# jnvance/DMRG.x

Measured on AMD Instinct MI355X. Metric: superblock MatMults/sec inside the ground-state eigensolve (Lanczos step = 1 MatMult + reorthogonalisation), higher is better.
Workload: dtype f64

## Files before the change

### dmrg.x_amd/_capi.py

```python
import ctypes as C
import os

_HERE = os.path.dirname(os.path.abspath(__file__))
LIB_PATH = os.environ.get("DMRGX_LIB") or os.path.join(_HERE, "libdmrgx_hip.so")

DMRGX_OK = 0
DMRGX_ERR_ARG = 62
DMRGX_ERR_OUTOFRANGE = 63
DMRGX_ERR_DEVICE = 97
DMRGX_ERR_NOTCONV = 91
CELL_DENSE, CELL_IDENT = 1, 2


class DmrgxError(RuntimeError):
    def __init__(self, code, msg):
        super().__init__(f"dmrgx status {code}: {msg}")
        self.code = code


class Cell(C.Structure):
    _fields_ = [("row_sector", C.c_int32), ("r0", C.c_int32), ("c0", C.c_int32), ("nr", C.c_int32), ("nc", C.c_int32),
                ("kind", C.c_int32), ("scale", C.c_double), ("data", C.c_void_p), ("ld", C.c_int64)]


class SecOp(C.Structure):
    _fields_ = [("shift", C.c_int32), ("transposed", C.c_int32), ("ncells", C.c_int32), ("cells", C.POINTER(Cell))]


class Sectors(C.Structure):
    _fields_ = [("nsec", C.c_int32), ("size", C.POINTER(C.c_int32))]


class Term(C.Structure):
    _fields_ = [("a", C.c_double), ("left_op", C.c_int32), ("right_op", C.c_int32)]


class KronDesc(C.Structure):
    _fields_ = [("left", Sectors), ("right", Sectors), ("nblocks", C.c_int32),
                ("block_il", C.POINTER(C.c_int32)), ("block_ir", C.POINTER(C.c_int32)),
                ("n_left_ops", C.c_int32), ("n_right_ops", C.c_int32),
                ("left_ops", C.POINTER(SecOp)), ("right_ops", C.POINTER(SecOp)),
                ("h_left", C.POINTER(SecOp)), ("h_right", C.POINTER(SecOp)),
                ("nterms", C.c_int32), ("terms", C.POINTER(Term)),
                ("world_size", C.c_int32), ("rank", C.c_int32)]


class RdmReport(C.Structure):
    _fields_ = [(k, C.c_int32) for k in ("n_sweeps", "solver", "trid_persistent_matrices", "trid_launch_matrices", "max_workgroups_per_matrix",
                                         "merge_levels", "wy_blocks_max", "timed_out", "process_timeouts", "persistent_off")]


class RdmVecTask(C.Structure):
    _fields_ = [("side", C.c_int32), ("k", C.c_int32), ("count", C.c_int32), ("pad", C.c_int32), ("dst_dev", C.c_void_p), ("ld", C.c_int64)]


class KronInfo(C.Structure):
    _fields_ = [("n_states", C.c_int64), ("vec_len", C.c_int64), ("local_offset", C.c_int64), ("local_len", C.c_int64),
                ("seg_stride", C.c_int64), ("flops_alg", C.c_double), ("bytes_alg", C.c_double), ("flops_exec", C.c_double),
                ("bytes_workspace", C.c_double), ("n_groups", C.c_int32), ("n_tiles_stage1", C.c_int32), ("n_tiles_stage2", C.c_int32),
                ("n_tiles_big", C.c_int32), ("flops_alg_big", C.c_double)]


class AxpyTask(C.Structure):
    _fields_ = [("dst", C.c_void_p), ("dst_base", C.c_void_p), ("src", C.c_void_p), ("ldd", C.c_int64), ("lds", C.c_int64),
                ("nr", C.c_int32), ("nc", C.c_int32), ("transposed", C.c_int32), ("alpha", C.c_double)]


class Dot2dTask(C.Structure):
    _fields_ = [("a", C.c_void_p), ("lda", C.c_int64), ("b", C.c_void_p), ("ldb", C.c_int64), ("nr", C.c_int32), ("nc", C.c_int32), ("out", C.c_int32), ("pad", C.c_int32)]


class GemmTask(C.Structure):
    _fields_ = [("M", C.c_int32), ("N", C.c_int32), ("K", C.c_int32), ("accumulate", C.c_int32),
                ("A", C.c_void_p), ("lda", C.c_int64), ("B", C.c_void_p), ("ldb", C.c_int64), ("C", C.c_void_p), ("ldc", C.c_int64)]


class Rotation(C.Structure):
    _fields_ = [("n_new", C.c_int32), ("old_sector", C.POINTER(C.c_int32)), ("kept", C.POINTER(C.c_int32)), ("rot_t", C.POINTER(C.c_void_p))]


ALLGATHER_FN = C.CFUNCTYPE(C.c_int32, C.c_void_p, C.c_void_p, C.c_int64, C.c_void_p)
ALLREDUCE_FN = C.CFUNCTYPE(C.c_int32, C.c_void_p, C.c_void_p, C.c_int64, C.c_void_p)


class EigsOpts(C.Structure):
    _fields_ = [("ncv", C.c_int32), ("max_it", C.c_int32), ("tol", C.c_double), ("seed", C.c_uint64),
                ("use_initial", C.c_int32), ("max_matvec", C.c_int32), ("allgather", ALLGATHER_FN), ("allreduce_sum", ALLREDUCE_FN), ("user", C.c_void_p),
                ("comm", C.c_void_p), ("method", C.c_int32), ("min_initial_norm2", C.c_double), ("gd_minv", C.c_int32), ("reserved_", C.c_int32)]


class EigsStats(C.Structure):
    _fields_ = [("n_matvec", C.c_int32), ("n_restart", C.c_int32), ("converged", C.c_int32), ("start_rejected", C.c_int32),
                ("residual", C.c_double), ("seconds", C.c_double)]


SIGNATURES = {
    "dmrgx_abi_version": (C.c_int32, []),
    "dmrgx_last_error": (C.c_char_p, []),
    "dmrgx_device_count": (C.c_int32, [C.POINTER(C.c_int32)]),
    "dmrgx_kron_plan_create": (C.c_int32, [C.POINTER(KronDesc), C.c_void_p, C.POINTER(C.c_void_p)]),
    "dmrgx_kron_plan_info": (C.c_int32, [C.c_void_p, C.POINTER(KronInfo)]),
    "dmrgx_kron_apply": (C.c_int32, [C.c_void_p, C.c_void_p, C.c_void_p, C.c_void_p]),
    "dmrgx_kron_plan_destroy": (C.c_int32, [C.c_void_p]),
    "dmrgx_kron_diag": (C.c_int32, [C.c_void_p, C.c_void_p, C.c_void_p]),
    "dmrgx_kron_plan_timing": (C.c_int32, [C.c_void_p, C.c_int32]),
    "dmrgx_kron_plan_timing_read": (C.c_int32, [C.c_void_p, C.POINTER(C.c_double), C.POINTER(C.c_int64)]),
    "dmrgx_kron_vec_to_striped": (C.c_int32, [C.c_void_p, C.c_void_p, C.c_void_p, C.c_void_p]),
    "dmrgx_kron_vec_from_striped": (C.c_int32, [C.c_void_p, C.c_void_p, C.c_void_p, C.c_void_p]),
    "dmrgx_stripe_bounds": (C.c_int32, [C.c_int32, C.c_int32, C.c_int32, C.POINTER(C.c_int32), C.POINTER(C.c_int32)]),
    "dmrgx_stripe_bounds_of_block": (C.c_int32, [C.c_int32, C.c_int32, C.c_int32, C.c_int32, C.POINTER(C.c_int32), C.POINTER(C.c_int32)]),
    "dmrgx_dgemm_nn": (C.c_int32, [C.c_int32, C.c_int32, C.c_int32, C.c_void_p, C.c_int64, C.c_void_p, C.c_int64,
                                   C.c_void_p, C.c_int64, C.c_void_p]),
    "dmrgx_rdm_create": (C.c_int32, [C.POINTER(Sectors), C.POINTER(Sectors), C.c_int32, C.POINTER(C.c_int32), C.POINTER(C.c_int32),
                                     C.c_void_p, C.c_void_p, C.POINTER(C.c_void_p)]),
    "dmrgx_rdm_eigenvalues": (C.c_int32, [C.c_void_p, C.c_int32, C.c_int32, C.POINTER(C.c_double)]),
    "dmrgx_rdm_create_warm": (C.c_int32, [C.POINTER(Sectors), C.POINTER(Sectors), C.c_int32, C.POINTER(C.c_int32), C.POINTER(C.c_int32),
                               C.c_void_p, C.c_void_p, C.c_void_p, C.POINTER(C.c_void_p)]),
    "dmrgx_rdm_eigenvectors": (C.c_int32, [C.c_void_p, C.c_int32, C.c_int32, C.c_int32, C.c_void_p, C.c_int64, C.c_void_p]),
    "dmrgx_rdm_info": (C.c_int32, [C.c_void_p, C.POINTER(RdmReport)]),
    "dmrgx_rdm_select": (C.c_int32, [C.c_void_p, C.POINTER(C.c_int32), C.c_void_p]),
    "dmrgx_rdm_eigenvectors_batch": (C.c_int32, [C.c_void_p, C.c_int32, C.POINTER(RdmVecTask), C.c_void_p]),
    "dmrgx_rdm_destroy": (C.c_int32, [C.c_void_p]),
    "dmrgx_cells_axpy": (C.c_int32, [C.c_int32, C.POINTER(AxpyTask), C.c_void_p]),
    "dmrgx_rotate_ops": (C.c_int32, [C.POINTER(Sectors), C.POINTER(Rotation), C.c_int32, C.POINTER(SecOp), C.POINTER(C.POINTER(C.c_void_p)), C.c_void_p]),
    "dmrgx_malloc": (C.c_int32, [C.POINTER(C.c_void_p), C.c_size_t]),
    "dmrgx_free": (C.c_int32, [C.c_void_p]),
    "dmrgx_mem_stats": (C.c_int32, [C.POINTER(C.c_size_t), C.POINTER(C.c_size_t), C.POINTER(C.c_size_t)]),
    "dmrgx_memcpy_h2d": (C.c_int32, [C.c_void_p, C.c_void_p, C.c_size_t, C.c_void_p]),
    "dmrgx_memcpy_d2h": (C.c_int32, [C.c_void_p, C.c_void_p, C.c_size_t, C.c_void_p]),
    "dmrgx_memcpy_d2d": (C.c_int32, [C.c_void_p, C.c_void_p, C.c_size_t, C.c_void_p]),
    "dmrgx_memset_zero": (C.c_int32, [C.c_void_p, C.c_size_t, C.c_void_p]),
    "dmrgx_stream_sync": (C.c_int32, [C.c_void_p]),
    "dmrgx_dgemm_batch": (C.c_int32, [C.c_int32, C.c_void_p, C.c_void_p]),
    "dmrgx_dot": (C.c_int32, [C.c_int64, C.c_void_p, C.c_void_p, C.POINTER(C.c_double), C.c_void_p]),
    "dmrgx_dot_async": (C.c_int32, [C.c_int64, C.c_void_p, C.c_void_p, C.c_void_p, C.c_void_p]),
    "dmrgx_dot2d_batch": (C.c_int32, [C.c_int32, C.c_void_p, C.c_void_p, C.c_void_p]),
    "dmrgx_eigs_comm_timing": (C.c_int32, [C.POINTER(C.c_double), C.POINTER(C.c_double), C.POINTER(C.c_int64), C.c_int32]),
    "dmrgx_eigs_lowest": (C.c_int32, [C.c_void_p, C.POINTER(EigsOpts), C.POINTER(C.c_double), C.c_void_p,
                                      C.POINTER(EigsStats), C.c_void_p]),
    "dmrgx_rdm_create_subset": (C.c_int32, [C.POINTER(Sectors), C.POINTER(Sectors), C.c_int32, C.POINTER(C.c_int32), C.POINTER(C.c_int32),
                                            C.c_void_p, C.c_void_p, C.c_void_p, C.POINTER(C.c_void_p)]),
    "dmrgx_set_device": (C.c_int32, [C.c_int32]),
    "dmrgx_comm_unique_id": (C.c_int32, [C.c_void_p]),
    "dmrgx_comm_init": (C.c_int32, [C.c_int32, C.c_int32, C.c_void_p, C.POINTER(C.c_void_p)]),
    "dmrgx_comm_init_host_staged": (C.c_int32, [C.c_int32, C.c_int32, C.c_char_p, C.POINTER(C.c_void_p)]),
    "dmrgx_comm_info": (C.c_int32, [C.c_void_p, C.POINTER(C.c_int32), C.POINTER(C.c_int32), C.POINTER(C.c_int32)]),
    "dmrgx_comm_allgather": (C.c_int32, [C.c_void_p, C.c_void_p, C.c_int64, C.c_void_p]),
    "dmrgx_comm_allreduce_sum": (C.c_int32, [C.c_void_p, C.c_void_p, C.c_int64, C.c_void_p]),
    "dmrgx_comm_bcast": (C.c_int32, [C.c_void_p, C.c_void_p, C.c_size_t, C.c_int32, C.c_void_p]),
    "dmrgx_comm_allgather_host": (C.c_int32, [C.c_void_p, C.c_void_p, C.c_void_p, C.c_size_t, C.c_void_p]),
    "dmrgx_comm_barrier": (C.c_int32, [C.c_void_p, C.c_void_p]),
    "dmrgx_comm_destroy": (C.c_int32, [C.c_void_p]),
}

_lib = None


def lib():
    global _lib
    if _lib is None:
        import torch
        if not os.path.exists(LIB_PATH):
            raise ImportError(f"{LIB_PATH} not built: run `make` (hipcc --offload-arch=gfx950). "
                              "The dmrgx hot path has no CPU fallback.")
        L = C.CDLL(LIB_PATH)
        for name, (res, args) in SIGNATURES.items():
            fn = getattr(L, name)
            fn.restype, fn.argtypes = res, args
        if L.dmrgx_abi_version() != 3:
            raise ImportError("dmrgx ABI version mismatch")
        _lib = L
    return _lib


def check(status):
    if status != DMRGX_OK:
        raise DmrgxError(status, lib().dmrgx_last_error().decode(errors="replace"))


def require_device():
    n = C.c_int32(0)
    check(lib().dmrgx_device_count(C.byref(n)))
    return n.value
```

### dmrg.x_amd/csrc/common.h

```cpp
#pragma once
#include <cstring>
#include <hip/hip_runtime.h>
#include <algorithm>
#include <cstdarg>
#include <cstdio>
#include <cstdint>
#include <string>
#include <vector>
#include "dmrgx.h"

namespace dmrgx {

void set_error(const char* fmt, ...);

#define DMRGX_HIP(call)                                                                              \
    do {                                                                                             \
        hipError_t e__ = (call);                                                                     \
        if (e__ != hipSuccess) {                                                                     \
            ::dmrgx::set_error("%s:%d: %s -> %s", __FILE__, __LINE__, #call, hipGetErrorString(e__)); \
            return DMRGX_ERR_DEVICE;                                                                 \
        }                                                                                            \
    } while (0)

#define DMRGX_CHK(call)                    \
    do {                                   \
        dmrgx_status s__ = (call);         \
        if (s__ != DMRGX_OK) return s__;   \
    } while (0)

#define DMRGX_FAIL(code, ...)              \
    do {                                   \
        ::dmrgx::set_error(__VA_ARGS__);   \
        return (code);                     \
    } while (0)

inline int32_t stripe_cut(int32_t n, int32_t W, int32_t w)
{
    if (w <= 0) return 0;
    if (w >= W) return n;
    const int64_t even = ((int64_t)n * w) / W;
    if ((int64_t)n < (int64_t)48 * W) return (int32_t)even;
    const int64_t c16 = ((even + 8) / 16) * 16, c64 = ((even + 32) / 64) * 64;
    const int64_t d64 = c64 > even ? c64 - even : even - c64;
    const int64_t cut = (d64 <= 16 && c64 > 0 && c64 < n) ? c64 : c16;
    return (int32_t)std::min<int64_t>(std::max<int64_t>(cut, 0), n);
}

hipError_t pool_malloc(void** out, size_t bytes);
hipError_t pool_free(void* p);
hipError_t zero_async(void* p, size_t bytes, hipStream_t st);
constexpr uint64_t POISON_F64_BITS = 0x7ff8badbadbadbadull;
bool pool_poison();
hipError_t poison_f64_async(void* p, size_t bytes, hipStream_t st);
void pool_stats(size_t* in_use, size_t* cached, size_t* peak);
hipError_t h2d_async(void* dst, const void* src, size_t bytes, hipStream_t st);

inline int32_t stripe_of_rank(int32_t W, int32_t w, int32_t k) { return (w + k) % W; }

struct DevBuf {
    void* p = nullptr;
    size_t bytes = 0;
    DevBuf() = default;
    DevBuf(const DevBuf&) = delete;
    DevBuf& operator=(const DevBuf&) = delete;
    ~DevBuf() { release(); }
    dmrgx_status alloc(size_t n) {
        release();
        if (n == 0) return DMRGX_OK;
        hipError_t e = pool_malloc(&p, n);
        if (e != hipSuccess) { p = nullptr; set_error("hipMalloc(%zu) failed: %s", n, hipGetErrorString(e)); return DMRGX_ERR_MEM; }
        bytes = n;
        return DMRGX_OK;
    }
    dmrgx_status alloc_f64(size_t count, hipStream_t st) {
        DMRGX_CHK(alloc(count * sizeof(double)));
        if (p && pool_poison()) DMRGX_HIP(poison_f64_async(p, bytes, st));
        return DMRGX_OK;
    }
    void release() { if (p && owned) (void)pool_free(p); p = nullptr; bytes = 0; owned = true; }
    void view(void* ptr, size_t n) { release(); p = n ? ptr : nullptr; bytes = n; owned = false; }
    template <class T> T* as() const { return reinterpret_cast<T*>(p); }
    bool owned = true;
};

template <class T>
dmrgx_status upload(DevBuf& buf, const std::vector<T>& host, hipStream_t st) {
    DMRGX_CHK(buf.alloc(host.size() * sizeof(T)));
    if (!host.empty()) DMRGX_HIP(h2d_async(buf.p, host.data(), host.size() * sizeof(T), st));
    return DMRGX_OK;
}

struct PackedUpload {
    std::vector<char> host;
    template <class T> size_t add(const std::vector<T>& v) {
        const size_t off = (host.size() + 15) & ~(size_t)15, bytes = v.size() * sizeof(T);
        if (host.capacity() < off + bytes) host.reserve(std::max(2 * host.capacity(), off + bytes + (bytes >> 1)));
        host.resize(off);
        if (bytes) { const char* p = reinterpret_cast<const char*>(v.data()); host.insert(host.end(), p, p + bytes); }
        return off;
    }
    dmrgx_status upload(DevBuf& buf, hipStream_t st) {
        DMRGX_CHK(buf.alloc(std::max<size_t>(host.size(), 16)));
        constexpr size_t piece = (size_t)4 << 20;
        for (size_t off = 0; off < host.size(); off += piece)
            DMRGX_HIP(h2d_async(static_cast<char*>(buf.p) + off, host.data() + off, std::min(piece, host.size() - off), st));
        return DMRGX_OK;
    }
    template <class T> static void view(DevBuf& dst, const DevBuf& arena, size_t off, size_t n) { dst.view(static_cast<char*>(arena.p) + off, n * sizeof(T)); }
};
template <class T> inline T* packed_at(const DevBuf& buf, size_t off) { return reinterpret_cast<T*>(static_cast<char*>(buf.p) + off); }

}
```

### dmrg.x_amd/csrc/eigs.hip

```cpp
#include "common.h"
#include <mutex>
#include <algorithm>
#include <chrono>
#include <cmath>
#include <cstring>
#include <cstddef>

namespace dmrgx {
namespace {

constexpr int DOT_BLOCKS = 1024, DOT_THREADS = 256, DOT_CHUNK = 8, MAX_NCV = 64, FUSE_NV = 24, GD_NV = 8;

__device__ __forceinline__ double wave_sum(double v) {
#pragma unroll
    for (int o = 32; o > 0; o >>= 1) v += __shfl_down(v, o, 64);
    return v;
}

template <bool VEC2>
__global__ void __launch_bounds__(DOT_THREADS)
multi_dot_kernel(const double* __restrict__ V, int64_t ldv, int nv, const double* __restrict__ w, int64_t n, double* __restrict__ partial)
{
    __shared__ double red[DOT_THREADS / 64][DOT_CHUNK];
    const int v0 = blockIdx.y * DOT_CHUNK;
// ... 421 lines not shown
#pragma unroll
    for (int i = 0; i < NVMAX + 2; ++i) {
        if ((DOTS && (i < nv || i == NVMAX)) || i == NVMAX + 1) {
            const double s2 = wave_sum(acc[i]);
            if (lane == 0) red[wave][i] = s2;
        }
    }
    __syncthreads();
    if (DOTS) {
        if (threadIdx.x <= nv + 1) {
            const int src = threadIdx.x < nv ? threadIdx.x : (threadIdx.x == nv ? NVMAX : NVMAX + 1);
            double s2 = 0.0;
            for (int wv = 0; wv < DOT_THREADS / 64; ++wv) s2 += red[wv][src];
            partial[(int64_t)threadIdx.x * gridDim.x + blockIdx.x] = s2;
        }
    } else if (threadIdx.x == 0) {
        double s2 = 0.0;
        for (int wv = 0; wv < DOT_THREADS / 64; ++wv) s2 += red[wv][NVMAX + 1];
        partial[blockIdx.x] = s2;
    }
}

__global__ void gd_zero_pads_kernel(double* __restrict__ W, int64_t ld, int count, int64_t n, double* __restrict__ t, double* __restrict__ D)
{
    for (int j = threadIdx.x; j < count; j += blockDim.x) W[(int64_t)j * ld + n] = 0.0;
    if (threadIdx.x == 0) { t[n] = 0.0; D[n] = 0.0; }
}

__global__ void __launch_bounds__(DOT_THREADS)
gd_reduce_look_kernel(const double* __restrict__ partial, double* __restrict__ out, int count, int nblk, int look_idx, int look_only,
                      const GdState* __restrict__ S, double* __restrict__ look)
{
    __shared__ double red[DOT_THREADS / 64];
    const int i = blockIdx.x;
    if (i >= count) return;
    double t = 0.0;
    if (!look_only) {
        double s = 0.0;
        for (int b = threadIdx.x; b < nblk; b += DOT_THREADS) s += partial[(int64_t)i * nblk + b];
        s = wave_sum(s);
        if ((threadIdx.x & 63) == 0) red[threadIdx.x >> 6] = s;
        __syncthreads();
        if (threadIdx.x == 0) { for (int k = 0; k < DOT_THREADS / 64; ++k) t += red[k]; out[i] = t; }
    } else if (threadIdx.x == 0) t = out[i];
    if (threadIdx.x == 0 && i == look_idx) { look[0] = t; look[1] = S->theta; look[2] = S->hv0_2; }
}

__global__ void random_fill_kernel(double* __restrict__ v, int64_t n, uint64_t seed, int64_t index_offset)
{
    for (int64_t e = (int64_t)blockIdx.x * blockDim.x + threadIdx.x; e < n; e += (int64_t)gridDim.x * blockDim.x) {
        uint64_t z = seed + 0x9E3779B97F4A7C15ull * (uint64_t)(e + index_offset + 1);
        z = (z ^ (z >> 30)) * 0xBF58476D1CE4E5B9ull;
        z = (z ^ (z >> 27)) * 0x94D049BB133111EBull;
        z ^= z >> 31;
        v[e] = (double)(z >> 11) * (2.0 / 9007199254740992.0) - 1.0;
    }
}

void jacobi_eigh(int n, std::vector<double>& A, std::vector<double>& w, std::vector<double>& Q)
{
    Q.assign((size_t)n * n, 0.0);
    for (int i = 0; i < n; ++i) Q[(size_t)i * n + i] = 1.0;
    for (int sweep = 0; sweep < 60; ++sweep) {
        double off = 0.0, diag = 0.0;
        for (int i = 0; i < n; ++i) { diag += A[(size_t)i * n + i] * A[(size_t)i * n + i]; for (int j = i + 1; j < n; ++j) off += A[(size_t)i * n + j] * A[(size_t)i * n + j]; }
        if (off <= 1e-32 * (diag + off) || off == 0.0) break;
        for (int p = 0; p < n - 1; ++p)
            for (int q = p + 1; q < n; ++q) {
                const double apq = A[(size_t)p * n + q];
                if (apq == 0.0) continue;
                const double app = A[(size_t)p * n + p], aqq = A[(size_t)q * n + q];
                const double tau = (aqq - app) / (2.0 * apq);
                const double t = (tau >= 0 ? 1.0 : -1.0) / (std::fabs(tau) + std::sqrt(1.0 + tau * tau));
                const double c = 1.0 / std::sqrt(1.0 + t * t), s = t * c;
                for (int k = 0; k < n; ++k) {
                    const double akp = A[(size_t)k * n + p], akq = A[(size_t)k * n + q];
                    A[(size_t)k * n + p] = c * akp - s * akq; A[(size_t)k * n + q] = s * akp + c * akq;
                }
                for (int k = 0; k < n; ++k) {
                    const double apk = A[(size_t)p * n + k], aqk = A[(size_t)q * n + k];
                    A[(size_t)p * n + k] = c * apk - s * aqk; A[(size_t)q * n + k] = s * apk + c * aqk;
                }
                for (int k = 0; k < n; ++k) {
                    const double qkp = Q[(size_t)k * n + p], qkq = Q[(size_t)k * n + q];
                    Q[(size_t)k * n + p] = c * qkp - s * qkq; Q[(size_t)k * n + q] = s * qkp + c * qkq;
                }
            }
    }
    std::vector<int> idx(n);
    for (int i = 0; i < n; ++i) idx[i] = i;
    std::sort(idx.begin(), idx.end(), [&](int a, int b) { return A[(size_t)a * n + a] < A[(size_t)b * n + b]; });
    w.resize(n);
    std::vector<double> Qs((size_t)n * n);
    for (int j = 0; j < n; ++j) { w[j] = A[(size_t)idx[j] * n + idx[j]]; for (int i = 0; i < n; ++i) Qs[(size_t)i * n + j] = Q[(size_t)i * n + idx[j]]; }
    Q.swap(Qs);
}

}
}

using namespace dmrgx;

static dmrgx_status eigs_davidson(dmrgx_kron_plan* plan, const dmrgx_eigs_opts* opts, double* e0, double* psi_full, dmrgx_eigs_stats* stats, hipStream_t st);

namespace {
std::mutex g_ct_mutex;
double g_ct_allgather_ms = 0.0, g_ct_apply_ms = 0.0;
int64_t g_ct_matvecs = 0;
struct CommTimer {
    hipStream_t st;
    std::vector<hipEvent_t> ev;
    size_t used = 0;
    explicit CommTimer(hipStream_t s) : st(s) {}
    void mark()
    {
        if (used == ev.size()) { hipEvent_t e; if (hipEventCreate(&e) != hipSuccess) return; ev.push_back(e); }
        (void)hipEventRecord(ev[used++], st);
    }
    ~CommTimer()
    {
        double ag = 0.0, ap = 0.0; int64_t nmv = 0;
        for (size_t i = 0; i + 2 < used; i += 3) {
            float a = 0.f, b = 0.f;
            if (hipEventSynchronize(ev[i + 2]) != hipSuccess) break;
            if (hipEventElapsedTime(&a, ev[i], ev[i + 1]) == hipSuccess && hipEventElapsedTime(&b, ev[i + 1], ev[i + 2]) == hipSuccess) { ag += a; ap += b; ++nmv; }
        }
        for (hipEvent_t e : ev) (void)hipEventDestroy(e);
        if (nmv) { std::lock_guard<std::mutex> lk(g_ct_mutex); g_ct_allgather_ms += ag; g_ct_apply_ms += ap; g_ct_matvecs += nmv; }
    }
};
}

extern "C" dmrgx_status dmrgx_eigs_comm_timing(double* allgather_ms, double* apply_ms, int64_t* n_matvec, int32_t reset)
{
    std::lock_guard<std::mutex> lk(g_ct_mutex);
    if (allgather_ms) *allgather_ms = g_ct_allgather_ms;
    if (apply_ms) *apply_ms = g_ct_apply_ms;
    if (n_matvec) *n_matvec = g_ct_matvecs;
    if (reset) { g_ct_allgather_ms = 0.0; g_ct_apply_ms = 0.0; g_ct_matvecs = 0; }
    return DMRGX_OK;
}

static double* pinned_scalars()
{
    static thread_local double* p = nullptr;
    if (!p && hipHostMalloc((void**)&p, (8 + MAX_NCV + 2) * sizeof(double), hipHostMallocDefault) != hipSuccess) { (void)hipGetLastError(); p = nullptr; }
    return p;
}
static bool start_too_light(const dmrgx_eigs_opts* opts, const double* pin)
{
    return opts->min_initial_norm2 > 0.0 && pin && !(pin[2] >= opts->min_initial_norm2);
}

extern "C" dmrgx_status dmrgx_eigs_lowest(dmrgx_kron_plan* plan, const dmrgx_eigs_opts* opts, double* e0,
                                          double* psi_full, dmrgx_eigs_stats* stats, void* stream)
{
    hipStream_t st = (hipStream_t)stream;
    if (!plan || !opts || !e0 || !psi_full) DMRGX_FAIL(DMRGX_ERR_ARG, "eigs_lowest: null argument");
    dmrgx_kron_info I;
    DMRGX_CHK(dmrgx_kron_plan_info(plan, &I));
    const bool gd_space = std::min<int64_t>(opts->ncv > 0 ? opts->ncv : 16, I.n_states) >= 2;
    if (opts->method == 1 && opts->use_initial && opts->max_matvec <= 0 && gd_space) return eigs_davidson(plan, opts, e0, psi_full, stats, st);
    const bool dist = I.vec_len != I.n_states;
    const bool hooks = opts->allgather && opts->allreduce_sum;
    if (dist && !hooks && !opts->comm) DMRGX_FAIL(DMRGX_ERR_ARG, "eigs_lowest: a striped plan needs a communicator (opts->comm) or the allgather/allreduce hooks");
    auto gather_full = [&](double* full) -> dmrgx_status {
        return hooks ? opts->allgather(opts->user, full, I.seg_stride, st) : dmrgx_comm_allgather(opts->comm, full, I.seg_stride, st);
    };
    const int64_t n = I.local_len, N = I.n_states;
    int m = opts->ncv > 0 ? opts->ncv : 16;
    m = (int)std::min<int64_t>(std::min(m, MAX_NCV), N);
    if (m < 1) DMRGX_FAIL(DMRGX_ERR_ARG, "eigs_lowest: empty problem");
    const int max_it = opts->max_it > 0 ? opts->max_it : std::max<int>(100, (int)(2 * N / m));
    const double tol = opts->tol > 0 ? opts->tol : 1e-8;
    const auto t_begin = std::chrono::steady_clock::now();

    DevBuf dV, dW, dX, dTmp, dPartial, dScal, dQ;
    DMRGX_CHK(dV.alloc_f64((size_t)(m + 1) * n, st));
    DMRGX_CHK(dW.alloc_f64((size_t)n, st));
    DMRGX_CHK(dTmp.alloc_f64((size_t)(m / 2 + 2) * n, st));
    if (dist) DMRGX_CHK(dX.alloc_f64((size_t)I.vec_len, st));
    DMRGX_CHK(dPartial.alloc_f64((size_t)(MAX_NCV + DOT_CHUNK + 1) * DOT_BLOCKS, st));
    const int row = m + 2;
    DMRGX_CHK(dScal.alloc_f64((size_t)((m + 1) * row + 3 * (MAX_NCV + 2)), st));
    DMRGX_CHK(dQ.alloc_f64((size_t)MAX_NCV * MAX_NCV, st));
    double* V = dV.as<double>();
    double* w = dW.as<double>();
    double* c1 = dScal.as<double>() + (size_t)(m + 1) * row;
    double* c2 = c1 + (MAX_NCV + 2);
    double* nrm = c2 + (MAX_NCV + 2);
    auto Hrow = [&](int j) { return dScal.as<double>() + (size_t)j * row; };
    auto vec = [&](int j) { return V + (size_t)j * n; };
    DMRGX_HIP(zero_async(dV.p, dV.bytes, st));
    DMRGX_HIP(zero_async(dW.p, dW.bytes, st));
    if (dist) DMRGX_HIP(zero_async(dX.p, dX.bytes, st));

    const bool vec2 = (n % 2 == 0);
    const int nblk = DOT_BLOCKS;
    auto allreduce = [&](double* buf, int64_t count) -> dmrgx_status {
        if (!dist) return DMRGX_OK;
        return hooks ? opts->allreduce_sum(opts->user, buf, count, st) : dmrgx_comm_allreduce_sum(opts->comm, buf, count, st);
    };
    auto multi_dot = [&](int nv) -> dmrgx_status {
        const int chunks = (nv + 1 + DOT_CHUNK - 1) / DOT_CHUNK;
        if (vec2) hipLaunchKernelGGL(multi_dot_kernel<true>, dim3(nblk, chunks), dim3(DOT_THREADS), 0, st, V, n, nv, w, n, dPartial.as<double>());
        else hipLaunchKernelGGL(multi_dot_kernel<false>, dim3(nblk, chunks), dim3(DOT_THREADS), 0, st, V, n, nv, w, n, dPartial.as<double>());
        DMRGX_HIP(hipGetLastError());
        hipLaunchKernelGGL(reduce_partials_kernel, dim3(nv + 1), dim3(DOT_THREADS), 0, st, dPartial.as<double>(), c1, nv + 1, nblk);
        DMRGX_HIP(hipGetLastError());
        return allreduce(c1, nv + 1);
    };
    auto multi_axpy = [&](int nv, double* hacc, bool final) -> dmrgx_status {
        if (final) { hipLaunchKernelGGL(norm_after_projection_kernel, dim3(1), dim3(64), 0, st, c1, nv, nrm); DMRGX_HIP(hipGetLastError()); }
        hipLaunchKernelGGL(multi_axpy_kernel, dim3(nblk), dim3(DOT_THREADS), 0, st, V, n, nv, c1, w, n, dPartial.as<double>(), hacc);
        DMRGX_HIP(hipGetLastError());
        return DMRGX_OK;
    };
    auto normalise_into = [&](double* dst) -> dmrgx_status {
        hipLaunchKernelGGL(scale_copy_kernel, dim3(1024), dim3(256), 0, st, w, dst, n, nrm);
        DMRGX_HIP(hipGetLastError());
        return DMRGX_OK;
    };
    CommTimer ctimer(st);
    auto matvec = [&](const double* v_local, double* y_local) -> dmrgx_status {
        if (!dist) return dmrgx_kron_apply(plan, v_local, y_local, st);
        DMRGX_HIP(hipMemcpyAsync(dX.as<double>() + I.local_offset, v_local, (size_t)n * sizeof(double), hipMemcpyDeviceToDevice, st));
        ctimer.mark();
        DMRGX_CHK(gather_full(dX.as<double>()));
        ctimer.mark();
        const dmrgx_status rc = dmrgx_kron_apply(plan, dX.as<double>(), y_local, st);
        ctimer.mark();
        return rc;
    };

    if (opts->use_initial) DMRGX_HIP(hipMemcpyAsync(w, psi_full + I.local_offset, (size_t)n * sizeof(double), hipMemcpyDeviceToDevice, st));
    else {
        if (!dist) { hipLaunchKernelGGL(random_fill_kernel, dim3(1024), dim3(256), 0, st, w, n, opts->seed, (int64_t)0); DMRGX_HIP(hipGetLastError()); }
        else {
            DevBuf ref;
            DMRGX_CHK(ref.alloc((size_t)N * sizeof(double)));
            hipLaunchKernelGGL(random_fill_kernel, dim3(1024), dim3(256), 0, st, ref.as<double>(), N, opts->seed, (int64_t)0);
            DMRGX_HIP(hipGetLastError());
            DMRGX_CHK(dmrgx_kron_vec_to_striped(plan, ref.as<double>(), dX.as<double>(), st));
            DMRGX_HIP(hipMemcpyAsync(w, dX.as<double>() + I.local_offset, (size_t)n * sizeof(double), hipMemcpyDeviceToDevice, st));
            DMRGX_HIP(hipStreamSynchronize(st));
        }
    }
    DMRGX_CHK(multi_dot(0));
    double* const pin = opts->use_initial ? pinned_scalars() : nullptr;
    if (pin) { pin[2] = 0.0; DMRGX_HIP(hipMemcpyAsync(pin + 2, c1, sizeof(double), hipMemcpyDeviceToHost, st)); }
    DMRGX_HIP(hipMemcpyAsync(nrm, c1, sizeof(double), hipMemcpyDeviceToDevice, st));
    DMRGX_CHK(normalise_into(vec(0)));

    const bool looks = opts->max_matvec <= 0;
    static thread_local double* look_buf = nullptr;
    static thread_local hipEvent_t look_ev[2] = {nullptr, nullptr};
    constexpr size_t look_stride = (size_t)(MAX_NCV + 1) * (MAX_NCV + 2);
    if (looks && !look_buf) {
        DMRGX_HIP(hipHostMalloc((void**)&look_buf, 2 * look_stride * sizeof(double), hipHostMallocDefault));
        DMRGX_HIP(hipEventCreateWithFlags(&look_ev[0], hipEventDisableTiming)); DMRGX_HIP(hipEventCreateWithFlags(&look_ev[1], hipEventDisableTiming));
    }
    int look_mm[2] = {0, 0};
    std::vector<double> T((size_t)m * m, 0.0), theta, Q, hbuf((size_t)(m + 1) * row);
    int k = 0, n_matvec = 0, restarts = 0, converged = 0;
    double beta_m = 0.0, resid = 0.0, lambda = 0.0;
    std::vector<double> Qdev;
    auto null_start = [&]() { return opts->use_initial && restarts == 0 && k == 0 && ((!(std::fabs(hbuf[0]) > 0.0) && !(hbuf[(size_t)m + 1] > 0.0)) || start_too_light(opts, pin)); };
    auto redo_from_random = [&]() -> dmrgx_status {
        dV.release(); dW.release(); dTmp.release(); dX.release();
        dmrgx_eigs_opts o2 = *opts;
        o2.use_initial = 0;
        dmrgx_eigs_stats s2;
        memset(&s2, 0, sizeof(s2));
        const dmrgx_status rc = dmrgx_eigs_lowest(plan, &o2, e0, psi_full, &s2, (void*)st);
        if (stats) { *stats = s2; stats->n_matvec += n_matvec; stats->start_rejected = 1;
                     stats->seconds = std::chrono::duration<double>(std::chrono::steady_clock::now() - t_begin).count(); }
        return rc;
    };
    while (true) {
        DMRGX_HIP(zero_async(Hrow(k), (size_t)(m + 1 - k) * row * sizeof(double), st));
        int jend = m;
        if (opts->max_matvec > 0) jend = std::min(m, k + std::max(0, opts->max_matvec - n_matvec));
        const bool capped = jend < m || (opts->max_matvec > 0 && n_matvec + (m - k) >= opts->max_matvec);
        bool early = false;
        for (int j = k; j < jend; ++j) {
            DMRGX_CHK(matvec(vec(j), w));
            ++n_matvec;
            const int nv = j + 1;
            DMRGX_CHK(multi_dot(nv));
            if (nv <= FUSE_NV) {
                hipLaunchKernelGGL(axpy_dot_kernel<FUSE_NV>, dim3(nblk), dim3(DOT_THREADS), 0, st, V, n, nv, c1, w, n, dPartial.as<double>(), Hrow(j));
                DMRGX_HIP(hipGetLastError());
                hipLaunchKernelGGL(reduce_partials_kernel, dim3(nv + 1), dim3(DOT_THREADS), 0, st, dPartial.as<double>(), c2, nv + 1, nblk);
                DMRGX_HIP(hipGetLastError());
                DMRGX_CHK(allreduce(c2, nv + 1));
            } else {
                DMRGX_CHK(multi_axpy(nv, Hrow(j), false));
                DMRGX_CHK(multi_dot(nv));
                DMRGX_HIP(hipMemcpyAsync(c2, c1, (size_t)(nv + 1) * sizeof(double), hipMemcpyDeviceToDevice, st));
            }
            if (vec2) hipLaunchKernelGGL(axpy_normalise_kernel<true>, dim3(nblk), dim3(DOT_THREADS), 0, st, V, n, nv, c2, w, vec(j + 1), n, Hrow(j) + m + 1, Hrow(j));
            else hipLaunchKernelGGL(axpy_normalise_kernel<false>, dim3(nblk), dim3(DOT_THREADS), 0, st, V, n, nv, c2, w, vec(j + 1), n, Hrow(j) + m + 1, Hrow(j));
            DMRGX_HIP(hipGetLastError());
            if (looks && j + 1 < m) {
                const int slot = j & 1;
                DMRGX_HIP(hipMemcpyAsync(look_buf + (size_t)slot * look_stride, dScal.p, (size_t)(m + 1) * row * sizeof(double), hipMemcpyDeviceToHost, st));
                DMRGX_HIP(hipEventRecord(look_ev[slot], st));
                look_mm[slot] = j + 1;
// ... 321 lines not shown
```

### dmrg.x_amd/csrc/ggemm.h

```cpp
#pragma once
#include "common.h"
#include <algorithm>

namespace dmrgx {

enum : int32_t { GPROD_GEMM = 0, GPROD_AXPY = 1 };

struct GProd {
    const double* A;
    const double* B;
    int32_t lda, ldb;
    int32_t K;
    int32_t kind;
    double alpha;
};

struct GGroup {
    double* C;
    int32_t ldc;
    int32_t M, N;
    int32_t prod_begin, prod_end;
    int32_t n_axpy;
    int32_t accumulate;
};

struct GTile { int32_t group, tm, tn, pad; };

constexpr int GG_BM = 64, GG_BN = 64, GG_BK = 16, GG_THREADS = 256;

dmrgx_status ggemm_launch(const GTile* d_tiles, const GGroup* d_groups, const GProd* d_prods, int32_t ntiles, hipStream_t st, int big = 0);

constexpr int GG_CLUSTER = 8;
inline void ggemm_append_tiles(std::vector<GTile>& tiles, int32_t g, int32_t M, int32_t N, int32_t cost = 1) {
    const int32_t TM = (M + GG_BM - 1) / GG_BM, TN = (N + GG_BN - 1) / GG_BN;
    for (int32_t bm = 0; bm < TM; bm += GG_CLUSTER)
        for (int32_t bn = 0; bn < TN; bn += GG_CLUSTER)
            for (int32_t tm = bm; tm < std::min(TM, bm + GG_CLUSTER); ++tm)
                for (int32_t tn = bn; tn < std::min(TN, bn + GG_CLUSTER); ++tn) tiles.push_back(GTile{g, tm, tn, cost});
}

inline void ggemm_append_tiles_mixed(std::vector<GTile>& big, std::vector<GTile>& small, int32_t g, int32_t M, int32_t N, int32_t cost = 1, bool allow_big = true) {
    const int32_t mb = allow_big ? (M / 128) * 2 : 0, nb = allow_big ? (N / 128) * 2 : 0;
    for (int32_t bm = 0; bm < mb; bm += 2 * GG_CLUSTER)
        for (int32_t bn = 0; bn < nb; bn += 2 * GG_CLUSTER)
            for (int32_t tm = bm; tm < std::min(mb, bm + 2 * GG_CLUSTER); tm += 2)
                for (int32_t tn = bn; tn < std::min(nb, bn + 2 * GG_CLUSTER); tn += 2) big.push_back(GTile{g, tm, tn, 4 * cost});
    const int32_t TM = (M + GG_BM - 1) / GG_BM, TN = (N + GG_BN - 1) / GG_BN;
    for (int32_t bm = 0; bm < TM; bm += GG_CLUSTER)
        for (int32_t bn = 0; bn < TN; bn += GG_CLUSTER)
            for (int32_t tm = bm; tm < std::min(TM, bm + GG_CLUSTER); ++tm)
                for (int32_t tn = bn; tn < std::min(TN, bn + GG_CLUSTER); ++tn)
                    if (tm >= mb || tn >= nb) small.push_back(GTile{g, tm, tn, cost});
}

int ggemm_slots(int unit = 1);
void ggemm_schedule_core(std::vector<GTile>& tiles, const std::vector<int32_t>& first_gemm_product_of_group, int unit);
template <class GroupVec>
inline void ggemm_schedule(std::vector<GTile>& tiles, const GroupVec& groups, int unit = 1) {
    std::vector<int32_t> p0(groups.size());
    for (size_t i = 0; i < groups.size(); ++i) p0[i] = groups[i].prod_begin + groups[i].n_axpy < groups[i].prod_end ? groups[i].prod_begin + groups[i].n_axpy : -1;
    ggemm_schedule_core(tiles, p0, unit);
}

struct GemmSet {
    std::vector<GTile> big, small;
    size_t off_big = 0, off_small = 0;
};
struct GemmBatch {
    std::vector<GProd> prods;
    std::vector<GGroup> groups;
    bool skip_empty_k = false;
    size_t off_prods = 0, off_groups = 0;
    const GProd* d_prods = nullptr;
    const GGroup* d_groups = nullptr;

    void group(GemmSet& s, const GGroup& g, int32_t cost) {
        groups.push_back(g);
        ggemm_append_tiles_mixed(s.big, s.small, (int32_t)groups.size() - 1, g.M, g.N, cost);
    }
    void gemm(GemmSet& s, double* C, int32_t ldc, int32_t M, int32_t N, const double* A, int32_t lda, const double* B, int32_t ldb, int32_t K, int32_t accumulate = 0) {
        if (M <= 0 || N <= 0 || (K <= 0 && skip_empty_k)) return;
        const int32_t p0 = (int32_t)prods.size();
        if (K > 0) prods.push_back(GProd{A, B, lda, ldb, K, GPROD_GEMM, 1.0});
        group(s, GGroup{C, ldc, M, N, p0, (int32_t)prods.size(), 0, accumulate}, (K + GG_BK - 1) / GG_BK);
    }
    void pack(PackedUpload& pk) {
        if (prods.empty()) prods.push_back(GProd{nullptr, nullptr, 0, 0, 0, GPROD_GEMM, 0.0});
        if (groups.empty()) groups.push_back(GGroup{nullptr, 0, 0, 0, 0, 0, 0, 0});
        off_prods = pk.add(prods); off_groups = pk.add(groups);
    }
    void pack(GemmSet& s, PackedUpload& pk) const {
        ggemm_schedule(s.big, groups, 2); ggemm_schedule(s.small, groups);
        s.off_big = pk.add(s.big); s.off_small = pk.add(s.small);
    }
    void bind(const DevBuf& tab) { d_prods = packed_at<GProd>(tab, off_prods); d_groups = packed_at<GGroup>(tab, off_groups); }
    dmrgx_status launch(const GemmSet& s, const DevBuf& tab, hipStream_t st) const {
        if (!d_groups) DMRGX_FAIL(DMRGX_ERR_INTERNAL, "GemmBatch::launch before bind");
        DMRGX_CHK(ggemm_launch(packed_at<GTile>(tab, s.off_big), d_groups, d_prods, (int32_t)s.big.size(), st, 1));
        return ggemm_launch(packed_at<GTile>(tab, s.off_small), d_groups, d_prods, (int32_t)s.small.size(), st, 0);
    }
};

}
```

### dmrg.x_amd/csrc/ggemm.hip

```cpp
#include "ggemm.h"
#include <algorithm>
#include <cstdlib>
#include <map>
#include <mutex>
#include <utility>

namespace dmrgx {

typedef double d4 __attribute__((ext_vector_type(4)));

#ifdef DMRGX_TILE_TRACE
#define GG_TRACE_PARAM , unsigned long long* __restrict__ trace
#define GG_STAMP(I) { if (trace && threadIdx.x == 0) trace[(size_t)t * 8 + (I)] = __builtin_amdgcn_s_memrealtime(); }
#define GG_STAMP_ID() { if (trace && threadIdx.x == 0) { unsigned hw, xcc; asm volatile("s_getreg_b32 %0, hwreg(HW_REG_HW_ID)" : "=s"(hw)); asm volatile("s_getreg_b32 %0, hwreg(HW_REG_XCC_ID)" : "=s"(xcc)); trace[(size_t)t * 8 + 7] = ((unsigned long long)xcc << 32) | hw; } }
#define GG_TRACE_FWD , trace
#define GG_CLK0() unsigned long long clk0_ = __builtin_amdgcn_s_memtime();
#define GG_CLK1() { if (trace && threadIdx.x == 0) trace[(size_t)t * 8 + 6] = __builtin_amdgcn_s_memtime() - clk0_; }
#else
#define GG_TRACE_PARAM
#define GG_TRACE_FWD
#define GG_STAMP(I)
#define GG_STAMP_ID()
#define GG_CLK0()
#define GG_CLK1()
#endif
typedef const double __attribute__((address_space(1)))* gptr;
typedef double __attribute__((address_space(1)))* gwptr;
typedef const char __attribute__((address_space(1)))* gbptr;

typedef const GTile __attribute__((address_space(4)))* ktile_ptr;
typedef const GGroup __attribute__((address_space(4)))* kgroup_ptr;
typedef const GProd __attribute__((address_space(4)))* kprod_ptr;
__device__ __forceinline__ GTile kload(ktile_ptr p, int i) { GTile r; r.group = p[i].group; r.tm = p[i].tm; r.tn = p[i].tn; r.pad = p[i].pad; return r; }
__device__ __forceinline__ GGroup kload(kgroup_ptr p, int i)
{
    GGroup r;
    r.C = p[i].C; r.ldc = p[i].ldc; r.M = p[i].M; r.N = p[i].N; r.prod_begin = p[i].prod_begin; r.prod_end = p[i].prod_end;
    r.n_axpy = p[i].n_axpy; r.accumulate = p[i].accumulate;
    return r;
}
__device__ __forceinline__ GProd kload(kprod_ptr p, int i)
{
    GProd r;
    r.A = p[i].A; r.B = p[i].B; r.lda = p[i].lda; r.ldb = p[i].ldb; r.K = p[i].K; r.kind = p[i].kind; r.alpha = p[i].alpha;
    return r;
}


template <int TR, int TC, int WR, int WC, bool DEEP>
__device__ __forceinline__ void
ggemm_body(const GTile* __restrict__ tiles_, const GGroup* __restrict__ groups_, const GProd* __restrict__ prods_, int ntiles, int* __restrict__ ctr GG_TRACE_PARAM)
{
    const ktile_ptr tiles = (ktile_ptr)tiles_;
    const kgroup_ptr groups = (kgroup_ptr)groups_;
    const kprod_ptr prods = (kprod_ptr)prods_;
    constexpr int THREADS = 64 * WR * WC;
    constexpr int BM = 16 * TR * WR, BN = 16 * TC * WC, BK = GG_BK;
    constexpr int AS_LD = BK + 2;
    constexpr int BS_LD = BN + 16;
    constexpr int AROWS = THREADS / 16;
    constexpr int NA = BM / AROWS;
    constexpr int BROWS = THREADS / BN;
    constexpr int NB = BK / BROWS;
    constexpr bool RELAYOUT = (TR == 2 && TC == 2 && WR == 2 && WC == 2);
    extern __shared__ double gg_smem[];
    double (*As)[BM * AS_LD] = (double (*)[BM * AS_LD])gg_smem;
    double (*Bs)[BK * BS_LD] = (double (*)[BK * BS_LD])(gg_smem + 2 * BM * AS_LD);

    const int tid = threadIdx.x, wave = __builtin_amdgcn_readfirstlane(tid >> 6);
    int& sh_next = *(int*)(gg_smem + 2 * BM * AS_LD + 2 * BK * BS_LD);
    const int G = gridDim.x;
    const bool dyn = ntiles > G;
    const int xcd = blockIdx.x & 7, qbase = G >> 3;
    int t = blockIdx.x;
    GTile tl = kload(tiles, t);
    if (tl.group < 0) return;
    GGroup g = kload(groups, tl.group);
    const GTile tl_none = GTile{-1, 0, 0, 0};
#define GG_LANES()                                                                            \
    int tp_ = tid;                                                                            \
    asm volatile("" : "+v"(tp_));                                                             \
    const int a_r = tp_ >> 4, a_k = tp_ & 15, b_k = tp_ / BN, b_j = tp_ % BN;                 \
    (void)a_r; (void)a_k; (void)b_k; (void)b_j;
    unsigned st_a, st_b;
    {
        GG_LANES();
        st_a = (unsigned)(size_t)&As[0][a_r * AS_LD + a_k];
        st_b = (unsigned)(size_t)&Bs[0][b_k * BS_LD + b_j];
    }

    int lm0, ln0, lmrem, lnrem;
    double rc_a[NA], rc_b[NB];
    const double *cA = nullptr, *cB = nullptr;
    int clda = 0, cldb = 0, cK = 0;
    int lp = 0, lk = 0, lpend = 0;
    bool lmore = false;
    int kz[2] = {0, 0};
    int npre = 0;
    int vm_after = 0;

#define GG_LOADER_TILE(TL, GR)                                                                \
    {                                                                                         \
        lm0 = (TL).tm * GG_BM; ln0 = (TL).tn * GG_BN;                                         \
        lmrem = min(BM, (GR).M - lm0);                                                        \
        lnrem = min(BN, (GR).N - ln0);                                                        \
    }
#define GG_PRODUCT_SET(PR)                                                                    \
    {                                                                                         \
        cA = (PR).A; cB = (PR).B; clda = (PR).lda; cldb = (PR).ldb; cK = (PR).K;              \
        const int kc_ = min(cK, BK) - 1;                                                      \
        GG_LANES();                                                                           \
        const int bcol = min(b_j, lnrem - 1);                                                 \
        _Pragma("unroll") for (int s = 0; s < NA; ++s) aoff[s] = ((unsigned)min(a_r + AROWS * s, lmrem - 1) * (unsigned)clda + (unsigned)min(a_k, kc_)) * 8u; \
        _Pragma("unroll") for (int s = 0; s < NB; ++s) boff[s] = ((unsigned)min(b_k + BROWS * s, kc_) * (unsigned)cldb + (unsigned)bcol) * 8u; \
    }
#define GG_PRODUCT(P) { const GProd pr_ = kload(prods, P); GG_PRODUCT_SET(pr_); }
#define GG_RA_0_0 "v[96:97]"
#define GG_CA_0_0 "v96", "v97"
#define GG_RA_0_1 "v[98:99]"
#define GG_CA_0_1 "v98", "v99"
#define GG_RA_0_2 "v[100:101]"
#define GG_CA_0_2 "v100", "v101"
#define GG_RA_0_3 "v[102:103]"
#define GG_CA_0_3 "v102", "v103"
#define GG_RB_0_0 "v[104:105]"
#define GG_CB_0_0 "v104", "v105"
#define GG_RB_0_1 "v[106:107]"
#define GG_CB_0_1 "v106", "v107"
#define GG_RB_0_2 "v[108:109]"
#define GG_CB_0_2 "v108", "v109"
#define GG_RB_0_3 "v[110:111]"
#define GG_CB_0_3 "v110", "v111"
#define GG_RA_1_0 "v[112:113]"
#define GG_CA_1_0 "v112", "v113"
#define GG_RA_1_1 "v[114:115]"
#define GG_CA_1_1 "v114", "v115"
#define GG_RA_1_2 "v[116:117]"
#define GG_CA_1_2 "v116", "v117"
#define GG_RA_1_3 "v[118:119]"
#define GG_CA_1_3 "v118", "v119"
#define GG_RB_1_0 "v[120:121]"
#define GG_CB_1_0 "v120", "v121"
#define GG_RB_1_1 "v[122:123]"
#define GG_CB_1_1 "v122", "v123"
#define GG_RB_1_2 "v[124:125]"
#define GG_CB_1_2 "v124", "v125"
#define GG_RB_1_3 "v[126:127]"
#define GG_CB_1_3 "v126", "v127"
#define GG_ZT_0_0 "v_cndmask_b32_e64 v96, v96, 0, %0\n\tv_cndmask_b32_e64 v97, v97, 0, %0"
#define GG_ZT_0_1 "v_cndmask_b32_e64 v98, v98, 0, %0\n\tv_cndmask_b32_e64 v99, v99, 0, %0"
#define GG_ZT_0_2 "v_cndmask_b32_e64 v100, v100, 0, %0\n\tv_cndmask_b32_e64 v101, v101, 0, %0"
#define GG_ZT_0_3 "v_cndmask_b32_e64 v102, v102, 0, %0\n\tv_cndmask_b32_e64 v103, v103, 0, %0"
#define GG_ZT_1_0 "v_cndmask_b32_e64 v112, v112, 0, %0\n\tv_cndmask_b32_e64 v113, v113, 0, %0"
#define GG_ZT_1_1 "v_cndmask_b32_e64 v114, v114, 0, %0\n\tv_cndmask_b32_e64 v115, v115, 0, %0"
#define GG_ZT_1_2 "v_cndmask_b32_e64 v116, v116, 0, %0\n\tv_cndmask_b32_e64 v117, v117, 0, %0"
#define GG_ZT_1_3 "v_cndmask_b32_e64 v118, v118, 0, %0\n\tv_cndmask_b32_e64 v119, v119, 0, %0"
#define GG_LD1(OP, SET, S, OFFV, BASE, BREG) asm volatile("global_load_dwordx2 " GG_R##OP##_##SET##_##S ", %0, %1" : : "v"(OFFV), BREG(BASE) : "memory", GG_C##OP##_##SET##_##S)
#define GG_ST1(OP, SET, S, ADDR, OFFS) asm volatile("ds_write_b64 %0, " GG_R##OP##_##SET##_##S " offset:%1" : : "v"(ADDR), "i"(OFFS) : "memory")
#define GG_Z1(SET, S) asm volatile(GG_ZT_##SET##_##S : : "s"(zm_) : GG_CA_##SET##_##S)
#define GG_LOADER_NEXT()                                                                      \
    {                                                                                         \
        lk += BK;                                                                             \
        if (lk >= cK) { ++lp; lk = 0; if (lp < lpend) GG_PRODUCT(lp); }                       \
        lmore = lp < lpend;                                                                   \
    }
#define GG_LOADER_BASES()                                                                     \
        const int klast_ = cK - 1 - lk;                                                       \
        const int back_ = (klast_ < BK - 1 && cK >= BK) ? BK - 1 - klast_ : 0;                \
        const int kz_ = klast_ < BK - 1 ? (cK >= BK ? back_ : -(klast_ + 1)) : 0;             \
        gbptr A_ = (gbptr)(cA + (size_t)lm0 * clda + (lk - back_));                           \
        gbptr B_ = (gbptr)(cB + (size_t)(lk - back_) * cldb + ln0);
#define GG_GLOAD_D(SET)                                                                       \
    {                                                                                         \
        static_assert(!DEEP || (NA == 4 && NB == 4), "staging register table");               \
        GG_LOADER_BASES();                                                                    \
        kz[SET] = kz_;                                                                        \
        GG_LD1(A, SET, 0, aoff[0], A_, "{s[96:97]}"); GG_LD1(A, SET, 1, aoff[1 % NA], A_, "{s[96:97]}");   \
        GG_LD1(A, SET, 2, aoff[2 % NA], A_, "{s[96:97]}"); GG_LD1(A, SET, 3, aoff[3 % NA], A_, "{s[96:97]}");   \
        GG_LD1(B, SET, 0, boff[0], B_, "{s[98:99]}"); GG_LD1(B, SET, 1, boff[1 % NB], B_, "{s[98:99]}");   \
        GG_LD1(B, SET, 2, boff[2 % NB], B_, "{s[98:99]}"); GG_LD1(B, SET, 3, boff[3 % NB], B_, "{s[98:99]}");   \
        GG_LOADER_NEXT();                                                                     \
    }
#define GG_VMWAIT(N) asm volatile("s_waitcnt vmcnt(%0)" : : "n"(N) : "memory")
#define GG_LSTORE_D(BUF, SET)                                                                 \
    {                                                                                         \
        if (kz[SET] != 0) {                                                                   \
            GG_LANES();                                                                       \
            const unsigned long long zm_ = __builtin_amdgcn_ballot_w64(kz[SET] > 0 ? a_k < kz[SET] : a_k >= -kz[SET]);   \
            GG_Z1(SET, 0); GG_Z1(SET, 1); GG_Z1(SET, 2); GG_Z1(SET, 3);                       \
        }                                                                                     \
        GG_ST1(A, SET, 0, st_a, 8 * ((BUF) * BM * AS_LD + AROWS * 0 * AS_LD)); GG_ST1(A, SET, 1, st_a, 8 * ((BUF) * BM * AS_LD + AROWS * 1 * AS_LD)); \
        GG_ST1(A, SET, 2, st_a, 8 * ((BUF) * BM * AS_LD + AROWS * 2 * AS_LD)); GG_ST1(A, SET, 3, st_a, 8 * ((BUF) * BM * AS_LD + AROWS * 3 * AS_LD)); \
        GG_ST1(B, SET, 0, st_b, 8 * ((BUF) * BK * BS_LD + BROWS * 0 * BS_LD)); GG_ST1(B, SET, 1, st_b, 8 * ((BUF) * BK * BS_LD + BROWS * 1 * BS_LD)); \
        GG_ST1(B, SET, 2, st_b, 8 * ((BUF) * BK * BS_LD + BROWS * 2 * BS_LD)); GG_ST1(B, SET, 3, st_b, 8 * ((BUF) * BK * BS_LD + BROWS * 3 * BS_LD)); \
    }
#define GG_GLOAD_C()                                                                          \
    {                                                                                         \
        GG_LOADER_BASES();                                                                    \
        kz[0] = kz_;                                                                          \
        _Pragma("unroll") for (int s = 0; s < NA; ++s) rc_a[s] = *(gptr)(A_ + aoff[s]);       \
        _Pragma("unroll") for (int s = 0; s < NB; ++s) rc_b[s] = *(gptr)(B_ + boff[s]);       \
        GG_LOADER_NEXT();                                                                     \
    }
#define GG_LSTORE_C(BUF)                                                                      \
    {                                                                                         \
        if (kz[0] != 0) {                                                                     \
            GG_LANES();                                                                       \
            const bool z_ = kz[0] > 0 ? a_k < kz[0] : a_k >= -kz[0];                          \
            _Pragma("unroll") for (int s = 0; s < NA; ++s) rc_a[s] = z_ ? 0.0 : rc_a[s];      \
        }                                                                                     \
        _Pragma("unroll") for (int s = 0; s < NA; ++s)                                        \
            asm volatile("ds_write_b64 %0, %1 offset:%2" : : "v"(st_a), "v"(rc_a[s]), "i"(8 * ((BUF) * BM * AS_LD + AROWS * s * AS_LD)) : "memory"); \
        _Pragma("unroll") for (int s = 0; s < NB; ++s)                                        \
            asm volatile("ds_write_b64 %0, %1 offset:%2" : : "v"(st_b), "v"(rc_b[s]), "i"(8 * ((BUF) * BK * BS_LD + BROWS * s * BS_LD)) : "memory"); \
    }

#define GG_FRAG(SET, BUF, KK)                                                                 \
    {                                                                                         \
        _Pragma("unroll") for (int mi = 0; mi < TR; ++mi)                                     \
            asm volatile("ds_read_b64 %0, %1 offset:%2" : "=v"(fa[SET][mi]) : "v"(lds_a), "i"(8 * ((BUF) * BM * AS_LD + 16 * AS_LD * mi + (KK))) : "memory"); \
        _Pragma("unroll") for (int ni = 0; ni < TC; ++ni)                                     \
            asm volatile("ds_read_b64 %0, %1 offset:%2" : "=v"(fb[SET][ni]) : "v"(lds_b), "i"(8 * ((BUF) * BK * BS_LD + (KK) * BS_LD + 16 * ni)) : "memory"); \
    }
#define GG_FRAG_WAIT(SET)                                                                     \
    {                                                                                         \
        asm volatile("s_waitcnt lgkmcnt(0)" ::: "memory");                                    \
        _Pragma("unroll") for (int mi = 0; mi < TR; ++mi) asm volatile("" : "+v"(fa[SET][mi])); \
        _Pragma("unroll") for (int ni = 0; ni < TC; ++ni) asm volatile("" : "+v"(fb[SET][ni])); \
    }
#define GG_MFMA(SET, GUARD, I0, I1)       \
    {                                                                                         \
        _Pragma("unroll") for (int q = (I0); q < (I1); ++q) {                                 \
            const int mi = q / TC, ni = q % TC;                                               \
            GUARD(acc[mi][ni], fa[SET][mi], fb[SET][ni], q);                                  \
        }                                                                                     \
        __builtin_amdgcn_sched_barrier(0);                                                    \
    }
#define GG_CLAIM()                                                                            \
    asm volatile("s_mov_b64 s[94:95], exec\n\ts_mov_b64 exec, 1\n\tglobal_atomic_add %0, %1, %2, %3 sc0\n\ts_mov_b64 exec, s[94:95]" \
                 : "+v"(claim) : "v"(0u), "v"(1u), "{s[92:93]}"(ctr + xcd) : "memory", "s94", "s95")
#define GG_STEP_D(BUF, OTH, GUARD)                                                            \
    {                                                                                         \
        constexpr int NM = TR * TC;                                                           \
        GG_FRAG_WAIT(0);                                                                      \
        GG_MFMA(0, GUARD, 0, 1);                                                              \
        const bool ld_ = lmore;                                                               \
        __builtin_amdgcn_sched_barrier(0);                                                    \
        GG_MFMA(0, GUARD, 1, 2);                                                              \
        if (ld_) {                                                                            \
            GG_GLOAD_D(BUF);                                                                  \
            if (dyn && !lmore && wave == 0) GG_CLAIM();    \
        }                                                                                     \
        __builtin_amdgcn_sched_barrier(0);                                                    \
        GG_MFMA(0, GUARD, 2, NM - 1);                                                         \
        GG_FRAG(1, BUF, 4);                                                                   \
        GG_MFMA(0, GUARD, NM - 1, NM);                                                        \
        GG_FRAG_WAIT(1);                                                                      \
        GG_MFMA(1, GUARD, 0, NM - 1);                                                         \
        GG_FRAG(0, BUF, 8);                                                                   \
        GG_MFMA(1, GUARD, NM - 1, NM);                                                        \
        GG_FRAG_WAIT(0);                                                                      \
        GG_MFMA(0, GUARD, 0, 1);                                                              \
        if (have1) {                                                                          \
            if (ld_ && lmore) { GG_VMWAIT(NA + NB); } else { GG_VMWAIT(0); }    \
            GG_LSTORE_D(OTH, OTH);                                                            \
        }                                                                                     \
        __builtin_amdgcn_sched_barrier(0);                                                    \
        GG_MFMA(0, GUARD, 1, NM - 1);                                                         \
        GG_FRAG(1, BUF, 12);                                                                  \
        GG_MFMA(0, GUARD, NM - 1, NM);                                                        \
        GG_FRAG_WAIT(1);                                                                      \
        __syncthreads();                                                                      \
        if (have1) GG_FRAG(0, OTH, 0);                                                        \
        __builtin_amdgcn_sched_barrier(0);                                                    \
        GG_MFMA(1, GUARD, 0, NM);                                                             \
        have = have1; have1 = ld_;                                                            \
    }
#define GG_STEP_C(BUF, OTH, GUARD)                                                            \
    {                                                                                         \
        constexpr int NM = TR * TC;                                                           \
        GG_FRAG_WAIT(0);                                                                      \
        GG_MFMA(0, GUARD, 0, 1);                                                              \
        const bool ld_ = lmore;                                                               \
        __builtin_amdgcn_sched_barrier(0);                                                    \
        GG_MFMA(0, GUARD, 1, 2);                                                              \
        if (ld_) {                                                                            \
            GG_GLOAD_C();                                                                     \
            if (dyn && !lmore && wave == 0) GG_CLAIM();                                       \
        }                                                                                     \
        __builtin_amdgcn_sched_barrier(0);                                                    \
        GG_MFMA(0, GUARD, 2, NM - 1);                                                         \
        GG_FRAG(1, BUF, 4);                                                                   \
        GG_MFMA(0, GUARD, NM - 1, NM);                                                        \
        GG_FRAG_WAIT(1);                                                                      \
        GG_MFMA(1, GUARD, 0, NM - 1);                                                         \
        GG_FRAG(0, BUF, 8);                                                                   \
        GG_MFMA(1, GUARD, NM - 1, NM);                                                        \
        GG_FRAG_WAIT(0);                                                                      \
        GG_MFMA(0, GUARD, 0, 1);                                                              \
        if (ld_) GG_LSTORE_C(OTH);                                                            \
        __builtin_amdgcn_sched_barrier(0);                                                    \
        GG_MFMA(0, GUARD, 1, NM - 1);                                                         \
        GG_FRAG(1, BUF, 12);                                                                  \
        GG_MFMA(0, GUARD, NM - 1, NM);                                                        \
        GG_FRAG_WAIT(1);                                                                      \
        __syncthreads();                                                                      \
        if (ld_) GG_FRAG(0, OTH, 0);                                                          \
        __builtin_amdgcn_sched_barrier(0);                                                    \
        GG_MFMA(1, GUARD, 0, NM);                                                             \
        have = ld_;                                                                           \
    }
#define GG_STREAM(GUARD)                                                                      \
    while (have) {                                                                            \
        if (DEEP) { GG_STEP_D(0, 1, GUARD); } else { GG_STEP_C(0, 1, GUARD); }                \
        if (!have) break;                                                                     \
        if (DEEP) { GG_STEP_D(1, 0, GUARD); } else { GG_STEP_C(1, 0, GUARD); }                \
    }

    for (;;) {
        GG_STAMP(0);
        unsigned aoff[NA], boff[NB];
        const int m0 = tl.tm * GG_BM, n0 = tl.tn * GG_BN;
        const int mrem = min(BM, g.M - m0), nrem = min(BN, g.N - n0);
        int wrow = (wave / WC) * 16 * TR, wcol = (wave % WC) * 16 * TC;
        int tr_eff, tc_eff;
        if (RELAYOUT && mrem <= 32) {
            wrow = 0; wcol = 16 * wave;
            tr_eff = (mrem + 15) >> 4; tc_eff = nrem > wcol ? 1 : 0;
        } else if (RELAYOUT && nrem <= 32) {
            wrow = 16 * wave; wcol = 0;
            tr_eff = mrem > wrow ? 1 : 0; tc_eff = (nrem + 15) >> 4;
        } else {
            tr_eff = min(TR, max(0, (mrem - wrow + 15) >> 4)); tc_eff = min(TC, max(0, (nrem - wcol + 15) >> 4));
        }
        unsigned lds_a, lds_b;
        {
            int tf = tid;
            asm volatile("" : "+v"(tf));
            const int l15 = tf & 15, l4 = (tf >> 4) & 3;
            lds_a = (unsigned)(size_t)&As[0][(wrow + l15) * AS_LD + l4];
            lds_b = (unsigned)(size_t)&Bs[0][l4 * BS_LD + wcol + l15];
        }
        double fa[2][TR], fb[2][TC];

        d4 acc[TR][TC];
#pragma unroll
        for (int mi = 0; mi < TR; ++mi)
#pragma unroll
            for (int ni = 0; ni < TC; ++ni) acc[mi][ni] = (d4){0.0, 0.0, 0.0, 0.0};

        const int pend = g.prod_end;
        const int p0 = tl.pad >= 0 ? tl.pad : pend;
        if (npre == 0 && p0 < pend) {
            GG_LOADER_TILE(tl, g);
            lp = p0; lk = 0; lpend = pend;
            GG_PRODUCT(lp);
            GG_STAMP(1);
            vm_after = 0;
            if (DEEP) { GG_GLOAD_D(0); npre = 1; if (lmore) { GG_GLOAD_D(1); npre = 2; vm_after = NA + NB; } }
            else { GG_GLOAD_C(); npre = 1; }
        } else if (lmore) {
            GG_PRODUCT(lp);
        } else {
#pragma unroll
            for (int s = 0; s < NA; ++s) aoff[s] = 0u;
#pragma unroll
            for (int s = 0; s < NB; ++s) boff[s] = 0u;
        }
        bool have = npre >= 1, have1 = npre >= 2;
        (void)have1;
        if (have) {
            if (DEEP) {
                if (vm_after == NA + NB) { GG_VMWAIT(NA + NB); }
                else if (vm_after == NA + NB + TR * TC * 4) { GG_VMWAIT(NA + NB + TR * TC * 4); }
                else if (vm_after == TR * TC * 4) { GG_VMWAIT(TR * TC * 4); }
                else { GG_VMWAIT(0); }
                GG_LSTORE_D(0, 0);
            } else GG_LSTORE_C(0);
        }
        npre = 0;
        unsigned claim = 0xffffffffu;
        if (dyn && have && !lmore && wave == 0) GG_CLAIM();
        __syncthreads();
        GG_STAMP(2);
        GG_CLK0();
        if (have) GG_FRAG(0, 0, 0);
        unsigned gmask = 0;
#pragma unroll
        for (int q = 0; q < TR * TC; ++q) gmask |= ((q / TC) < tr_eff && (q % TC) < tc_eff) ? (1u << q) : 0u;
gmask = __builtin_amdgcn_readfirstlane(gmask);
#define GG_ALL(ACC, FA, FB, Q) ACC = __builtin_amdgcn_mfma_f64_16x16x4f64(FA, FB, ACC, 0, 0, 0)
#define GG_BIT(ACC, FA, FB, Q)                                                                \
        asm volatile("s_bitcmp1_b32 %3, %4\n\ts_cbranch_scc0 1f\n\tv_mfma_f64_16x16x4_f64 %0, %1, %2, %0\n1:" : "+v"(ACC) : "v"(FA), "v"(FB), "s"(gmask), "n"(Q) : "scc")
        if (TR * TC > 6) { GG_STREAM(GG_ALL) }
        else { GG_STREAM(GG_BIT) }
        GG_STAMP(3);
        GG_CLK1();
#pragma unroll
        for (int s = 0; s < NA; ++s) asm volatile("" : "=v"(rc_a[s]));
#pragma unroll
        for (int s = 0; s < NB; ++s) asm volatile("" : "=v"(rc_b[s]));
        int t_n = ntiles;
        if (dyn) {
            asm volatile("s_waitcnt vmcnt(0)" : "+v"(claim) : : "memory");
            if (tid == 0) sh_next = claim != 0xffffffffu ? (int)claim : (int)atomicAdd(&ctr[xcd], 1);
            __syncthreads();
            t_n = xcd + 8 * (__builtin_amdgcn_readfirstlane(sh_next) + qbase);
        }
        const GTile tl_n = t_n < ntiles ? kload(tiles, t_n) : tl_none;
        const bool nx = tl_n.group >= 0;
        GGroup g_n = g;
        GProd pr_n = GProd{nullptr, nullptr, 0, 0, 0, 0, 0.0};
        if (nx) g_n = kload(groups, tl_n.group);
        if (nx && tl_n.pad >= 0) pr_n = kload(prods, tl_n.pad);

        int tq = tid;
        asm volatile("" : "+v"(tq));
        const int el15 = tq & 15, el4 = (tq >> 4) & 3;
        const int erow = wrow + el4, ecol = wcol + el15;
        int q = g.prod_begin;
        const int axpy_end = q + g.n_axpy;
        const bool full_tile = mrem == BM && nrem == BN;
        if (DEEP && full_tile && q < axpy_end) {
#define GG_SREG_0 "v[96:97]"
#define GG_SCLB_0 "v96", "v97"
#define GG_SREG_1 "v[98:99]"
#define GG_SCLB_1 "v98", "v99"
#define GG_SREG_2 "v[100:101]"
#define GG_SCLB_2 "v100", "v101"
#define GG_SREG_3 "v[102:103]"
#define GG_SCLB_3 "v102", "v103"
#define GG_SREG_4 "v[104:105]"
#define GG_SCLB_4 "v104", "v105"
#define GG_SREG_5 "v[106:107]"
#define GG_SCLB_5 "v106", "v107"
#define GG_SREG_6 "v[108:109]"
#define GG_SCLB_6 "v108", "v109"
#define GG_SREG_7 "v[110:111]"
#define GG_SCLB_7 "v110", "v111"
#define GG_SREG_8 "v[112:113]"
#define GG_SCLB_8 "v112", "v113"
#define GG_SREG_9 "v[114:115]"
#define GG_SCLB_9 "v114", "v115"
#define GG_SREG_10 "v[116:117]"
#define GG_SCLB_10 "v116", "v117"
#define GG_SREG_11 "v[118:119]"
#define GG_SCLB_11 "v118", "v119"
#define GG_SREG_12 "v[120:121]"
#define GG_SCLB_12 "v120", "v121"
#define GG_SREG_13 "v[122:123]"
#define GG_SCLB_13 "v122", "v123"
#define GG_SREG_14 "v[124:125]"
#define GG_SCLB_14 "v124", "v125"
#define GG_SREG_15 "v[126:127]"
#define GG_SCLB_15 "v126", "v127"
#define GG_SLD(U, OFFV, BASE, IMM) asm volatile("global_load_dwordx2 " GG_SREG_##U ", %0, %1 offset:" #IMM : : "v"(OFFV), "{s[96:97]}"(BASE) : "memory", GG_SCLB_##U)
#define GG_SFMA(U, EL, AL) { double t_ = EL; asm volatile("v_fma_f64 %0, %1, " GG_SREG_##U ", %0" : "+v"(t_) : "s"(AL)); EL = t_; }
#define GG_SLOAD0(PR)                                                                         \
            {                                                                                 \
                const unsigned lo_ = ((unsigned)erow * (unsigned)(PR).ldb + (unsigned)ecol) * 8u;   \
                { gbptr S_ = (gbptr)((PR).B + (size_t)(m0 + 0 + 4 * 0) * (PR).ldb + n0); GG_SLD(0, lo_, S_, 0); GG_SLD(1, lo_, S_, 128); } \
                { gbptr S_ = (gbptr)((PR).B + (size_t)(m0 + 0 + 4 * 1) * (PR).ldb + n0); GG_SLD(2, lo_, S_, 0); GG_SLD(3, lo_, S_, 128); } \
                { gbptr S_ = (gbptr)((PR).B + (size_t)(m0 + 0 + 4 * 2) * (PR).ldb + n0); GG_SLD(4, lo_, S_, 0); GG_SLD(5, lo_, S_, 128); } \
                { gbptr S_ = (gbptr)((PR).B + (size_t)(m0 + 0 + 4 * 3) * (PR).ldb + n0); GG_SLD(6, lo_, S_, 0); GG_SLD(7, lo_, S_, 128); } \
            }
#define GG_SLOAD1(PR)                                                                         \
            {                                                                                 \
                const unsigned lo_ = ((unsigned)erow * (unsigned)(PR).ldb + (unsigned)ecol) * 8u;   \
                { gbptr S_ = (gbptr)((PR).B + (size_t)(m0 + 16 + 4 * 0) * (PR).ldb + n0); GG_SLD(8, lo_, S_, 0); GG_SLD(9, lo_, S_, 128); } \
                { gbptr S_ = (gbptr)((PR).B + (size_t)(m0 + 16 + 4 * 1) * (PR).ldb + n0); GG_SLD(10, lo_, S_, 0); GG_SLD(11, lo_, S_, 128); } \
                { gbptr S_ = (gbptr)((PR).B + (size_t)(m0 + 16 + 4 * 2) * (PR).ldb + n0); GG_SLD(12, lo_, S_, 0); GG_SLD(13, lo_, S_, 128); } \
                { gbptr S_ = (gbptr)((PR).B + (size_t)(m0 + 16 + 4 * 3) * (PR).ldb + n0); GG_SLD(14, lo_, S_, 0); GG_SLD(15, lo_, S_, 128); } \
            }
#define GG_SFMA0(AL)                                                                          \
            {                                                                                 \
                GG_SFMA(0, acc[0][0][0], AL); \
                GG_SFMA(1, acc[0][1][0], AL); \
                GG_SFMA(2, acc[0][0][1], AL); \
                GG_SFMA(3, acc[0][1][1], AL); \
                GG_SFMA(4, acc[0][0][2], AL); \
                GG_SFMA(5, acc[0][1][2], AL); \
                GG_SFMA(6, acc[0][0][3], AL); \
                GG_SFMA(7, acc[0][1][3], AL); \
            }
#define GG_SFMA1(AL)                                                                          \
            {                                                                                 \
                GG_SFMA(8, acc[1][0][0], AL); \
                GG_SFMA(9, acc[1][1][0], AL); \
                GG_SFMA(10, acc[1][0][1], AL); \
                GG_SFMA(11, acc[1][1][1], AL); \
                GG_SFMA(12, acc[1][0][2], AL); \
                GG_SFMA(13, acc[1][1][2], AL); \
                GG_SFMA(14, acc[1][0][3], AL); \
                GG_SFMA(15, acc[1][1][3], AL); \
            }
            static_assert(!DEEP || (TR == 2 && TC == 2), "scaled-copy register table");
            GProd pa = kload(prods, q);
            GG_SLOAD0(pa); GG_SLOAD1(pa);
            for (; q < axpy_end; ++q) {
                const bool more = q + 1 < axpy_end;
                const GProd pb = more ? kload(prods, q + 1) : pa;
                const double al = pa.alpha;
                GG_VMWAIT(8);
                GG_SFMA0(al);
                if (more) { GG_SLOAD0(pb); GG_VMWAIT(8); } else { GG_VMWAIT(0); }
                GG_SFMA1(al);
                if (more) GG_SLOAD1(pb);
                pa = pb;
            }
#undef GG_SLOAD0
#undef GG_SLOAD1
#undef GG_SFMA0
#undef GG_SFMA1
        }
        for (; q < axpy_end; ++q) {
            const GProd pr = kload(prods, q);
            gbptr S = (gbptr)(pr.B + (size_t)m0 * pr.ldb + n0);
#pragma unroll
            for (int mi = 0; mi < TR; ++mi)
#pragma unroll
                for (int ni = 0; ni < TC; ++ni)
#pragma unroll
                    for (int r = 0; r < 4; ++r) {
                        const int row = erow + mi * 16 + 4 * r, col = ecol + ni * 16;
                        if (row < mrem && col < nrem && mi < tr_eff && ni < tc_eff) acc[mi][ni][r] += pr.alpha * *(gptr)(S + ((unsigned)row * (unsigned)pr.ldb + (unsigned)col) * 8u);
                    }
        }
        GG_STAMP(4);

        vm_after = 0;
        if (nx && tl_n.pad >= 0) {
            GG_LOADER_TILE(tl_n, g_n);
            lp = tl_n.pad; lk = 0; lpend = g_n.prod_end;
            GG_PRODUCT_SET(pr_n);
            if (DEEP) { GG_GLOAD_D(0); npre = 1; if (lmore) { GG_GLOAD_D(1); npre = 2; vm_after = NA + NB; } }
            else { GG_GLOAD_C(); npre = 1; }
        }

        if (full_tile && !g.accumulate) {
            const unsigned lo = ((unsigned)erow * (unsigned)g.ldc + (unsigned)ecol) * 8u;
#pragma unroll
            for (int mi = 0; mi < TR; ++mi)
#pragma unroll
                for (int r = 0; r < 4; ++r) {
                    char __attribute__((address_space(1)))* C = (char __attribute__((address_space(1)))*)(g.C + (size_t)(m0 + mi * 16 + 4 * r) * g.ldc + n0);
#pragma unroll
                    for (int ni = 0; ni < TC; ++ni)
                        asm volatile("global_store_dwordx2 %0, %1, %2 offset:%3" : : "v"(lo), "v"(acc[mi][ni][r]), "s"(C), "n"(ni * 128) : "memory");
                }
            vm_after += TR * TC * 4;
        } else {
            vm_after = -1;
            char __attribute__((address_space(1)))* C = (char __attribute__((address_space(1)))*)(g.C + (size_t)m0 * g.ldc + n0);
#pragma unroll
            for (int mi = 0; mi < TR; ++mi)
#pragma unroll
                for (int r = 0; r < 4; ++r) {
                    const int row = erow + mi * 16 + 4 * r;
                    const unsigned ro = (unsigned)row * (unsigned)g.ldc;
#pragma unroll
                    for (int ni = 0; ni < TC; ++ni) {
                        const int col = ecol + ni * 16;
                        if (row < mrem && col < nrem && mi < tr_eff && ni < tc_eff) {
                            gwptr c = (gwptr)(C + (ro + (unsigned)col) * 8u);
                            *c = g.accumulate ? (*c + acc[mi][ni][r]) : acc[mi][ni][r];
                        }
                    }
                }
        }
        GG_STAMP(5);
        GG_STAMP_ID();
        if (!nx) break;
        t = t_n; tl = tl_n; g = g_n;
    }
#undef GG_STREAM
#undef GG_STEP
#undef GG_FRAG
#undef GG_FRAG_WAIT
#undef GG_MFMA
#undef GG_PRODUCT
#undef GG_PRODUCT_SET
#undef GG_LOADER_TILE
#undef GG_GLOAD_D
#undef GG_GLOAD_C
#undef GG_LSTORE_D
#undef GG_LSTORE_C
}

__global__ void __launch_bounds__(256) __attribute__((amdgpu_waves_per_eu(5, 5)))
ggemm_kernel_64(const GTile* __restrict__ tiles, const GGroup* __restrict__ groups, const GProd* __restrict__ prods, int ntiles, int* __restrict__ ctr GG_TRACE_PARAM)
{
    ggemm_body<2, 2, 2, 2, true>(tiles, groups, prods, ntiles, ctr GG_TRACE_FWD);
}
__global__ void __launch_bounds__(512, 4)
ggemm_kernel_128(const GTile* __restrict__ tiles, const GGroup* __restrict__ groups, const GProd* __restrict__ prods, int ntiles, int* __restrict__ ctr GG_TRACE_PARAM)
{
    ggemm_body<4, 2, 2, 4, false>(tiles, groups, prods, ntiles, ctr GG_TRACE_FWD);
}


int ggemm_slots(int unit)
{
    static std::mutex mu;
    static int cus_of[64] = {0};
    int dev = 0;
    if (hipGetDevice(&dev) != hipSuccess || dev < 0 || dev >= 64) { (void)hipGetLastError(); dev = 0; }
    int cus;
    {
        std::lock_guard<std::mutex> lock(mu);
        if (cus_of[dev] == 0) {
            int n = 0;
            if (hipDeviceGetAttribute(&n, hipDeviceAttributeMultiprocessorCount, dev) != hipSuccess || n <= 0) { (void)hipGetLastError(); n = 256; }
            cus_of[dev] = (n / 8) * 8 > 0 ? (n / 8) * 8 : 8;
        }
        cus = cus_of[dev];
    }
    return (unit == 2 ? 2 : 4) * cus;
}

static inline int64_t tile_cost(const GTile& t) { return 4 * (int64_t)t.pad + 12; }

void ggemm_schedule_core(std::vector<GTile>& tiles, const std::vector<int32_t>& first_gemm, int unit)
{
    constexpr int NX = 8;
    if (tiles.empty()) return;
    if (tiles.size() <= (size_t)ggemm_slots(unit) / 4) {
        for (GTile& t : tiles) t.pad = first_gemm[(size_t)t.group];
        return;
    }
    struct Cl { uint32_t begin, end; int32_t len16; int64_t cost; };
    static_assert(GG_CLUSTER == 8, "cluster edge as a shift");
    const int sh = unit == 2 ? 4 : 3;
    static thread_local std::vector<Cl> cl;
    cl.clear();
    const size_t nt = tiles.size();
    for (size_t i = 0; i < nt;) {
        size_t j = i;
        int64_t c = 0;
        const int32_t grp = tiles[i].group, cm = tiles[i].tm >> sh, cn = tiles[i].tn >> sh;
        while (j < nt && tiles[j].group == grp && (tiles[j].tm >> sh) == cm && (tiles[j].tn >> sh) == cn && j - i < 256) { c += tile_cost(tiles[j]); ++j; }
        cl.push_back(Cl{(uint32_t)i, (uint32_t)j, tiles[i].pad >> 4, c});
        i = j;
    }
    std::stable_sort(cl.begin(), cl.end(), [](const Cl& a, const Cl& b) { return a.cost > b.cost; });
    static thread_local std::vector<Cl> binc[NX];
    int64_t load[NX] = {0};
    size_t count[NX] = {0};
    for (int x = 0; x < NX; ++x) binc[x].clear();
    for (const Cl& c : cl) {
        int best = 0;
        for (int x = 1; x < NX; ++x) if (load[x] < load[best]) best = x;
        load[best] += c.cost;
        count[best] += c.end - c.begin;
        binc[best].push_back(c);
    }
    size_t maxbin = 0;
    for (int x = 0; x < NX; ++x) maxbin = std::max(maxbin, count[x]);
    std::vector<GTile> out(maxbin * NX, GTile{-1, 0, 0, -1});
    for (int x = 0; x < NX; ++x) {
        std::stable_sort(binc[x].begin(), binc[x].end(), [](const Cl& a, const Cl& b) { return a.len16 > b.len16; });
        size_t pos = (size_t)x;
        for (const Cl& c : binc[x])
            for (uint32_t t = c.begin; t < c.end; ++t, pos += NX) { GTile v = tiles[t]; v.pad = first_gemm[(size_t)v.group]; out[pos] = v; }
    }
    tiles.swap(out);
}

#ifdef DMRGX_TILE_TRACE
static unsigned long long* g_trace_buf = nullptr;
static size_t g_trace_cap = 0, g_trace_used = 0;
extern "C" void dmrgx_debug_tile_trace(void* dev_buf, size_t capacity_words) { g_trace_buf = (unsigned long long*)dev_buf; g_trace_cap = capacity_words; g_trace_used = 0; }
extern "C" size_t dmrgx_debug_tile_trace_used() { return g_trace_used; }
#define GG_TRACE_ARG , trace_
#else
#define GG_TRACE_ARG
#endif

dmrgx_status ggemm_launch(const GTile* d_tiles, const GGroup* d_groups, const GProd* d_prods, int32_t ntiles, hipStream_t st, int big)
{
    if (ntiles <= 0) return DMRGX_OK;
#ifdef DMRGX_TILE_TRACE
    unsigned long long* trace_ = nullptr;
    if (g_trace_buf && g_trace_used + (size_t)ntiles * 8 <= g_trace_cap) { trace_ = g_trace_buf + g_trace_used; g_trace_used += (size_t)ntiles * 8; }
#endif
    const unsigned grid = (unsigned)std::min(ntiles, ggemm_slots(big ? 2 : 1));
    int* ctr = nullptr;
    if (ntiles > (int32_t)grid) {
        constexpr unsigned HALF = 512;
        struct Ring { int* base; unsigned next; };
        static std::mutex mu;
        static std::map<std::pair<int, hipStream_t>, Ring> rings;
        int dev = 0;
        DMRGX_HIP(hipGetDevice(&dev));
        std::lock_guard<std::mutex> lock(mu);
        Ring& r = rings[std::make_pair(dev, st)];
        if (!r.base) { DMRGX_HIP(hipMalloc((void**)&r.base, 2 * HALF * 16 * sizeof(int))); r.next = 0; }
        const unsigned slot = r.next % (2 * HALF);
        if (slot % HALF == 0) DMRGX_HIP(hipMemsetAsync(r.base + (size_t)slot * 16, 0, HALF * 16 * sizeof(int), st));
        r.next = slot + 1;
        ctr = r.base + (size_t)slot * 16;
    }
    constexpr size_t lds64 = (2 * 64 * (GG_BK + 2) + 2 * GG_BK * (64 + 16)) * sizeof(double) + 16, lds128 = (2 * 128 * (GG_BK + 2) + 2 * GG_BK * (128 + 16)) * sizeof(double) + 16;
    if (big) hipLaunchKernelGGL(ggemm_kernel_128, dim3(grid), dim3(512), lds128, st, d_tiles, d_groups, d_prods, ntiles, ctr GG_TRACE_ARG);
    else hipLaunchKernelGGL(ggemm_kernel_64, dim3(grid), dim3(256), lds64, st, d_tiles, d_groups, d_prods, ntiles, ctr GG_TRACE_ARG);
    DMRGX_HIP(hipGetLastError());
    return DMRGX_OK;
}

}
```

### dmrg.x_amd/csrc/kron_plan.hip

```cpp
#include "ggemm.h"
#include <algorithm>
#include <functional>
#include <map>
#include <set>
#include <tuple>
#include <cstring>
#include <memory>
#include <new>

namespace dmrgx {

namespace {

struct NCell {
    int32_t q, r0, c0, nr, nc, kind;
    double scale;
    const double* data;
    int64_t ld;
    bool tr;
};

struct PCell {
    int32_t q, r0, c0, nr, nc, kind;
    double scale;
    int64_t off;
};

struct CopyTask {
    int64_t dst_off;
    const double* src;
    int64_t lds;
    int32_t nr, nc, ldd, tr;
    double a;
    int32_t round;
};

struct CopyTile { int32_t task, ti, tj, pad; };

struct ZeroRect { int64_t off; int32_t ld, nr, nc, pad; };
__global__ void __launch_bounds__(256) zero_rects_kernel(const ZeroRect* __restrict__ rects, double* __restrict__ arena)
{
    const ZeroRect r = rects[blockIdx.x];
    const int64_t n = (int64_t)r.nr * r.nc;
    for (int64_t e = (int64_t)blockIdx.y * 256 + threadIdx.x; e < n; e += (int64_t)gridDim.y * 256) arena[r.off + (e / r.nc) * r.ld + e % r.nc] = 0.0;
}

__global__ void __launch_bounds__(256)
cell_copy_kernel(const CopyTile* __restrict__ tiles, const CopyTask* __restrict__ tasks, double* __restrict__ arena)
{
    __shared__ double buf[32][33];
    const CopyTile t = tiles[blockIdx.x];
    const CopyTask k = tasks[t.task];
    const int tx = threadIdx.x & 31, ty = threadIdx.x >> 5;
    const int i0 = t.ti * 32, j0 = t.tj * 32;
    double* dst = arena + k.dst_off;
    if (!k.tr) {
        for (int r = ty; r < 32; r += 8) {
            const int i = i0 + r, j = j0 + tx;
            if (i < k.nr && j < k.nc) { const double v = k.a * k.src[(size_t)i * k.lds + j]; double& o = dst[(size_t)i * k.ldd + j]; o = k.round == 0 ? v : o + v; }
        }
    } else {
        for (int r = ty; r < 32; r += 8) {
            const int j = j0 + r, i = i0 + tx;
            buf[r][tx] = (i < k.nr && j < k.nc) ? k.src[(size_t)j * k.lds + i] : 0.0;
        }
        __syncthreads();
        for (int r = ty; r < 32; r += 8) {
            const int i = i0 + r, j = j0 + tx;
            if (i < k.nr && j < k.nc) { const double v = k.a * buf[tx][r]; double& o = dst[(size_t)i * k.ldd + j]; o = k.round == 0 ? v : o + v; }
        }
    }
}

struct LayoutSeg { int64_t ref_off, full_off; int32_t nrow, ncol, ref_ld, full_ld; };
__global__ void layout_copy_kernel(const LayoutSeg* __restrict__ segs, const double* __restrict__ src, double* __restrict__ dst, int to_striped)
{
    const LayoutSeg s = segs[blockIdx.y];
    const int64_t n = (int64_t)s.nrow * s.ncol;
    for (int64_t e = (int64_t)blockIdx.x * blockDim.x + threadIdx.x; e < n; e += (int64_t)gridDim.x * blockDim.x) {
        const int64_t i = e / s.ncol, j = e % s.ncol;
        const int64_t a = s.ref_off + i * s.ref_ld + j, b = s.full_off + i * s.full_ld + j;
        if (to_striped) dst[b] = src[a]; else dst[a] = src[b];
    }
}

struct RedTask { int64_t dst_off, slab_off; int32_t ldc, M, N, nslab; };
struct RedTile { int32_t task, chunk; };
constexpr int RED_CHUNK = 2048;
__global__ __launch_bounds__(256) void slab_reduce_kernel(const RedTile* __restrict__ tiles, const RedTask* __restrict__ tasks,
                                                          double* __restrict__ y, const double* __restrict__ arena)
{
    const RedTile t = tiles[blockIdx.x];
    const RedTask k = tasks[t.task];
    const uint32_t mn = (uint32_t)k.M * (uint32_t)k.N, N = (uint32_t)k.N;
    const double* sl = arena + k.slab_off;
    double* yb = y + k.dst_off;
    constexpr int NE = RED_CHUNK / 256;
    const uint32_t e0 = (uint32_t)t.chunk * RED_CHUNK + threadIdx.x;
    double v[NE];
    double* d[NE];
#pragma unroll
    for (int i = 0; i < NE; ++i) {
        const uint32_t e = min(e0 + (uint32_t)i * 256u, mn - 1);
        const uint32_t row = e / N, col = e - row * N;
        d[i] = yb + (size_t)row * k.ldc + col;
        v[i] = *d[i];
    }
    for (int s = 0; s < k.nslab; ++s) {
        const double* p = sl + (size_t)s * mn;
#pragma unroll
        for (int i = 0; i < NE; ++i) v[i] += p[min(e0 + (uint32_t)i * 256u, mn - 1)];
    }
#pragma unroll
    for (int i = 0; i < NE; ++i) if (e0 + (uint32_t)i * 256u < mn) *d[i] = v[i];
}

struct DiagSrc { int64_t off; int32_t ld, n, round; int64_t dst; double scale; };
struct DiagSeg { int64_t out_off; int32_t nrow, ncol; int64_t l0, r0; };
__global__ void __launch_bounds__(256) diag_gather_kernel(const DiagSrc* __restrict__ src, int nsrc, int round, const double* __restrict__ arena, double* __restrict__ dvec)
{
    const int t = blockIdx.x;
    if (t >= nsrc) return;
    const DiagSrc s = src[t];
    if (s.round != round) return;
    for (int i = threadIdx.x; i < s.n; i += 256) dvec[s.dst + i] += s.off >= 0 ? arena[s.off + (int64_t)i * (s.ld + 1)] : s.scale;
}
__global__ void __launch_bounds__(256) diag_fill_kernel(const DiagSeg* __restrict__ segs, const double* __restrict__ dA, const double* __restrict__ dB,
                                                         int nterms, int64_t NL, int64_t NR, double* __restrict__ out)
{
    const DiagSeg s = segs[blockIdx.y];
    const int64_t n = (int64_t)s.nrow * s.ncol;
    for (int64_t e = (int64_t)blockIdx.x * 256 + threadIdx.x; e < n; e += (int64_t)gridDim.x * 256) {
        const int64_t l = e / s.ncol, r = e % s.ncol;
        double d = 0.0;
        for (int t = 0; t < nterms; ++t) d += dA[(int64_t)t * NL + s.l0 + l] * dB[(int64_t)t * NR + s.r0 + r];
        out[s.out_off + e] = d;
    }
}

}
}

using namespace dmrgx;

enum : int32_t { BASE_ARENA = 0, BASE_X = 1, BASE_Y = 2 };

namespace dmrgx {
struct RelProd { int64_t a_off, b_off; int32_t lda, ldb, K, kind; double alpha; int32_t a_base, b_base; };
struct RelGroup { int64_t c_off; int32_t c_base, ldc, M, N, prod_begin, prod_end, n_axpy, accumulate; };

__global__ void patch_tables_kernel(const RelProd* __restrict__ rp, GProd* __restrict__ gp, int np,
                                    const RelGroup* __restrict__ rg, GGroup* __restrict__ gg, int ng,
                                    double* arena, const double* x, double* y)
{
    const int i = blockIdx.x * blockDim.x + threadIdx.x;
    const double* bases[3] = {arena, x, y};
    if (i < np) {
        const RelProd r = rp[i];
        GProd g;
        g.A = bases[r.a_base] + r.a_off; g.B = bases[r.b_base] + r.b_off;
        g.lda = r.lda; g.ldb = r.ldb; g.K = r.K; g.kind = r.kind; g.alpha = r.alpha;
        gp[i] = g;
    }
    if (i < ng) {
        const RelGroup r = rg[i];
        GGroup g;
        g.C = const_cast<double*>(bases[r.c_base]) + r.c_off;
        g.ldc = r.ldc; g.M = r.M; g.N = r.N; g.prod_begin = r.prod_begin; g.prod_end = r.prod_end;
        g.n_axpy = r.n_axpy; g.accumulate = r.accumulate;
        gg[i] = g;
    }
}
}

struct dmrgx_kron_plan {
    int32_t world = 1, rank = 0;
    dmrgx_kron_info info{};
    DevBuf arena;
    DevBuf d_tables;
    DevBuf d_rprods, d_rgroups;
    struct Patched { const double* x = nullptr; double* y = nullptr; DevBuf prods, groups; };
    std::vector<std::unique_ptr<Patched>> patched;
    size_t patched_next = 0;
    static constexpr size_t PATCHED_MAX = 24;
    DevBuf d_tiles1, d_tiles2, d_tiles1b, d_tiles2b;
    int32_t nprods = 0, ngroups = 0, ntiles1 = 0, ntiles2 = 0, ntiles1b = 0, ntiles2b = 0;
    DevBuf d_layout;
    int32_t nlayout = 0;
    DevBuf d_red_tasks, d_red_tiles;
    int32_t n_red_tiles = 0;
    std::vector<DiagSrc> diag_src;
    std::vector<DiagSeg> diag_segs;
    int32_t diag_terms = 0, diag_rounds = 0;
    int64_t diag_NL = 0, diag_NR = 0;
    bool timing = false;
    std::vector<hipEvent_t> ev;
    size_t ev_used = 0;
    ~dmrgx_kron_plan() { for (hipEvent_t e : ev) (void)hipEventDestroy(e); }
};

namespace {

dmrgx_status normalise_op(const dmrgx_secop* op, const dmrgx_sectors& sec, const char* what, std::vector<NCell>& out)
{
    out.clear();
    if (!op) return DMRGX_OK;
    if (op->ncells < 0 || (op->ncells > 0 && !op->cells)) DMRGX_FAIL(DMRGX_ERR_ARG, "%s: bad cell list", what);
    for (int32_t i = 0; i < op->ncells; ++i) {
        const dmrgx_cell& c = op->cells[i];
        NCell n;
        if (!op->transposed) { n.q = c.row_sector; n.r0 = c.r0; n.c0 = c.c0; n.nr = c.nr; n.nc = c.nc; n.tr = false; }
        else { n.q = c.row_sector - op->shift; n.r0 = c.c0; n.c0 = c.r0; n.nr = c.nc; n.nc = c.nr; n.tr = true; }
        n.kind = c.kind; n.scale = c.scale; n.data = c.data; n.ld = c.ld;
        const int32_t qc = n.q + op->shift;
        if (n.q < 0 || n.q >= sec.nsec || qc < 0 || qc >= sec.nsec)
            DMRGX_FAIL(DMRGX_ERR_OUTOFRANGE, "%s: cell %d sector (%d -> %d) out of range [0,%d)", what, i, n.q, qc, sec.nsec);
        if (n.nr <= 0 || n.nc <= 0 || n.r0 < 0 || n.c0 < 0 || n.r0 + n.nr > sec.size[n.q] || n.c0 + n.nc > sec.size[qc])
            DMRGX_FAIL(DMRGX_ERR_OUTOFRANGE, "%s: cell %d rectangle [%d+%d, %d+%d) exceeds block %d x %d", what, i,
                       n.r0, n.nr, n.c0, n.nc, sec.size[n.q], sec.size[qc]);
        if (n.kind == DMRGX_CELL_IDENT) { if (n.nr != n.nc) DMRGX_FAIL(DMRGX_ERR_ARG, "%s: identity cell %d not square", what, i); }
        else if (n.kind == DMRGX_CELL_DENSE) {
            if (!n.data || n.ld < (n.tr ? n.nr : n.nc)) DMRGX_FAIL(DMRGX_ERR_ARG, "%s: dense cell %d has no data / bad ld", what, i);
        } else DMRGX_FAIL(DMRGX_ERR_ARG, "%s: cell %d has unknown kind %d", what, i, n.kind);
        out.push_back(n);
    }
    return DMRGX_OK;
}

struct Builder {
    std::vector<RelProd> prods;
    std::vector<RelGroup> groups;
    std::vector<GTile> tiles1, tiles2, tiles1b, tiles2b;
    std::vector<int32_t> stage2_groups;
    double flops_alg = 0, flops_exec = 0, flops_alg_big = 0;
    static constexpr bool big = false;
    void append_tiles(std::vector<GTile>& b, std::vector<GTile>& s64, int32_t g, int32_t M, int32_t N, int32_t cost) { ggemm_append_tiles_mixed(b, s64, g, M, N, cost, big); }
    int32_t max_split = 1;

    int32_t ksteps(int32_t g) const {
        int32_t c = 0;
        for (int32_t p = groups[g].prod_begin; p < groups[g].prod_end; ++p)
            c += prods[p].kind == GPROD_GEMM ? (prods[p].K + GG_BK - 1) / GG_BK : 1;
        return c;
    }

    std::vector<RedTask> red_tasks;
    std::vector<RedTile> red_tiles;
    int64_t slab_elems = 0;
    void finalize_stage2(int64_t slab_base) {
        double total = 0;
        for (int32_t g : stage2_groups) {
            const RelGroup& G = groups[g];
            total += (double)ksteps(g) * ((G.M + GG_BM - 1) / GG_BM) * ((G.N + GG_BN - 1) / GG_BN);
        }
        constexpr double units = 8192.0;
        const double min_seg = std::min(16.0, std::max(4.0, total / 1024.0));
        const double seg_target = std::max(total / units, min_seg);
        const size_t ng = stage2_groups.size();
        for (size_t gi = 0; gi < ng; ++gi) {
            const int32_t g = stage2_groups[gi];
            const int32_t cost = ksteps(g);
            const int32_t axpy_begin = groups[g].prod_begin, gemm_begin = groups[g].prod_begin + groups[g].n_axpy, gemm_end = groups[g].prod_end;
            int32_t gcost = 0;
            for (int32_t p = gemm_begin; p < gemm_end; ++p) gcost += (prods[p].K + GG_BK - 1) / GG_BK;
            std::vector<int32_t> cuts;
            {
                int32_t S = (int32_t)std::min<double>(64.0, std::max(1.0, std::floor(gcost / seg_target + 0.5)));
                if ((int64_t)groups[g].M * groups[g].N >= (int64_t)1 << 31) S = 1;
                if (gcost < 2) S = 1;
                S = std::min(S, gcost);
                for (int32_t i = 1; i < S; ++i) cuts.push_back((int32_t)(((int64_t)gcost * i) / S));
                cuts.push_back(gcost);
                cuts.erase(std::unique(cuts.begin(), cuts.end()), cuts.end());
            }
            const int32_t S = (int32_t)cuts.size();
            if (S == 1) { append_tiles(tiles2b, tiles2, g, groups[g].M, groups[g].N, cost); continue; }
            max_split = std::max(max_split, S);
            const int64_t mn = (int64_t)groups[g].M * groups[g].N;
            red_tasks.push_back(RedTask{groups[g].c_off, slab_base + slab_elems, groups[g].ldc, groups[g].M, groups[g].N, S - 1});
            for (int64_t c = 0; c * RED_CHUNK < mn; ++c) red_tiles.push_back(RedTile{(int32_t)red_tasks.size() - 1, (int32_t)c});
            std::vector<int32_t> pstart;
            { int32_t acc = 0; for (int32_t p = gemm_begin; p < gemm_end; ++p) { pstart.push_back(acc); acc += (prods[p].K + GG_BK - 1) / GG_BK; } }
            const int32_t n_axpy = groups[g].n_axpy;
            int32_t lo = 0, pcur = gemm_begin;
            for (int32_t sidx = 0; sidx < S; ++sidx) {
                const int32_t hi = cuts[sidx];
                const int32_t nb = (int32_t)prods.size();
                int32_t n_axpy_seg = 0;
                for (int32_t q = sidx; q < n_axpy; q += S) { const RelProd ax = prods[axpy_begin + q]; prods.push_back(ax); ++n_axpy_seg; }
                while (pcur < gemm_end && pstart[pcur - gemm_begin] + (prods[pcur].K + GG_BK - 1) / GG_BK <= lo) ++pcur;
                for (int32_t p = pcur; p < gemm_end; ++p) {
                    const int32_t ps = pstart[p - gemm_begin], pe = ps + (prods[p].K + GG_BK - 1) / GG_BK;
                    if (ps >= hi) break;
                    const int32_t olo = std::max(lo, ps), ohi = std::min(hi, pe);
                    if (olo >= ohi) continue;
                    RelProd sub = prods[p];
                    const int32_t k0 = (olo - ps) * GG_BK, k1 = std::min(prods[p].K, (ohi - ps) * GG_BK);
                    sub.a_off += k0; sub.b_off += (int64_t)k0 * sub.ldb; sub.K = k1 - k0;
                    prods.push_back(sub);
                }
                const int32_t ne = (int32_t)prods.size();
                if (sidx == 0) {
                    groups[g].prod_begin = nb; groups[g].prod_end = ne; groups[g].n_axpy = n_axpy_seg;
                    append_tiles(tiles2b, tiles2, g, groups[g].M, groups[g].N, (hi - lo) + n_axpy_seg);
                } else {
                    RelGroup ng2 = groups[g];
                    ng2.c_base = BASE_ARENA;
                    ng2.c_off = slab_base + slab_elems + (int64_t)(sidx - 1) * mn;
                    ng2.ldc = ng2.N;
                    ng2.prod_begin = nb; ng2.prod_end = ne; ng2.n_axpy = n_axpy_seg; ng2.accumulate = 0;
                    groups.push_back(ng2);
                    append_tiles(tiles2b, tiles2, (int32_t)groups.size() - 1, ng2.M, ng2.N, (hi - lo) + n_axpy_seg);
                }
                lo = hi;
            }
            slab_elems += (int64_t)(S - 1) * mn;
        }
    }

    int32_t open(int32_t c_base, int64_t c_off, int32_t ldc, int32_t M, int32_t N, int32_t accumulate) {
        RelGroup g{c_off, c_base, ldc, M, N, (int32_t)prods.size(), (int32_t)prods.size(), 0, accumulate};
        groups.push_back(g);
        return (int32_t)groups.size() - 1;
    }
    void add_gemm(int32_t a_base, int64_t a_off, int32_t lda, int32_t b_base, int64_t b_off, int32_t ldb, int32_t K) {
        prods.push_back(RelProd{a_off, b_off, lda, ldb, K, GPROD_GEMM, 1.0, a_base, b_base});
    }
    void add_axpy(int32_t s_base, int64_t s_off, int32_t lds, double alpha) {
        prods.push_back(RelProd{0, s_off, 0, lds, 0, GPROD_AXPY, alpha, BASE_ARENA, s_base});
    }
    void close(int32_t g, int stage) {
        RelGroup& G = groups[g];
        G.prod_end = (int32_t)prods.size();
        std::stable_sort(prods.begin() + G.prod_begin, prods.end(), [](const RelProd& a, const RelProd& b) { return a.kind > b.kind; });
        G.n_axpy = 0;
        for (int32_t p = G.prod_begin; p < G.prod_end; ++p) {
            const double mn = (double)G.M * G.N;
            if (prods[p].kind == GPROD_AXPY) { G.n_axpy++; flops_alg += 2.0 * mn; }
            else {
                flops_alg += 2.0 * mn * prods[p].K;
                const double tm = (G.M + 15) / 16, tn = (G.N + 15) / 16;
                flops_exec += 2.0 * tm * tn * 256.0 * (double)(((prods[p].K + 3) / 4) * 4);
                if (big) flops_alg_big += 2.0 * (double)((G.M / 128) * 128) * (double)((G.N / 128) * 128) * prods[p].K;
            }
        }
        if (stage == 1) append_tiles(tiles1b, tiles1, g, G.M, G.N, ksteps(g));
        else stage2_groups.push_back(g);
    }
};

}

extern "C" dmrgx_status dmrgx_kron_plan_create(const dmrgx_kron_desc* d, void* stream, dmrgx_kron_plan** out)
{
    hipStream_t st = (hipStream_t)stream;
    if (!d || !out) DMRGX_FAIL(DMRGX_ERR_ARG, "kron_plan_create: null argument");
    *out = nullptr;
    const int32_t W = d->world_size <= 0 ? 1 : d->world_size, me = d->rank;
    if (me < 0 || me >= W) DMRGX_FAIL(DMRGX_ERR_ARG, "kron_plan_create: rank %d outside world %d", me, W);
    const dmrgx_sectors& SL = d->left;
    const dmrgx_sectors& SR = d->right;
    if (SL.nsec <= 0 || SR.nsec <= 0 || !SL.size || !SR.size) DMRGX_FAIL(DMRGX_ERR_ARG, "kron_plan_create: empty sector table");
    for (int i = 0; i < SL.nsec; ++i) if (SL.size[i] <= 0) DMRGX_FAIL(DMRGX_ERR_ARG, "left sector %d has size %d", i, SL.size[i]);
    for (int i = 0; i < SR.nsec; ++i) if (SR.size[i] <= 0) DMRGX_FAIL(DMRGX_ERR_ARG, "right sector %d has size %d", i, SR.size[i]);
    const int32_t nb = d->nblocks;
    if (nb <= 0 || !d->block_il || !d->block_ir) DMRGX_FAIL(DMRGX_ERR_ARG, "kron_plan_create: no KronBlocks");

    std::map<std::pair<int32_t, int32_t>, int32_t> kmap;
    std::vector<int64_t> ref_off(nb + 1, 0);
    for (int32_t k = 0; k < nb; ++k) {
        const int32_t il = d->block_il[k], ir = d->block_ir[k];
        if (il < 0 || il >= SL.nsec || ir < 0 || ir >= SR.nsec) DMRGX_FAIL(DMRGX_ERR_OUTOFRANGE, "KronBlock %d = (%d,%d) out of range", k, il, ir);
        if (!kmap.emplace(std::make_pair(il, ir), k).second) DMRGX_FAIL(DMRGX_ERR_ARG, "KronBlock (%d,%d) listed twice", il, ir);
        ref_off[k + 1] = ref_off[k] + (int64_t)SL.size[il] * SR.size[ir];
    }
    const int64_t N = ref_off[nb];
    auto nLk = [&](int32_t k) { return SL.size[d->block_il[k]]; };
    auto nRk = [&](int32_t k) { return SR.size[d->block_ir[k]]; };
    auto cbeg = [&](int32_t k, int32_t w) { return stripe_cut(nRk(k), W, stripe_of_rank(W, w, k)); };
    auto cend = [&](int32_t k, int32_t w) { return stripe_cut(nRk(k), W, stripe_of_rank(W, w, k) + 1); };
    std::vector<std::vector<int64_t>> seg_off(W, std::vector<int64_t>(nb + 1, 0));
    int64_t max_seg = 0;
    for (int32_t w = 0; w < W; ++w) {
        for (int32_t k = 0; k < nb; ++k) seg_off[w][k + 1] = seg_off[w][k] + (int64_t)nLk(k) * (cend(k, w) - cbeg(k, w));
        max_seg = std::max(max_seg, seg_off[w][nb]);
    }
    const int64_t seg_stride = (W == 1) ? N : ((max_seg + 63) / 64) * 64;
    auto panel_off = [&](int32_t k, int32_t w) { return (int64_t)w * seg_stride + seg_off[w][k]; };
    auto panel_ld = [&](int32_t k, int32_t w) { return cend(k, w) - cbeg(k, w); };

    if (d->n_left_ops < 0 || d->n_right_ops < 0 || d->nterms < 0) DMRGX_FAIL(DMRGX_ERR_ARG, "negative count");
    std::vector<std::vector<NCell>> Lops(d->n_left_ops), Rops(d->n_right_ops);
    std::vector<NCell> HL, HR;
    for (int32_t i = 0; i < d->n_left_ops; ++i) DMRGX_CHK(normalise_op(&d->left_ops[i], SL, "left op", Lops[i]));
    for (int32_t i = 0; i < d->n_right_ops; ++i) DMRGX_CHK(normalise_op(&d->right_ops[i], SR, "right op", Rops[i]));
    if (d->h_left) { if (d->h_left->shift != 0) DMRGX_FAIL(DMRGX_ERR_ARG, "H_L must have shift 0"); DMRGX_CHK(normalise_op(d->h_left, SL, "H_L", HL)); }
    if (d->h_right) { if (d->h_right->shift != 0) DMRGX_FAIL(DMRGX_ERR_ARG, "H_R must have shift 0"); DMRGX_CHK(normalise_op(d->h_right, SR, "H_R", HR)); }

    std::set<int32_t> usedL, usedR;
    for (int32_t t = 0; t < d->nterms; ++t) {
        const dmrgx_term& T = d->terms[t];
        if (T.left_op < 0 || T.left_op >= d->n_left_ops || T.right_op < 0 || T.right_op >= d->n_right_ops)
            DMRGX_FAIL(DMRGX_ERR_OUTOFRANGE, "term %d references operator (%d,%d) out of range", t, T.left_op, T.right_op);
        if (d->left_ops[T.left_op].shift + d->right_ops[T.right_op].shift != 0)
            DMRGX_FAIL(DMRGX_ERR_ARG, "term %d does not conserve Sz (shifts %d,%d)", t, d->left_ops[T.left_op].shift, d->right_ops[T.right_op].shift);
        if (T.a != 0.0) { usedL.insert(T.left_op); usedR.insert(T.right_op); }
    }
    std::vector<char> coverL(d->n_left_ops, 0), coverR(d->n_right_ops, 0);
    {
        std::vector<std::vector<int32_t>> adj(d->n_left_ops);
        for (int32_t t = 0; t < d->nterms; ++t) if (d->terms[t].a != 0.0) adj[d->terms[t].left_op].push_back(d->terms[t].right_op);
        std::vector<int32_t> matchR(d->n_right_ops, -1), matchL(d->n_left_ops, -1);
        std::vector<char> seen;
        std::function<bool(int32_t)> augment = [&](int32_t l) -> bool {
            for (int32_t r : adj[l]) {
                if (seen[r]) continue;
                seen[r] = 1;
                if (matchR[r] < 0 || augment(matchR[r])) { matchR[r] = l; matchL[l] = r; return true; }
            }
            return false;
        };
        for (int32_t l : usedL) { seen.assign(d->n_right_ops, 0); augment(l); }
        std::vector<char> zL(d->n_left_ops, 0), zR(d->n_right_ops, 0);
        std::vector<int32_t> stack;
        for (int32_t l : usedL) if (matchL[l] < 0) { zL[l] = 1; stack.push_back(l); }
        while (!stack.empty()) {
            const int32_t l = stack.back(); stack.pop_back();
            for (int32_t r : adj[l]) {
                if (zR[r] || matchL[l] == r) continue;
                zR[r] = 1;
                const int32_t l2 = matchR[r];
                if (l2 >= 0 && !zL[l2]) { zL[l2] = 1; stack.push_back(l2); }
            }
        }
        for (int32_t l : usedL) coverL[l] = !zL[l];
        for (int32_t r : usedR) coverR[r] = zR[r];
    }
    struct Group { int32_t sA, sB; std::vector<PCell> left, rightT; };
    std::vector<Group> G;
    std::vector<CopyTask> copies;
    int64_t arena_ops = 0;
    auto new_dense = [&](int32_t nr, int32_t nc) { int64_t o = arena_ops; arena_ops += (int64_t)nr * nc; return o; };

    auto build_side = [&](const std::vector<std::pair<double, const std::vector<NCell>*>>& contrib, bool transpose_out, std::vector<PCell>& dst) {
        std::map<std::tuple<int32_t, int32_t, int32_t, int32_t, int32_t, int32_t>, int32_t> index;
        std::map<int32_t, int32_t> rounds;
        for (auto& ct : contrib) {
            for (const NCell& c : *ct.second) {
                auto key = std::make_tuple(c.q, c.r0, c.c0, c.nr, c.nc, c.kind);
                auto it = index.find(key);
                int32_t di;
                if (it == index.end()) {
                    PCell pc;
                    pc.kind = c.kind; pc.scale = 0.0; pc.off = -1;
                    if (!transpose_out) { pc.q = c.q; pc.r0 = c.r0; pc.c0 = c.c0; pc.nr = c.nr; pc.nc = c.nc; }
                    else { pc.q = c.q; pc.r0 = c.c0; pc.c0 = c.r0; pc.nr = c.nc; pc.nc = c.nr; }
                    if (c.kind == DMRGX_CELL_DENSE) pc.off = new_dense(pc.nr, pc.nc);
                    dst.push_back(pc);
                    di = (int32_t)dst.size() - 1;
                    index.emplace(key, di);
                } else di = it->second;
                if (c.kind == DMRGX_CELL_IDENT) dst[di].scale += ct.first * c.scale;
                else {
                    CopyTask k;
                    k.dst_off = dst[di].off; k.src = c.data; k.lds = c.ld;
                    k.nr = dst[di].nr; k.nc = dst[di].nc; k.ldd = dst[di].nc;
                    k.tr = (c.tr != transpose_out) ? 1 : 0;
                    k.a = ct.first; k.round = rounds[di]++;
                    copies.push_back(k);
                }
            }
        }
    };

    {
        std::map<std::pair<int32_t, int32_t>, std::vector<int32_t>> by_key;
        for (int32_t t = 0; t < d->nterms; ++t) {
            const dmrgx_term& T = d->terms[t];
            if (T.a == 0.0) continue;
            if (coverR[T.right_op]) by_key[{1, T.right_op}].push_back(t);
            else if (coverL[T.left_op]) by_key[{0, T.left_op}].push_back(t);
            else DMRGX_FAIL(DMRGX_ERR_INTERNAL, "kron_plan_create: term %d is not covered", t);
        }
        for (auto& kv : by_key) {
            Group g;
            std::vector<std::pair<double, const std::vector<NCell>*>> cl, cr;
            if (kv.first.first == 1) {
                g.sB = d->right_ops[kv.first.second].shift; g.sA = -g.sB;
                cr.push_back({1.0, &Rops[kv.first.second]});
                for (int32_t t : kv.second) cl.push_back({d->terms[t].a, &Lops[d->terms[t].left_op]});
            } else {
                g.sA = d->left_ops[kv.first.second].shift; g.sB = -g.sA;
                cl.push_back({1.0, &Lops[kv.first.second]});
                for (int32_t t : kv.second) cr.push_back({d->terms[t].a, &Rops[d->terms[t].right_op]});
            }
            build_side(cl, false, g.left);
            build_side(cr, true, g.rightT);
            G.push_back(std::move(g));
        }
    }
    std::vector<PCell> PHL, PHRT;
    build_side({{1.0, &HL}}, false, PHL);
    build_side({{1.0, &HR}}, true, PHRT);

    int64_t arena_T = 0;
    std::vector<std::vector<int64_t>> Toff(G.size(), std::vector<int64_t>(nb, -1));
    std::vector<std::vector<int32_t>> Ksrc(G.size(), std::vector<int32_t>(nb, -1));
    for (size_t g = 0; g < G.size(); ++g)
        for (int32_t k = 0; k < nb; ++k) {
            auto it = kmap.find({d->block_il[k] + G[g].sA, d->block_ir[k] + G[g].sB});
            if (it == kmap.end()) continue;
            Ksrc[g][k] = it->second;
            Toff[g][k] = arena_ops + arena_T;
            arena_T += (int64_t)nLk(it->second) * panel_ld(k, me);
        }
    std::vector<int64_t> TRoff(nb, -1);
    if (!PHRT.empty())
        for (int32_t k = 0; k < nb; ++k) { TRoff[k] = arena_ops + arena_T; arena_T += (int64_t)nLk(k) * panel_ld(k, me); }

    Builder B;
    std::vector<ZeroRect> zero_rects;
    auto stage1 = [&](const std::vector<PCell>& cellsT, int32_t sB, int32_t k, int32_t ksrc, int64_t toff) {
        (void)sB;
        const int32_t ir = d->block_ir[k], cs = cbeg(k, me), ce = cend(k, me), w = ce - cs;
        if (w <= 0) return;
        const int32_t M = nLk(ksrc);
        std::set<int32_t> cuts = {cs, ce};
        auto clampc = [&](int32_t v) { return std::min(std::max(v, cs), ce); };
        for (const PCell& c : cellsT) {
            if (c.q != ir) continue;
            cuts.insert(clampc(c.c0)); cuts.insert(clampc(c.c0 + c.nc));
            if (c.kind == DMRGX_CELL_IDENT)
                for (int32_t p = 0; p < W; ++p) { const int32_t sc = cbeg(ksrc, p); if (sc > c.r0 && sc < c.r0 + c.nr) cuts.insert(clampc(c.c0 + (sc - c.r0))); }
        }
        std::vector<int32_t> cv(cuts.begin(), cuts.end());
        for (size_t s = 0; s + 1 < cv.size(); ++s) {
            const int32_t o0 = cv[s], o1 = cv[s + 1];
            if (o0 >= o1) continue;
            bool any = false;
            for (const PCell& c : cellsT) if (c.q == ir && c.c0 <= o0 && c.c0 + c.nc >= o1) { any = true; break; }
            if (!any) { zero_rects.push_back(ZeroRect{toff + (o0 - cs), w, M, o1 - o0, 0}); continue; }
            const int32_t g = B.open(BASE_ARENA, toff + (o0 - cs), w, M, o1 - o0, 0);
            for (const PCell& c : cellsT) {
                if (c.q != ir || c.c0 > o0 || c.c0 + c.nc < o1) continue;
                if (c.kind == DMRGX_CELL_DENSE) {
                    for (int32_t p = 0; p < W; ++p) {
                        const int32_t k0 = std::max(c.r0, cbeg(ksrc, p)), k1 = std::min(c.r0 + c.nr, cend(ksrc, p));
                        if (k0 >= k1) continue;
                        B.add_gemm(BASE_X, panel_off(ksrc, p) + (k0 - cbeg(ksrc, p)), panel_ld(ksrc, p),
                                   BASE_ARENA, c.off + (int64_t)(k0 - c.r0) * c.nc + (o0 - c.c0), c.nc, k1 - k0);
                    }
                } else {
                    const int32_t s0 = c.r0 + (o0 - c.c0);
                    int32_t p = 0;
                    for (int32_t pp = 0; pp < W; ++pp) if (cbeg(ksrc, pp) <= s0 && s0 < cend(ksrc, pp)) p = pp;
                    B.add_axpy(BASE_X, panel_off(ksrc, p) + (s0 - cbeg(ksrc, p)), panel_ld(ksrc, p), c.scale);
                }
            }
            B.close(g, 1);
        }
    };
    for (size_t g = 0; g < G.size(); ++g)
        for (int32_t k = 0; k < nb; ++k) if (Ksrc[g][k] >= 0) stage1(G[g].rightT, G[g].sB, k, Ksrc[g][k], Toff[g][k]);
    if (!PHRT.empty()) for (int32_t k = 0; k < nb; ++k) stage1(PHRT, 0, k, k, TRoff[k]);
    const int32_t n_groups_stage1 = (int32_t)B.groups.size();

    for (int32_t k = 0; k < nb; ++k) {
        const int32_t il = d->block_il[k], w = panel_ld(k, me), nl = nLk(k);
        if (w <= 0) continue;
        std::set<int32_t> cuts = {0, nl};
        for (size_t g = 0; g < G.size(); ++g) if (Ksrc[g][k] >= 0) for (const PCell& c : G[g].left) if (c.q == il) { cuts.insert(c.r0); cuts.insert(c.r0 + c.nr); }
        for (const PCell& c : PHL) if (c.q == il) { cuts.insert(c.r0); cuts.insert(c.r0 + c.nr); }
        std::vector<int32_t> cv(cuts.begin(), cuts.end());
        for (size_t s = 0; s + 1 < cv.size(); ++s) {
            const int32_t ra = cv[s], rb = cv[s + 1];
            const int32_t grp = B.open(BASE_Y, seg_off[me][k] + (int64_t)ra * w, w, rb - ra, w, 0);
            for (size_t g = 0; g < G.size(); ++g) {
                if (Ksrc[g][k] < 0) continue;
                for (const PCell& c : G[g].left) {
                    if (c.q != il || c.r0 > ra || c.r0 + c.nr < rb) continue;
                    if (c.kind == DMRGX_CELL_DENSE)
                        B.add_gemm(BASE_ARENA, c.off + (int64_t)(ra - c.r0) * c.nc, c.nc, BASE_ARENA, Toff[g][k] + (int64_t)c.c0 * w, w, c.nc);
                    else
                        B.add_axpy(BASE_ARENA, Toff[g][k] + (int64_t)(c.c0 + (ra - c.r0)) * w, w, c.scale);
                }
            }
            for (const PCell& c : PHL) {
                if (c.q != il || c.r0 > ra || c.r0 + c.nr < rb) continue;
                if (c.kind == DMRGX_CELL_DENSE)
                    B.add_gemm(BASE_ARENA, c.off + (int64_t)(ra - c.r0) * c.nc, c.nc, BASE_X, panel_off(k, me) + (int64_t)c.c0 * w, w, c.nc);
                else
                    B.add_axpy(BASE_X, panel_off(k, me) + (int64_t)(c.c0 + (ra - c.r0)) * w, w, c.scale);
            }
            if (TRoff[k] >= 0) B.add_axpy(BASE_ARENA, TRoff[k] + (int64_t)ra * w, w, 1.0);
            B.close(grp, 2);
        }
    }

    const int64_t slab_base = arena_ops + arena_T;
    B.finalize_stage2(slab_base);
    const int64_t arena_slabs = B.slab_elems;
    ggemm_schedule(B.tiles1, B.groups);
    ggemm_schedule(B.tiles2, B.groups);
    ggemm_schedule(B.tiles1b, B.groups, 2);
    ggemm_schedule(B.tiles2b, B.groups, 2);
    if (const char* dump = getenv("DMRGX_PLAN_DUMP")) {
        if (FILE* f = fopen(dump, "w")) {
            auto put = [&](const char* name, const std::vector<GTile>& tl) {
                for (size_t i = 0; i < tl.size(); ++i) {
                    const GTile& t = tl[i];
                    if (t.group < 0) { fprintf(f, "%s %zu -1 0 0 0 0 0 0\n", name, i); continue; }
                    const RelGroup& G2 = B.groups[t.group];
                    fprintf(f, "%s %zu %d %d %d %d %d %d %d\n", name, i, t.group, t.tm, t.tn, G2.M, G2.N, B.ksteps(t.group), G2.prod_end - G2.prod_begin);
                }
            };
            put("s1", B.tiles1); put("s2", B.tiles2); put("s1b", B.tiles1b); put("s2b", B.tiles2b);
            for (size_t i = 0; i < zero_rects.size(); ++i) {
                const ZeroRect& z = zero_rects[i];
                fprintf(f, "zr %zu %lld %d %d %d\n", i, (long long)z.off, z.ld, z.nr, z.nc);
            }
            for (size_t i = 0; i < B.red_tasks.size(); ++i) {
                const RedTask& r = B.red_tasks[i];
                fprintf(f, "red %zu %lld %lld %d %d %d %d\n", i, (long long)r.dst_off, (long long)r.slab_off, r.ldc, r.M, r.N, r.nslab);
            }
            fclose(f);
        }
    }

    dmrgx_kron_plan* P = new (std::nothrow) dmrgx_kron_plan();
    if (!P) DMRGX_FAIL(DMRGX_ERR_MEM, "out of host memory");
    std::unique_ptr<dmrgx_kron_plan> guard(P);
    P->world = W; P->rank = me;
    DMRGX_CHK(P->arena.alloc_f64((size_t)std::max<int64_t>(arena_ops + arena_T + arena_slabs, 1), st));
    P->n_red_tiles = (int32_t)B.red_tiles.size();
    {
        int32_t max_round = -1;
        for (auto& c : copies) max_round = std::max(max_round, c.round);
        DevBuf d_tab;
        PackedUpload pk;
        const size_t o_tasks = pk.add(copies);
        const size_t o_zero = pk.add(zero_rects);
        std::vector<std::pair<size_t, size_t>> lists;
        for (int32_t r = 0; r <= max_round; ++r) {
            std::vector<CopyTile> ct;
            for (size_t i = 0; i < copies.size(); ++i) if (copies[i].round == r)
                for (int32_t ti = 0; ti < (copies[i].nr + 31) / 32; ++ti)
                    for (int32_t tj = 0; tj < (copies[i].nc + 31) / 32; ++tj) ct.push_back(CopyTile{(int32_t)i, ti, tj, 0});
            if (ct.empty()) continue;
            lists.push_back({pk.add(ct), ct.size()});
        }
        DMRGX_CHK(pk.upload(d_tab, st));
        if (!zero_rects.empty()) {
            int64_t big = 1;
            for (const ZeroRect& r : zero_rects) big = std::max(big, (int64_t)r.nr * r.nc);
            if (zero_rects.size() >= ((size_t)1 << 23)) DMRGX_FAIL(DMRGX_ERR_ARG, "kron_plan: %zu zero rectangles exceed the launch grid", zero_rects.size());
            hipLaunchKernelGGL(zero_rects_kernel, dim3((unsigned)zero_rects.size(), (unsigned)std::min<int64_t>((big + 2047) / 2048, 512)), dim3(256), 0, st,
                               (const ZeroRect*)packed_at<ZeroRect>(d_tab, o_zero), P->arena.as<double>());
            DMRGX_HIP(hipGetLastError());
        }
        for (const auto& l : lists) {
            hipLaunchKernelGGL(cell_copy_kernel, dim3((unsigned)l.second), dim3(256), 0, st, (const CopyTile*)packed_at<CopyTile>(d_tab, l.first), (const CopyTask*)packed_at<CopyTask>(d_tab, o_tasks), P->arena.as<double>());
            DMRGX_HIP(hipGetLastError());
        }
    }
    P->nprods = (int32_t)B.prods.size(); P->ngroups = (int32_t)B.groups.size();
    P->ntiles1 = (int32_t)B.tiles1.size(); P->ntiles2 = (int32_t)B.tiles2.size();
    P->ntiles1b = (int32_t)B.tiles1b.size(); P->ntiles2b = (int32_t)B.tiles2b.size();
    {
        std::vector<LayoutSeg> segs;
        for (int32_t k = 0; k < nb; ++k) for (int32_t w = 0; w < W; ++w) {
            if (panel_ld(k, w) <= 0) continue;
            segs.push_back(LayoutSeg{ref_off[k] + cbeg(k, w), panel_off(k, w), nLk(k), panel_ld(k, w), nRk(k), panel_ld(k, w)});
        }
        P->nlayout = (int32_t)segs.size();
        PackedUpload pk;
        const size_t o0 = pk.add(B.prods), o1 = pk.add(B.groups), o2 = pk.add(B.tiles1), o3 = pk.add(B.tiles2), o4 = pk.add(B.tiles1b), o5 = pk.add(B.tiles2b),
                     o8 = pk.add(B.red_tasks), o9 = pk.add(B.red_tiles), o10 = pk.add(segs);
        DMRGX_CHK(pk.upload(P->d_tables, st));
        PackedUpload::view<std::decay<decltype(B.prods[0])>::type>(P->d_rprods, P->d_tables, o0, B.prods.size());
        PackedUpload::view<std::decay<decltype(B.groups[0])>::type>(P->d_rgroups, P->d_tables, o1, B.groups.size());
        PackedUpload::view<GTile>(P->d_tiles1, P->d_tables, o2, B.tiles1.size());
        PackedUpload::view<GTile>(P->d_tiles2, P->d_tables, o3, B.tiles2.size());
        PackedUpload::view<GTile>(P->d_tiles1b, P->d_tables, o4, B.tiles1b.size());
        PackedUpload::view<GTile>(P->d_tiles2b, P->d_tables, o5, B.tiles2b.size());
        PackedUpload::view<std::decay<decltype(B.red_tasks[0])>::type>(P->d_red_tasks, P->d_tables, o8, B.red_tasks.size());
        PackedUpload::view<std::decay<decltype(B.red_tiles[0])>::type>(P->d_red_tiles, P->d_tables, o9, B.red_tiles.size());
        PackedUpload::view<LayoutSeg>(P->d_layout, P->d_tables, o10, segs.size());
    }

    {
        std::vector<int64_t> offL(SL.nsec + 1, 0), offR(SR.nsec + 1, 0);
        for (int i = 0; i < SL.nsec; ++i) offL[i + 1] = offL[i] + SL.size[i];
        for (int i = 0; i < SR.nsec; ++i) offR[i + 1] = offR[i] + SR.size[i];
        P->diag_NL = offL[SL.nsec]; P->diag_NR = offR[SR.nsec];
        int32_t nt = 2;
        for (auto& g : G) if (g.sA == 0 && g.sB == 0) ++nt;
        P->diag_terms = nt;
        const int64_t baseB = (int64_t)nt * P->diag_NL;
        std::map<std::tuple<int32_t, int32_t, int32_t>, int32_t> rounds;
        auto add_cells = [&](const std::vector<PCell>& cells, int side, int32_t t, const std::vector<int64_t>& off, bool transposed_storage) {
            for (const PCell& c : cells) {
                const int32_t lo = std::max(c.r0, c.c0), hi = std::min(c.r0 + c.nr, c.c0 + c.nc);
                if (lo >= hi) continue;
                if (c.kind != DMRGX_CELL_DENSE && c.r0 != c.c0) continue;
                DiagSrc d;
                d.n = hi - lo; d.scale = c.scale; d.ld = c.nc;
                d.off = c.kind == DMRGX_CELL_DENSE ? c.off + (int64_t)(lo - c.r0) * c.nc + (lo - c.c0) : -1;
                d.dst = (side == 0 ? (int64_t)t * P->diag_NL : baseB + (int64_t)t * P->diag_NR) + off[c.q] + lo;
                d.round = rounds[std::make_tuple(side, t, c.q)]++;
                P->diag_rounds = std::max(P->diag_rounds, d.round + 1);
                P->diag_src.push_back(d);
                (void)transposed_storage;
            }
        };
        auto add_ones = [&](int side, int32_t t, const dmrgx_sectors& S, const std::vector<int64_t>& off) {
            for (int32_t q = 0; q < S.nsec; ++q) {
                DiagSrc d;
                d.n = S.size[q]; d.scale = 1.0; d.ld = 0; d.off = -1; d.round = rounds[std::make_tuple(side, t, q)]++;
                d.dst = (side == 0 ? (int64_t)t * P->diag_NL : baseB + (int64_t)t * P->diag_NR) + off[q];
                P->diag_rounds = std::max(P->diag_rounds, d.round + 1);
                P->diag_src.push_back(d);
            }
        };
        add_cells(PHL, 0, 0, offL, false); add_ones(1, 0, SR, offR);
        add_ones(0, 1, SL, offL); add_cells(PHRT, 1, 1, offR, true);
        int32_t t = 2;
        for (auto& g : G) {
            if (g.sA != 0 || g.sB != 0) continue;
            add_cells(g.left, 0, t, offL, false); add_cells(g.rightT, 1, t, offR, true);
            ++t;
        }
        for (int32_t k = 0; k < nb; ++k) {
            if (panel_ld(k, me) <= 0) continue;
            P->diag_segs.push_back(DiagSeg{seg_off[me][k], nLk(k), panel_ld(k, me), offL[d->block_il[k]], offR[d->block_ir[k]] + cbeg(k, me)});
        }
    }

    dmrgx_kron_info& I = P->info;
    I.n_states = N; I.vec_len = (W == 1) ? N : (int64_t)W * seg_stride; I.local_offset = (int64_t)me * seg_stride;
    I.local_len = (W == 1) ? N : seg_stride; I.seg_stride = seg_stride;
    I.flops_alg = B.flops_alg; I.flops_exec = B.flops_exec;
    double opbytes = 0;
    auto cellbytes = [&](const std::vector<PCell>& v) { for (auto& c : v) if (c.kind == DMRGX_CELL_DENSE) opbytes += 8.0 * c.nr * c.nc; };
    for (auto& g : G) { cellbytes(g.left); cellbytes(g.rightT); }
    cellbytes(PHL); cellbytes(PHRT);
    I.bytes_alg = opbytes + 8.0 * ((double)N + (double)seg_off[me][nb]);
    I.bytes_workspace = 16.0 * (double)arena_T + 16.0 * (double)B.slab_elems;
    I.n_groups = (int32_t)G.size(); I.n_tiles_stage1 = P->ntiles1 + P->ntiles1b; I.n_tiles_stage2 = P->ntiles2 + P->ntiles2b;
    I.n_tiles_big = P->ntiles1b + P->ntiles2b; I.flops_alg_big = B.flops_alg_big;
    (void)n_groups_stage1;
    *out = guard.release();
    return DMRGX_OK;
}

extern "C" dmrgx_status dmrgx_kron_plan_info(const dmrgx_kron_plan* plan, dmrgx_kron_info* info)
{
    if (!plan || !info) DMRGX_FAIL(DMRGX_ERR_ARG, "kron_plan_info: null argument");
    *info = plan->info;
    return DMRGX_OK;
}

extern "C" dmrgx_status dmrgx_kron_apply(dmrgx_kron_plan* P, const double* x_full, double* y_local, void* stream)
{
    hipStream_t st = (hipStream_t)stream;
    if (!P || !x_full || !y_local) DMRGX_FAIL(DMRGX_ERR_ARG, "kron_apply: null argument");
    dmrgx_kron_plan::Patched* T = nullptr;
    for (auto& c : P->patched) if (c->x == x_full && c->y == y_local) { T = c.get(); break; }
    if (!T) {
        if (P->patched.size() < dmrgx_kron_plan::PATCHED_MAX) {
            std::unique_ptr<dmrgx_kron_plan::Patched> c(new (std::nothrow) dmrgx_kron_plan::Patched());
            if (!c) DMRGX_FAIL(DMRGX_ERR_MEM, "out of host memory");
            DMRGX_CHK(c->prods.alloc(std::max<size_t>((size_t)P->nprods, 1) * sizeof(GProd)));
            DMRGX_CHK(c->groups.alloc(std::max<size_t>((size_t)P->ngroups, 1) * sizeof(GGroup)));
            P->patched.push_back(std::move(c));
            T = P->patched.back().get();
        } else {
            T = P->patched[P->patched_next].get();
            P->patched_next = (P->patched_next + 1) % dmrgx_kron_plan::PATCHED_MAX;
        }
        T->x = x_full; T->y = y_local;
        const int n = std::max(P->nprods, P->ngroups);
        if (n > 0) {
            hipLaunchKernelGGL(patch_tables_kernel, dim3((n + 255) / 256), dim3(256), 0, st,
                               P->d_rprods.as<RelProd>(), T->prods.as<GProd>(), P->nprods,
                               P->d_rgroups.as<RelGroup>(), T->groups.as<GGroup>(), P->ngroups,
                               P->arena.as<double>(), x_full, y_local);
            DMRGX_HIP(hipGetLastError());
        }
    }
    hipEvent_t* e = nullptr;
    if (P->timing && P->ev_used + 5 <= 5 * 4096) {
        while (P->ev.size() < P->ev_used + 5) { hipEvent_t x; DMRGX_HIP(hipEventCreate(&x)); P->ev.push_back(x); }
        e = &P->ev[P->ev_used];
        P->ev_used += 5;
    }
    if (e) DMRGX_HIP(hipEventRecord(e[0], st));
    DMRGX_CHK(ggemm_launch(P->d_tiles1b.as<GTile>(), T->groups.as<GGroup>(), T->prods.as<GProd>(), P->ntiles1b, st, 1));
    if (e) DMRGX_HIP(hipEventRecord(e[1], st));
    DMRGX_CHK(ggemm_launch(P->d_tiles1.as<GTile>(), T->groups.as<GGroup>(), T->prods.as<GProd>(), P->ntiles1, st, 0));
    if (e) DMRGX_HIP(hipEventRecord(e[2], st));
    DMRGX_CHK(ggemm_launch(P->d_tiles2b.as<GTile>(), T->groups.as<GGroup>(), T->prods.as<GProd>(), P->ntiles2b, st, 1));
    if (e) DMRGX_HIP(hipEventRecord(e[3], st));
    DMRGX_CHK(ggemm_launch(P->d_tiles2.as<GTile>(), T->groups.as<GGroup>(), T->prods.as<GProd>(), P->ntiles2, st, 0));
    if (e) DMRGX_HIP(hipEventRecord(e[4], st));
    if (P->n_red_tiles > 0) {
        hipLaunchKernelGGL(slab_reduce_kernel, dim3((unsigned)P->n_red_tiles), dim3(256), 0, st, P->d_red_tiles.as<RedTile>(), P->d_red_tasks.as<RedTask>(), y_local, P->arena.as<double>());
        DMRGX_HIP(hipGetLastError());
    }
    return DMRGX_OK;
}

extern "C" dmrgx_status dmrgx_kron_plan_timing(dmrgx_kron_plan* P, int32_t enable)
{
    if (!P) DMRGX_FAIL(DMRGX_ERR_ARG, "kron_plan_timing: null plan");
    if (enable) P->ev_used = 0;
    P->timing = enable != 0;
    return DMRGX_OK;
}

extern "C" dmrgx_status dmrgx_kron_plan_timing_read(dmrgx_kron_plan* P, double* ms, int64_t* n_applies)
{
    if (!P || !ms || !n_applies) DMRGX_FAIL(DMRGX_ERR_ARG, "kron_plan_timing_read: null argument");
    ms[0] = ms[1] = ms[2] = ms[3] = 0.0; *n_applies = (int64_t)(P->ev_used / 5);
    for (size_t i = 0; i + 4 < P->ev_used; i += 5) {
        DMRGX_HIP(hipEventSynchronize(P->ev[i + 4]));
        for (int k = 0; k < 4; ++k) { float t = 0; DMRGX_HIP(hipEventElapsedTime(&t, P->ev[i + k], P->ev[i + k + 1])); ms[k] += t; }
    }
    return DMRGX_OK;
}

extern "C" dmrgx_status dmrgx_kron_plan_destroy(dmrgx_kron_plan* plan)
{
    if (!plan) return DMRGX_OK;
    delete plan;
    return DMRGX_OK;
}

static dmrgx_status layout_copy(const dmrgx_kron_plan* P, const double* src, double* dst, int to_striped, hipStream_t st)
{
    if (!P || !src || !dst) DMRGX_FAIL(DMRGX_ERR_ARG, "kron_vec layout copy: null argument");
    if (P->nlayout == 0) return DMRGX_OK;
    hipLaunchKernelGGL(layout_copy_kernel, dim3(64, (unsigned)P->nlayout), dim3(256), 0, st, P->d_layout.as<LayoutSeg>(), src, dst, to_striped);
    DMRGX_HIP(hipGetLastError());
    return DMRGX_OK;
}

extern "C" dmrgx_status dmrgx_kron_vec_to_striped(const dmrgx_kron_plan* plan, const double* v_ref_dev, double* v_full_dev, void* stream)
{ return layout_copy(plan, v_ref_dev, v_full_dev, 1, (hipStream_t)stream); }

extern "C" dmrgx_status dmrgx_kron_vec_from_striped(const dmrgx_kron_plan* plan, const double* v_full_dev, double* v_ref_dev, void* stream)
{ return layout_copy(plan, v_full_dev, v_ref_dev, 0, (hipStream_t)stream); }

extern "C" dmrgx_status dmrgx_kron_diag(dmrgx_kron_plan* P, double* d_local, void* stream)
{
    hipStream_t st = (hipStream_t)stream;
    if (!P || !d_local) DMRGX_FAIL(DMRGX_ERR_ARG, "kron_diag: null argument");
    DevBuf dvec, d_src, d_segs;
    const size_t nvec = (size_t)P->diag_terms * (size_t)(P->diag_NL + P->diag_NR);
    DMRGX_CHK(dvec.alloc(std::max<size_t>(nvec, 1) * sizeof(double)));
    DMRGX_HIP(zero_async(dvec.p, dvec.bytes, st));
    DMRGX_HIP(zero_async(d_local, (size_t)P->info.local_len * sizeof(double), st));
    DMRGX_CHK(upload(d_src, P->diag_src, st));
    DMRGX_CHK(upload(d_segs, P->diag_segs, st));
    for (int32_t r = 0; r < P->diag_rounds; ++r) {
        hipLaunchKernelGGL(diag_gather_kernel, dim3((unsigned)P->diag_src.size()), dim3(256), 0, st, d_src.as<DiagSrc>(), (int)P->diag_src.size(), r,
                           (const double*)P->arena.as<double>(), dvec.as<double>());
        DMRGX_HIP(hipGetLastError());
    }
    if (!P->diag_segs.empty()) {
        hipLaunchKernelGGL(diag_fill_kernel, dim3(64, (unsigned)P->diag_segs.size()), dim3(256), 0, st, d_segs.as<DiagSeg>(), (const double*)dvec.as<double>(),
                           (const double*)(dvec.as<double>() + (size_t)P->diag_terms * P->diag_NL), P->diag_terms, P->diag_NL, P->diag_NR, d_local);
        DMRGX_HIP(hipGetLastError());
    }
    return DMRGX_OK;
}
```

### dmrg.x_amd/superblock.py

```python
import ctypes as C

import numpy as np
import torch

from . import _capi
from .workloads import OpSm, OpSz, OpSp, CELL_DENSE, CELL_IDENT


def _i32(values):
    arr = (C.c_int32 * len(values))(*[int(v) for v in values])
    return arr


class KronPlan:
    def __init__(self, sb, device="cuda:0", world_size=1, rank=0, stream=None):
        _capi.require_device()
        self.sb = sb
        self.device = torch.device(device)
        self._keep = []
        L = _capi.lib()

        def secop(op, transposed=False, shift=None):
            cells = (_capi.Cell * max(len(op.cells), 1))()
            for i, c in enumerate(op.cells):
                cells[i].row_sector, cells[i].r0, cells[i].c0, cells[i].nr, cells[i].nc = c.row_sector, c.r0, c.c0, c.nr, c.nc
                cells[i].kind, cells[i].scale = c.kind, c.scale
                if c.kind == CELL_DENSE:
                    t = torch.from_numpy(np.ascontiguousarray(c.array, dtype=np.float64)).to(self.device)
                    self._keep.append(t)
                    cells[i].data, cells[i].ld = t.data_ptr(), c.nc
            self._keep.append(cells)
            s = _capi.SecOp()
            s.shift = op.shift if shift is None else shift
            s.transposed = 1 if transposed else 0
            s.ncells = len(op.cells)
            s.cells = cells
            return s

        def side(ops, which):
            index, lst = {}, []
            for t in sb.terms:
                key = (t[1], t[2]) if which == 0 else (t[3], t[4])
                if key in index:
                    continue
                op, site = key
                if op == OpSm:
                    lst.append(secop(ops[(OpSp, site)], transposed=True, shift=-1))
                else:
                    lst.append(secop(ops[(op, site)]))
                index[key] = len(lst) - 1
            arr = (_capi.SecOp * max(len(lst), 1))(*lst)
            self._keep.append(arr)
            return index, arr, len(lst)

        li, larr, nl = side(sb.left_ops, 0)
        ri, rarr, nr = side(sb.right_ops, 1)
        terms = (_capi.Term * max(len(sb.terms), 1))()
        for i, t in enumerate(sb.terms):
            terms[i].a, terms[i].left_op, terms[i].right_op = t[0], li[(t[1], t[2])], ri[(t[3], t[4])]
        hl = secop(sb.h_left) if sb.h_left is not None else None
        hr = secop(sb.h_right) if sb.h_right is not None else None
        d = _capi.KronDesc()
        ls, rs = _i32(sb.left_sizes), _i32(sb.right_sizes)
        bil, bir = _i32([b[0] for b in sb.blocks]), _i32([b[1] for b in sb.blocks])
        d.left.nsec, d.left.size = len(sb.left_sizes), ls
        d.right.nsec, d.right.size = len(sb.right_sizes), rs
        d.nblocks, d.block_il, d.block_ir = len(sb.blocks), bil, bir
        d.n_left_ops, d.n_right_ops, d.left_ops, d.right_ops = nl, nr, larr, rarr
        d.h_left = C.pointer(hl) if hl is not None else None
        d.h_right = C.pointer(hr) if hr is not None else None
        d.nterms, d.terms = len(sb.terms), terms
        d.world_size, d.rank = world_size, rank
        self._handle = C.c_void_p()
        st = self._stream_ptr(stream)
        with torch.cuda.device(self.device):
            _capi.check(L.dmrgx_kron_plan_create(C.byref(d), st, C.byref(self._handle)))
        self._keep.clear()
        info = _capi.KronInfo()
        _capi.check(L.dmrgx_kron_plan_info(self._handle, C.byref(info)))
        self.info = info
        self.world_size, self.rank = world_size, rank

    @staticmethod
    def _stream_ptr(stream):
        if stream is None:
            stream = torch.cuda.current_stream()
        return C.c_void_p(stream.cuda_stream)

    def new_vector(self):
        return torch.zeros(self.info.vec_len, dtype=torch.float64, device=self.device)

    def apply(self, x_full, y_local, stream=None):
        assert x_full.dtype == torch.float64 and y_local.dtype == torch.float64
        assert x_full.numel() >= self.info.vec_len and y_local.numel() >= self.info.local_len
        _capi.check(_capi.lib().dmrgx_kron_apply(self._handle, C.c_void_p(x_full.data_ptr()), C.c_void_p(y_local.data_ptr()),
                                                 self._stream_ptr(stream)))

    def to_striped(self, v_ref, v_full, stream=None):
        _capi.check(_capi.lib().dmrgx_kron_vec_to_striped(self._handle, C.c_void_p(v_ref.data_ptr()), C.c_void_p(v_full.data_ptr()),
                                                          self._stream_ptr(stream)))

    def from_striped(self, v_full, v_ref, stream=None):
        _capi.check(_capi.lib().dmrgx_kron_vec_from_striped(self._handle, C.c_void_p(v_full.data_ptr()), C.c_void_p(v_ref.data_ptr()),
                                                            self._stream_ptr(stream)))

    def eigs_lowest(self, ncv=16, max_it=1000, tol=1e-8, seed=1, psi0=None, allgather=None, allreduce=None, stream=None,
                    max_matvec=0, comm=None, method=0, min_initial_norm2=0.0, gd_minv=0):
        opts = _capi.EigsOpts()
        opts.ncv, opts.max_it, opts.tol, opts.seed, opts.max_matvec = ncv, max_it, tol, seed, max_matvec
        psi = self.new_vector()
        if psi0 is not None:
            psi.copy_(psi0)
            opts.use_initial = 1
        self._cb = (_capi.ALLGATHER_FN(allgather) if allgather else _capi.ALLGATHER_FN(),
                    _capi.ALLREDUCE_FN(allreduce) if allreduce else _capi.ALLREDUCE_FN())
        opts.allgather, opts.allreduce_sum = self._cb
        opts.comm = comm.handle if comm is not None else None
        opts.method = method
        opts.gd_minv = gd_minv
        opts.min_initial_norm2 = min_initial_norm2
        e0 = C.c_double(0.0)
        stats = _capi.EigsStats()
        rc = _capi.lib().dmrgx_eigs_lowest(self._handle, C.byref(opts), C.byref(e0), C.c_void_p(psi.data_ptr()),
                                           C.byref(stats), self._stream_ptr(stream))
        if not (rc == _capi.DMRGX_ERR_NOTCONV and max_matvec > 0):
            _capi.check(rc)
        return e0.value, psi, stats

    def timing(self, enable):
        _capi.check(_capi.lib().dmrgx_kron_plan_timing(self._handle, 1 if enable else 0))

    def timing_read(self):
        ms, n = (C.c_double * 4)(), C.c_int64(0)
        _capi.check(_capi.lib().dmrgx_kron_plan_timing_read(self._handle, ms, C.byref(n)))
        return list(ms), n.value

    def destroy(self):
        if self._handle:
            _capi.check(_capi.lib().dmrgx_kron_plan_destroy(self._handle))
            self._handle = C.c_void_p()

    def __del__(self):
        try:
            self.destroy()
        except Exception:
            pass


def dgemm_nn(A, B, out=None):
    assert A.dtype == torch.float64 and B.dtype == torch.float64 and A.is_contiguous() and B.is_contiguous()
    M, K = A.shape
    K2, N = B.shape
    assert K == K2
    if out is None:
        out = torch.empty((M, N), dtype=torch.float64, device=A.device)
    st = C.c_void_p(torch.cuda.current_stream().cuda_stream)
    _capi.check(_capi.lib().dmrgx_dgemm_nn(M, N, K, C.c_void_p(A.data_ptr()), K, C.c_void_p(B.data_ptr()), N,
                                           C.c_void_p(out.data_ptr()), N, st))
    return out


class ReducedDensityMatrices:

    def __init__(self, left_sizes, right_sizes, blocks, psi, warm=None):
        L = _capi.lib()
        self.left_sizes, self.right_sizes, self.blocks = list(left_sizes), list(right_sizes), list(blocks)
        ls, rs = _i32(left_sizes), _i32(right_sizes)
        sl, sr = _capi.Sectors(len(left_sizes), ls), _capi.Sectors(len(right_sizes), rs)
        bil, bir = _i32([b[0] for b in blocks]), _i32([b[1] for b in blocks])
        self._handle = C.c_void_p()
        self._psi = psi
        st = C.c_void_p(torch.cuda.current_stream().cuda_stream)
        if warm:
            ptrs = (C.c_void_p * (2 * len(blocks)))()
            for (side, k), t in warm.items():
                assert t.is_contiguous() and t.dtype == torch.float64 and t.shape == (self.size(side, k),) * 2
                ptrs[2 * k + side] = t.data_ptr()
            _capi.check(L.dmrgx_rdm_create_warm(C.byref(sl), C.byref(sr), len(blocks), bil, bir, C.c_void_p(psi.data_ptr()),
                                                C.cast(ptrs, C.c_void_p), st, C.byref(self._handle)))
        else:
            _capi.check(L.dmrgx_rdm_create(C.byref(sl), C.byref(sr), len(blocks), bil, bir, C.c_void_p(psi.data_ptr()), st, C.byref(self._handle)))
        self.report = _capi.RdmReport()
        _capi.check(L.dmrgx_rdm_info(self._handle, C.byref(self.report)))
        self.sweeps = self.report.n_sweeps

    def size(self, side, k):
        return (self.left_sizes[self.blocks[k][0]], self.right_sizes[self.blocks[k][1]])[side]

    def eigenvalues(self, side, k):
        out = (C.c_double * self.size(side, k))()
        _capi.check(_capi.lib().dmrgx_rdm_eigenvalues(self._handle, side, k, out))
        return np.array(out)

    def select(self, counts):
        arr = (C.c_int32 * (2 * len(self.blocks)))(*[int(c) for c in counts])
        _capi.check(_capi.lib().dmrgx_rdm_select(self._handle, arr, None))
        self._psi = None

    def eigenvectors_batch(self, requests):
        outs, tasks = [], (_capi.RdmVecTask * max(len(requests), 1))()
        for i, (side, k, count) in enumerate(requests):
            n = self.size(side, k)
            outs.append(torch.empty((count, n), dtype=torch.float64, device="cuda"))
            tasks[i].side, tasks[i].k, tasks[i].count, tasks[i].dst_dev, tasks[i].ld = side, k, count, outs[-1].data_ptr(), n
        _capi.check(_capi.lib().dmrgx_rdm_eigenvectors_batch(self._handle, len(requests), tasks, None))
        self._psi = None
        return outs

    def eigenvectors(self, side, k, count):
        n = self.size(side, k)
        dst = torch.empty((count, n), dtype=torch.float64, device="cuda")
        st = C.c_void_p(torch.cuda.current_stream().cuda_stream)
        _capi.check(_capi.lib().dmrgx_rdm_eigenvectors(self._handle, side, k, count, C.c_void_p(dst.data_ptr()), n, st))
        if count > 0:
            self._psi = None
        return dst

    def destroy(self):
        if self._handle:
            h, self._handle = self._handle, C.c_void_p()
            self._psi = None
            _capi.check(_capi.lib().dmrgx_rdm_destroy(h))

    def __del__(self):
        try:
            self.destroy()
        except Exception:
            pass


class Communicator:

    def __init__(self, rank, world, unique_id=None, host_staged_name=None):
        L = _capi.lib()
        self.handle = C.c_void_p()
        self.rank, self.world = rank, world
        if host_staged_name is not None:
            _capi.check(L.dmrgx_comm_init_host_staged(rank, world, host_staged_name.encode(), C.byref(self.handle)))
        else:
            assert unique_id is not None and len(unique_id) == 128
            buf = (C.c_uint8 * 128).from_buffer_copy(bytes(unique_id))
            _capi.check(L.dmrgx_comm_init(rank, world, C.cast(buf, C.c_void_p), C.byref(self.handle)))

    @staticmethod
    def unique_id():
        buf = (C.c_uint8 * 128)()
        _capi.check(_capi.lib().dmrgx_comm_unique_id(C.cast(buf, C.c_void_p)))
        return bytes(buf)

    @staticmethod
    def _st(stream):
        return C.c_void_p((stream or torch.cuda.current_stream()).cuda_stream)

    def allgather(self, full, seg_stride, stream=None):
        _capi.check(_capi.lib().dmrgx_comm_allgather(self.handle, C.c_void_p(full.data_ptr()), seg_stride, self._st(stream)))

    def allreduce_sum(self, buf, stream=None):
        _capi.check(_capi.lib().dmrgx_comm_allreduce_sum(self.handle, C.c_void_p(buf.data_ptr()), buf.numel(), self._st(stream)))

    def bcast(self, buf, root, stream=None):
        _capi.check(_capi.lib().dmrgx_comm_bcast(self.handle, C.c_void_p(buf.data_ptr()), buf.numel() * buf.element_size(), root, self._st(stream)))

    def allgather_host(self, arr, stream=None):
        arr = np.ascontiguousarray(arr)
        out = np.empty((self.world,) + arr.shape, dtype=arr.dtype)
        _capi.check(_capi.lib().dmrgx_comm_allgather_host(self.handle, arr.ctypes.data_as(C.c_void_p), out.ctypes.data_as(C.c_void_p), arr.nbytes, self._st(stream)))
        return out

    def barrier(self, stream=None):
        _capi.check(_capi.lib().dmrgx_comm_barrier(self.handle, self._st(stream)))

    def info(self):
        r, w, b = C.c_int32(), C.c_int32(), C.c_int32()
        _capi.check(_capi.lib().dmrgx_comm_info(self.handle, C.byref(r), C.byref(w), C.byref(b)))
        return r.value, w.value, b.value

    def destroy(self):
        if self.handle:
            _capi.check(_capi.lib().dmrgx_comm_destroy(self.handle))
            self.handle = C.c_void_p()
```

### include/dmrgx.h

```cpp
#ifndef DMRGX_H
#define DMRGX_H

#include <stdint.h>
#include <stddef.h>

#ifdef __cplusplus
extern "C" {
#endif

#define DMRGX_ABI_VERSION 3

typedef int32_t dmrgx_status;
enum {
    DMRGX_OK = 0,
    DMRGX_ERR_ARG = 62,
    DMRGX_ERR_OUTOFRANGE = 63,
    DMRGX_ERR_MEM = 55,
    DMRGX_ERR_DEVICE = 97,
    DMRGX_ERR_NOTCONV = 91,
    DMRGX_ERR_INTERNAL = 77
};

int32_t      dmrgx_abi_version(void);
const char*  dmrgx_last_error(void);
dmrgx_status dmrgx_device_count(int32_t* n);

typedef struct dmrgx_comm dmrgx_comm;
#define DMRGX_COMM_ID_BYTES 128
enum { DMRGX_COMM_RCCL = 1, DMRGX_COMM_HOST_STAGED = 2 };
dmrgx_status dmrgx_set_device(int32_t device);
dmrgx_status dmrgx_comm_unique_id(uint8_t* id128);
dmrgx_status dmrgx_comm_init(int32_t rank, int32_t world, const uint8_t* id128, dmrgx_comm** out);
dmrgx_status dmrgx_comm_init_host_staged(int32_t rank, int32_t world, const char* shm_name, dmrgx_comm** out);
dmrgx_status dmrgx_comm_info(const dmrgx_comm* comm, int32_t* rank, int32_t* world, int32_t* backend);
dmrgx_status dmrgx_comm_allgather(dmrgx_comm* comm, double* full_vec_dev, int64_t seg_stride, void* stream);
dmrgx_status dmrgx_comm_allreduce_sum(dmrgx_comm* comm, double* buf_dev, int64_t count, void* stream);
dmrgx_status dmrgx_comm_bcast(dmrgx_comm* comm, void* buf_dev, size_t bytes, int32_t root, void* stream);
dmrgx_status dmrgx_comm_allgather_host(dmrgx_comm* comm, const void* send, void* recv, size_t bytes_per_rank, void* stream);
dmrgx_status dmrgx_comm_barrier(dmrgx_comm* comm, void* stream);
dmrgx_status dmrgx_comm_destroy(dmrgx_comm* comm);

enum { DMRGX_CELL_DENSE = 1, DMRGX_CELL_IDENT = 2 };

typedef struct {
    int32_t row_sector;
    int32_t r0, c0;
    int32_t nr, nc;
    int32_t kind;
    double  scale;
    const double* data;
    int64_t ld;
} dmrgx_cell;

typedef struct {
    int32_t shift;
    int32_t transposed;
    int32_t ncells;
    const dmrgx_cell* cells;
} dmrgx_secop;

typedef struct {
    int32_t nsec;
    const int32_t* size;
} dmrgx_sectors;

typedef struct {
    double  a;
    int32_t left_op;
    int32_t right_op;
} dmrgx_term;

typedef struct {
    dmrgx_sectors left, right;
    int32_t nblocks;
    const int32_t* block_il;
    const int32_t* block_ir;
    int32_t n_left_ops, n_right_ops;
    const dmrgx_secop* left_ops;
    const dmrgx_secop* right_ops;
    const dmrgx_secop* h_left;
    const dmrgx_secop* h_right;
    int32_t nterms;
    const dmrgx_term* terms;
    int32_t world_size, rank;
} dmrgx_kron_desc;

typedef struct dmrgx_kron_plan dmrgx_kron_plan;

typedef struct {
    int64_t n_states;
    int64_t vec_len;
    int64_t local_offset;
    int64_t local_len;
    int64_t seg_stride;
    double  flops_alg;
    double  bytes_alg;
    double  flops_exec;
    double  bytes_workspace;
    int32_t n_groups;
    int32_t n_tiles_stage1, n_tiles_stage2;
    int32_t n_tiles_big;
    double  flops_alg_big;
} dmrgx_kron_info;

dmrgx_status dmrgx_kron_plan_create(const dmrgx_kron_desc* desc, void* stream, dmrgx_kron_plan** out);
dmrgx_status dmrgx_kron_plan_info(const dmrgx_kron_plan* plan, dmrgx_kron_info* info);
dmrgx_status dmrgx_kron_apply(dmrgx_kron_plan* plan, const double* x_full, double* y_local, void* stream);
dmrgx_status dmrgx_kron_plan_destroy(dmrgx_kron_plan* plan);
dmrgx_status dmrgx_kron_diag(dmrgx_kron_plan* plan, double* d_local_dev, void* stream);
dmrgx_status dmrgx_kron_plan_timing(dmrgx_kron_plan* plan, int32_t enable);
dmrgx_status dmrgx_kron_plan_timing_read(dmrgx_kron_plan* plan, double* ms4, int64_t* n_applies);
dmrgx_status dmrgx_kron_vec_to_striped(const dmrgx_kron_plan* plan, const double* v_ref_dev, double* v_full_dev, void* stream);
dmrgx_status dmrgx_kron_vec_from_striped(const dmrgx_kron_plan* plan, const double* v_full_dev, double* v_ref_dev, void* stream);

dmrgx_status dmrgx_stripe_bounds(int32_t n_right, int32_t world_size, int32_t rank, int32_t* c0, int32_t* c1);
dmrgx_status dmrgx_stripe_bounds_of_block(int32_t n_right, int32_t world_size, int32_t rank, int32_t block, int32_t* c0, int32_t* c1);

dmrgx_status dmrgx_dgemm_nn(int32_t M, int32_t N, int32_t K, const double* A, int64_t lda,
                            const double* B, int64_t ldb, double* C, int64_t ldc, void* stream);
typedef struct {
    int32_t M, N, K, accumulate;
    const double* A; int64_t lda;
    const double* B; int64_t ldb;
    double* C; int64_t ldc;
} dmrgx_gemm_task;
dmrgx_status dmrgx_dgemm_batch(int32_t count, const dmrgx_gemm_task* tasks, void* stream);

typedef struct {
    int32_t ncv;
    int32_t max_it;
    double  tol;
    uint64_t seed;
    int32_t use_initial;
    int32_t max_matvec;
    dmrgx_status (*allgather)(void* user, double* full_vec, int64_t seg_stride, void* stream);
    dmrgx_status (*allreduce_sum)(void* user, double* buf, int64_t count, void* stream);
    void* user;
    dmrgx_comm* comm;
    int32_t method;
    double min_initial_norm2;
    int32_t gd_minv;
    int32_t reserved_;
} dmrgx_eigs_opts;

typedef struct {
    int32_t n_matvec;
    int32_t n_restart;
    int32_t converged;
    int32_t start_rejected;
    double  residual;
    double  seconds;
} dmrgx_eigs_stats;

dmrgx_status dmrgx_eigs_lowest(dmrgx_kron_plan* plan, const dmrgx_eigs_opts* opts, double* e0,
                               double* psi_full, dmrgx_eigs_stats* stats, void* stream);

dmrgx_status dmrgx_eigs_comm_timing(double* allgather_ms, double* apply_ms, int64_t* n_matvec, int32_t reset);

typedef struct dmrgx_rdm dmrgx_rdm;
dmrgx_status dmrgx_rdm_create(const dmrgx_sectors* left, const dmrgx_sectors* right, int32_t nblocks,
                              const int32_t* block_il, const int32_t* block_ir, const double* psi_dev,
                              void* stream, dmrgx_rdm** out);
dmrgx_status dmrgx_rdm_create_subset(const dmrgx_sectors* left, const dmrgx_sectors* right, int32_t nblocks,
                                     const int32_t* block_il, const int32_t* block_ir, const double* psi_dev,
                                     const uint8_t* side_mask, void* stream, dmrgx_rdm** out);
dmrgx_status dmrgx_rdm_create_warm(const dmrgx_sectors* left, const dmrgx_sectors* right, int32_t nblocks,
                                   const int32_t* block_il, const int32_t* block_ir, const double* psi_dev,
                                   const double* const* v0_rows, void* stream, dmrgx_rdm** out);
dmrgx_status dmrgx_rdm_eigenvalues(const dmrgx_rdm* rdm, int32_t side, int32_t k, double* host_out);
dmrgx_status dmrgx_rdm_eigenvectors(const dmrgx_rdm* rdm, int32_t side, int32_t k, int32_t count, double* dst_dev, int64_t ld, void* stream);
typedef struct { int32_t side, k, count, pad; double* dst_dev; int64_t ld; } dmrgx_rdm_vec_task;
dmrgx_status dmrgx_rdm_eigenvectors_batch(const dmrgx_rdm* rdm, int32_t ntasks, const dmrgx_rdm_vec_task* tasks, void* stream);
dmrgx_status dmrgx_rdm_select(dmrgx_rdm* rdm, const int32_t* counts, void* stream);
typedef struct {
    int32_t n_sweeps;
    int32_t solver;
    int32_t trid_persistent_matrices;
    int32_t trid_launch_matrices;
    int32_t max_workgroups_per_matrix;
    int32_t merge_levels;
    int32_t wy_blocks_max;
    int32_t timed_out;
    int32_t process_timeouts;
    int32_t persistent_off;
} dmrgx_rdm_report;
dmrgx_status dmrgx_rdm_info(const dmrgx_rdm* rdm, dmrgx_rdm_report* out);
dmrgx_status dmrgx_rdm_destroy(dmrgx_rdm* rdm);

typedef struct {
    double* dst; const double* dst_base; const double* src;
    int64_t ldd, lds; int32_t nr, nc; int32_t transposed; double alpha;
} dmrgx_axpy_task;
dmrgx_status dmrgx_cells_axpy(int32_t ntasks, const dmrgx_axpy_task* tasks, void* stream);

typedef struct {
    int32_t n_new;
    const int32_t* old_sector;
    const int32_t* kept;
    const double* const* rot_t;
} dmrgx_rotation;
dmrgx_status dmrgx_rotate_ops(const dmrgx_sectors* old_sectors, const dmrgx_rotation* rot, int32_t nops,
                              const dmrgx_secop* src_ops, double* const* const* dst_blocks, void* stream);

dmrgx_status dmrgx_malloc(void** dev_ptr, size_t bytes);
dmrgx_status dmrgx_free(void* dev_ptr);
dmrgx_status dmrgx_mem_stats(size_t* in_use, size_t* cached, size_t* peak_in_use);
dmrgx_status dmrgx_memcpy_h2d(void* dst_dev, const void* src_host, size_t bytes, void* stream);
dmrgx_status dmrgx_memcpy_d2h(void* dst_host, const void* src_dev, size_t bytes, void* stream);
dmrgx_status dmrgx_memcpy_d2d(void* dst_dev, const void* src_dev, size_t bytes, void* stream);
dmrgx_status dmrgx_memset_zero(void* dst_dev, size_t bytes, void* stream);
dmrgx_status dmrgx_stream_sync(void* stream);
dmrgx_status dmrgx_dot(int64_t n, const double* x_dev, const double* y_dev, double* host_out, void* stream);
dmrgx_status dmrgx_dot_async(int64_t n, const double* x_dev, const double* y_dev, double* dev_out, void* stream);
typedef struct { const double* a; int64_t lda; const double* b; int64_t ldb; int32_t nr, nc, out, pad; } dmrgx_dot2d_task;
dmrgx_status dmrgx_dot2d_batch(int32_t count, const dmrgx_dot2d_task* tasks, double* dev_out, void* stream);

#ifdef __cplusplus
}
#endif
#endif
```

Baseline: 371.1.

## Fuse Kronecker stage-1 and stage-2 grouped GEMMs into one dataflow launch

Merges the two grouped-GEMM stages of the superblock matvec into a single persistent kernel launch. Stage-2 tiles spin-wait on per-cell atomic counters that stage-1 tiles increment after writing their T intermediate. This removes the kernel boundary and the tail idle time between stages. The cost is polling, extra fences and write-through stores, and a watchdog status word that turns a timeout into a reported error. Prefetch of the next tile is skipped when that tile has dependencies.

```diff
diff --git a/dmrg.x_amd/_capi.py b/dmrg.x_amd/_capi.py
--- a/dmrg.x_amd/_capi.py
+++ b/dmrg.x_amd/_capi.py
@@ -103,6 +103,7 @@
     "dmrgx_kron_apply": (C.c_int32, [C.c_void_p, C.c_void_p, C.c_void_p, C.c_void_p]),
     "dmrgx_kron_plan_destroy": (C.c_int32, [C.c_void_p]),
     "dmrgx_kron_diag": (C.c_int32, [C.c_void_p, C.c_void_p, C.c_void_p]),
+    "dmrgx_kron_plan_stage_mode": (C.c_int32, [C.c_void_p, C.POINTER(C.c_int32), C.POINTER(C.c_int32), C.POINTER(C.c_int32)]),
     "dmrgx_kron_plan_timing": (C.c_int32, [C.c_void_p, C.c_int32]),
     "dmrgx_kron_plan_timing_read": (C.c_int32, [C.c_void_p, C.POINTER(C.c_double), C.POINTER(C.c_int64)]),
     "dmrgx_kron_vec_to_striped": (C.c_int32, [C.c_void_p, C.c_void_p, C.c_void_p, C.c_void_p]),
diff --git a/dmrg.x_amd/csrc/common.h b/dmrg.x_amd/csrc/common.h
--- a/dmrg.x_amd/csrc/common.h
+++ b/dmrg.x_amd/csrc/common.h
@@ -57,6 +57,11 @@
 
 inline int32_t stripe_of_rank(int32_t W, int32_t w, int32_t k) { return (w + k) % W; }
 
+}
+struct dmrgx_kron_plan;
+namespace dmrgx {
+dmrgx_status kron_plan_check_status(const dmrgx_kron_plan* plan);
+
 struct DevBuf {
     void* p = nullptr;
     size_t bytes = 0;
diff --git a/dmrg.x_amd/csrc/eigs.hip b/dmrg.x_amd/csrc/eigs.hip
--- a/dmrg.x_amd/csrc/eigs.hip
+++ b/dmrg.x_amd/csrc/eigs.hip
@@ -597,8 +597,19 @@
     return opts->min_initial_norm2 > 0.0 && pin && !(pin[2] >= opts->min_initial_norm2);
 }
 
+static dmrgx_status eigs_lowest_impl(dmrgx_kron_plan* plan, const dmrgx_eigs_opts* opts, double* e0, double* psi_full, dmrgx_eigs_stats* stats, void* stream);
+
 extern "C" dmrgx_status dmrgx_eigs_lowest(dmrgx_kron_plan* plan, const dmrgx_eigs_opts* opts, double* e0,
                                           double* psi_full, dmrgx_eigs_stats* stats, void* stream)
+{
+    const dmrgx_status rc = eigs_lowest_impl(plan, opts, e0, psi_full, stats, stream);
+    if (rc != DMRGX_OK && rc != DMRGX_ERR_NOTCONV) return rc;
+    DMRGX_CHK(kron_plan_check_status(plan));
+    return rc;
+}
+
+static dmrgx_status eigs_lowest_impl(dmrgx_kron_plan* plan, const dmrgx_eigs_opts* opts, double* e0,
+                                     double* psi_full, dmrgx_eigs_stats* stats, void* stream)
 {
     hipStream_t st = (hipStream_t)stream;
     if (!plan || !opts || !e0 || !psi_full) DMRGX_FAIL(DMRGX_ERR_ARG, "eigs_lowest: null argument");
diff --git a/dmrg.x_amd/csrc/ggemm.h b/dmrg.x_amd/csrc/ggemm.h
--- a/dmrg.x_amd/csrc/ggemm.h
+++ b/dmrg.x_amd/csrc/ggemm.h
@@ -26,9 +26,22 @@
 
 struct GTile { int32_t group, tm, tn, pad; };
 
+struct GDep { int32_t cell, dep_begin, dep_end, pad; };
+struct GWait { int32_t cell, count; };
+struct GFused {
+    const GDep* deps = nullptr;
+    const GWait* waits = nullptr;
+    unsigned* cells = nullptr;
+    unsigned* status = nullptr;
+};
+constexpr unsigned long long GG_POLL_TICKS = 1000000000ull;
+
 constexpr int GG_BM = 64, GG_BN = 64, GG_BK = 16, GG_THREADS = 256;
 
 dmrgx_status ggemm_launch(const GTile* d_tiles, const GGroup* d_groups, const GProd* d_prods, int32_t ntiles, hipStream_t st, int big = 0);
+
+dmrgx_status ggemm_launch_fused(const GTile* d_tiles, const GGroup* d_groups, const GProd* d_prods, int32_t ntiles, const GFused& fz, hipStream_t st);
+void ggemm_fuse_lists(const std::vector<GTile>& s1, const std::vector<GTile>& s2, std::vector<GTile>& out, std::vector<int32_t>& src);
 
 constexpr int GG_CLUSTER = 8;
 inline void ggemm_append_tiles(std::vector<GTile>& tiles, int32_t g, int32_t M, int32_t N, int32_t cost = 1) {
diff --git a/dmrg.x_amd/csrc/ggemm.hip b/dmrg.x_amd/csrc/ggemm.hip
--- a/dmrg.x_amd/csrc/ggemm.hip
+++ b/dmrg.x_amd/csrc/ggemm.hip
@@ -31,6 +31,10 @@
 typedef const GTile __attribute__((address_space(4)))* ktile_ptr;
 typedef const GGroup __attribute__((address_space(4)))* kgroup_ptr;
 typedef const GProd __attribute__((address_space(4)))* kprod_ptr;
+typedef const GDep __attribute__((address_space(4)))* kdep_ptr;
+typedef const GWait __attribute__((address_space(4)))* kwait_ptr;
+typedef unsigned __attribute__((address_space(1)))* gu32;
+__device__ __forceinline__ GDep kload(kdep_ptr p, int i) { GDep r; r.cell = p[i].cell; r.dep_begin = p[i].dep_begin; r.dep_end = p[i].dep_end; r.pad = p[i].pad; return r; }
 __device__ __forceinline__ GTile kload(ktile_ptr p, int i) { GTile r; r.group = p[i].group; r.tm = p[i].tm; r.tn = p[i].tn; r.pad = p[i].pad; return r; }
 __device__ __forceinline__ GGroup kload(kgroup_ptr p, int i)
 {
@@ -47,10 +51,13 @@
 }
 
 
-template <int TR, int TC, int WR, int WC, bool DEEP>
+template <int TR, int TC, int WR, int WC, bool DEEP, bool FUSED>
 __device__ __forceinline__ void
-ggemm_body(const GTile* __restrict__ tiles_, const GGroup* __restrict__ groups_, const GProd* __restrict__ prods_, int ntiles, int* __restrict__ ctr GG_TRACE_PARAM)
-{
+ggemm_body(const GTile* __restrict__ tiles_, const GGroup* __restrict__ groups_, const GProd* __restrict__ prods_, int ntiles, int* __restrict__ ctr,
+           const GFused fz GG_TRACE_PARAM)
+{
+    const kdep_ptr deps = (kdep_ptr)fz.deps;
+    const kwait_ptr waits = (kwait_ptr)fz.waits;
     const ktile_ptr tiles = (ktile_ptr)tiles_;
     const kgroup_ptr groups = (kgroup_ptr)groups_;
     const kprod_ptr prods = (kprod_ptr)prods_;
@@ -76,6 +83,8 @@
     GTile tl = kload(tiles, t);
     if (tl.group < 0) return;
     GGroup g = kload(groups, tl.group);
+    GDep dp = GDep{-1, 0, 0, 0};
+    if constexpr (FUSED) dp = kload(deps, t);
     const GTile tl_none = GTile{-1, 0, 0, 0};
 #define GG_LANES()                                                                            \
     int tp_ = tid;                                                                            \
@@ -349,6 +358,29 @@
 #pragma unroll
             for (int ni = 0; ni < TC; ++ni) acc[mi][ni] = (d4){0.0, 0.0, 0.0, 0.0};
 
+        if constexpr (FUSED) if (dp.dep_end > dp.dep_begin) {
+            if (wave == 0) {
+                if (tid == 0) {
+                    const unsigned long long t0_ = __builtin_amdgcn_s_memrealtime();
+                    bool alive = true;
+                    for (int i = dp.dep_begin; i < dp.dep_end && alive; ++i) {
+                        const int c_ = waits[i].cell;
+                        const unsigned want_ = (unsigned)waits[i].count;
+                        while (__hip_atomic_load((gu32)fz.cells + c_, __ATOMIC_RELAXED, __HIP_MEMORY_SCOPE_AGENT) < want_) {
+                            __builtin_amdgcn_s_sleep(16);
+                            if (__builtin_amdgcn_s_memrealtime() - t0_ > GG_POLL_TICKS) {
+                                __hip_atomic_store(fz.status, 1u, __ATOMIC_RELAXED, __HIP_MEMORY_SCOPE_SYSTEM);
+                                alive = false;
+                                break;
+                            }
+                        }
+                    }
+                }
+                __builtin_amdgcn_fence(__ATOMIC_ACQUIRE, "agent");
+                asm volatile("s_waitcnt vmcnt(0)" ::: "memory");
+            }
+            __syncthreads();
+        }
         const int pend = g.prod_end;
         const int p0 = tl.pad >= 0 ? tl.pad : pend;
         if (npre == 0 && p0 < pend) {
@@ -374,6 +406,7 @@
                 if (vm_after == NA + NB) { GG_VMWAIT(NA + NB); }
                 else if (vm_after == NA + NB + TR * TC * 4) { GG_VMWAIT(NA + NB + TR * TC * 4); }
                 else if (vm_after == TR * TC * 4) { GG_VMWAIT(TR * TC * 4); }
+                else if (FUSED && vm_after == -2) { GG_VMWAIT(1); }
                 else { GG_VMWAIT(0); }
                 GG_LSTORE_D(0, 0);
             } else GG_LSTORE_C(0);
@@ -413,6 +446,8 @@
         GProd pr_n = GProd{nullptr, nullptr, 0, 0, 0, 0, 0.0};
         if (nx) g_n = kload(groups, tl_n.group);
         if (nx && tl_n.pad >= 0) pr_n = kload(prods, tl_n.pad);
+        GDep dp_n = GDep{-1, 0, 0, 0};
+        if constexpr (FUSED) { if (nx) dp_n = kload(deps, t_n); }
 
         int tq = tid;
         asm volatile("" : "+v"(tq));
@@ -529,15 +564,19 @@
         GG_STAMP(4);
 
         vm_after = 0;
-        if (nx && tl_n.pad >= 0) {
-            GG_LOADER_TILE(tl_n, g_n);
-            lp = tl_n.pad; lk = 0; lpend = g_n.prod_end;
-            GG_PRODUCT_SET(pr_n);
-            if (DEEP) { GG_GLOAD_D(0); npre = 1; if (lmore) { GG_GLOAD_D(1); npre = 2; vm_after = NA + NB; } }
-            else { GG_GLOAD_C(); npre = 1; }
-        }
-
-        if (full_tile && !g.accumulate) {
+#define GG_PREFETCH_NEXT()                                                                    \
+        {                                                                                     \
+            GG_LOADER_TILE(tl_n, g_n);                                                        \
+            lp = tl_n.pad; lk = 0; lpend = g_n.prod_end;                                      \
+            GG_PRODUCT_SET(pr_n);                                                             \
+            if (DEEP) { GG_GLOAD_D(0); npre = 1; if (lmore) { GG_GLOAD_D(1); npre = 2; vm_after = NA + NB; } } \
+            else { GG_GLOAD_C(); npre = 1; }                                                  \
+        }
+        if constexpr (FUSED) { if (nx && tl_n.pad >= 0 && !(dp_n.dep_end > dp_n.dep_begin)) GG_PREFETCH_NEXT(); }
+        else { if (nx && tl_n.pad >= 0) GG_PREFETCH_NEXT(); }
+#undef GG_PREFETCH_NEXT
+
+        if (full_tile && !g.accumulate && !(FUSED && dp.cell >= 0)) {
             const unsigned lo = ((unsigned)erow * (unsigned)g.ldc + (unsigned)ecol) * 8u;
 #pragma unroll
             for (int mi = 0; mi < TR; ++mi)
@@ -549,6 +588,17 @@
                         asm volatile("global_store_dwordx2 %0, %1, %2 offset:%3" : : "v"(lo), "v"(acc[mi][ni][r]), "s"(C), "n"(ni * 128) : "memory");
                 }
             vm_after += TR * TC * 4;
+        } else if (FUSED && full_tile && !g.accumulate) {
+            const unsigned lo = ((unsigned)erow * (unsigned)g.ldc + (unsigned)ecol) * 8u;
+#pragma unroll
+            for (int mi = 0; mi < TR; ++mi)
+#pragma unroll
+                for (int r = 0; r < 4; ++r) {
+                    char __attribute__((address_space(1)))* C = (char __attribute__((address_space(1)))*)(g.C + (size_t)(m0 + mi * 16 + 4 * r) * g.ldc + n0);
+#pragma unroll
+                    for (int ni = 0; ni < TC; ++ni)
+                        asm volatile("global_store_dwordx2 %0, %1, %2 offset:%3 sc1" : : "v"(lo), "v"(acc[mi][ni][r]), "s"(C), "n"(ni * 128) : "memory");
+                }
         } else {
             vm_after = -1;
             char __attribute__((address_space(1)))* C = (char __attribute__((address_space(1)))*)(g.C + (size_t)m0 * g.ldc + n0);
@@ -563,15 +613,26 @@
                         const int col = ecol + ni * 16;
                         if (row < mrem && col < nrem && mi < tr_eff && ni < tc_eff) {
                             gwptr c = (gwptr)(C + (ro + (unsigned)col) * 8u);
-                            *c = g.accumulate ? (*c + acc[mi][ni][r]) : acc[mi][ni][r];
+                            if constexpr (FUSED) {
+                                const double v_ = g.accumulate ? (*c + acc[mi][ni][r]) : acc[mi][ni][r];
+                                if (dp.cell >= 0) __hip_atomic_store(c, v_, __ATOMIC_RELAXED, __HIP_MEMORY_SCOPE_AGENT);
+                                else *c = v_;
+                            } else
+                                *c = g.accumulate ? (*c + acc[mi][ni][r]) : acc[mi][ni][r];
                         }
                     }
                 }
         }
+        if constexpr (FUSED) if (dp.cell >= 0) {
+            asm volatile("s_waitcnt vmcnt(0)" ::: "memory");
+            __syncthreads();
+            if (tid == 0) __hip_atomic_fetch_add((gu32)fz.cells + dp.cell, 1u, __ATOMIC_RELAXED, __HIP_MEMORY_SCOPE_AGENT);
+            vm_after = -2;
+        }
         GG_STAMP(5);
         GG_STAMP_ID();
         if (!nx) break;
-        t = t_n; tl = tl_n; g = g_n;
+        t = t_n; tl = tl_n; g = g_n; dp = dp_n;
     }
 #undef GG_STREAM
 #undef GG_STEP
@@ -590,12 +651,18 @@
 __global__ void __launch_bounds__(256) __attribute__((amdgpu_waves_per_eu(5, 5)))
 ggemm_kernel_64(const GTile* __restrict__ tiles, const GGroup* __restrict__ groups, const GProd* __restrict__ prods, int ntiles, int* __restrict__ ctr GG_TRACE_PARAM)
 {
-    ggemm_body<2, 2, 2, 2, true>(tiles, groups, prods, ntiles, ctr GG_TRACE_FWD);
+    ggemm_body<2, 2, 2, 2, true, false>(tiles, groups, prods, ntiles, ctr, GFused{} GG_TRACE_FWD);
+}
+__global__ void __launch_bounds__(256) __attribute__((amdgpu_waves_per_eu(5, 5)))
+ggemm_kernel_64_fused(const GTile* __restrict__ tiles, const GGroup* __restrict__ groups, const GProd* __restrict__ prods, int ntiles, int* __restrict__ ctr,
+                      const GFused fz GG_TRACE_PARAM)
+{
+    ggemm_body<2, 2, 2, 2, true, true>(tiles, groups, prods, ntiles, ctr, fz GG_TRACE_FWD);
 }
 __global__ void __launch_bounds__(512, 4)
 ggemm_kernel_128(const GTile* __restrict__ tiles, const GGroup* __restrict__ groups, const GProd* __restrict__ prods, int ntiles, int* __restrict__ ctr GG_TRACE_PARAM)
 {
-    ggemm_body<4, 2, 2, 4, false>(tiles, groups, prods, ntiles, ctr GG_TRACE_FWD);
+    ggemm_body<4, 2, 2, 4, false, false>(tiles, groups, prods, ntiles, ctr, GFused{} GG_TRACE_FWD);
 }
 
 
@@ -676,6 +743,26 @@
 #define GG_TRACE_ARG
 #endif
 
+static dmrgx_status claim_counters(hipStream_t st, int** ctr)
+{
+    constexpr unsigned HALF = 512;
+    struct Ring { int* base; unsigned next; };
+    static std::mutex mu;
+    static std::map<std::pair<int, hipStream_t>, Ring> rings;
+    int dev = 0;
+    DMRGX_HIP(hipGetDevice(&dev));
+    std::lock_guard<std::mutex> lock(mu);
+    Ring& r = rings[std::make_pair(dev, st)];
+    if (!r.base) { DMRGX_HIP(hipMalloc((void**)&r.base, 2 * HALF * 16 * sizeof(int))); r.next = 0; }
+    const unsigned slot = r.next % (2 * HALF);
+    if (slot % HALF == 0) DMRGX_HIP(hipMemsetAsync(r.base + (size_t)slot * 16, 0, HALF * 16 * sizeof(int), st));
+    r.next = slot + 1;
+    *ctr = r.base + (size_t)slot * 16;
+    return DMRGX_OK;
+}
+
+constexpr size_t gg_lds64 = (2 * 64 * (GG_BK + 2) + 2 * GG_BK * (64 + 16)) * sizeof(double) + 16, gg_lds128 = (2 * 128 * (GG_BK + 2) + 2 * GG_BK * (128 + 16)) * sizeof(double) + 16;
+
 dmrgx_status ggemm_launch(const GTile* d_tiles, const GGroup* d_groups, const GProd* d_prods, int32_t ntiles, hipStream_t st, int big)
 {
     if (ntiles <= 0) return DMRGX_OK;
@@ -685,26 +772,43 @@
 #endif
     const unsigned grid = (unsigned)std::min(ntiles, ggemm_slots(big ? 2 : 1));
     int* ctr = nullptr;
-    if (ntiles > (int32_t)grid) {
-        constexpr unsigned HALF = 512;
-        struct Ring { int* base; unsigned next; };
-        static std::mutex mu;
-        static std::map<std::pair<int, hipStream_t>, Ring> rings;
-        int dev = 0;
-        DMRGX_HIP(hipGetDevice(&dev));
-        std::lock_guard<std::mutex> lock(mu);
-        Ring& r = rings[std::make_pair(dev, st)];
-        if (!r.base) { DMRGX_HIP(hipMalloc((void**)&r.base, 2 * HALF * 16 * sizeof(int))); r.next = 0; }
-        const unsigned slot = r.next % (2 * HALF);
-        if (slot % HALF == 0) DMRGX_HIP(hipMemsetAsync(r.base + (size_t)slot * 16, 0, HALF * 16 * sizeof(int), st));
-        r.next = slot + 1;
-        ctr = r.base + (size_t)slot * 16;
-    }
-    constexpr size_t lds64 = (2 * 64 * (GG_BK + 2) + 2 * GG_BK * (64 + 16)) * sizeof(double) + 16, lds128 = (2 * 128 * (GG_BK + 2) + 2 * GG_BK * (128 + 16)) * sizeof(double) + 16;
-    if (big) hipLaunchKernelGGL(ggemm_kernel_128, dim3(grid), dim3(512), lds128, st, d_tiles, d_groups, d_prods, ntiles, ctr GG_TRACE_ARG);
-    else hipLaunchKernelGGL(ggemm_kernel_64, dim3(grid), dim3(256), lds64, st, d_tiles, d_groups, d_prods, ntiles, ctr GG_TRACE_ARG);
+    if (ntiles > (int32_t)grid) DMRGX_CHK(claim_counters(st, &ctr));
+    if (big) hipLaunchKernelGGL(ggemm_kernel_128, dim3(grid), dim3(512), gg_lds128, st, d_tiles, d_groups, d_prods, ntiles, ctr GG_TRACE_ARG);
+    else hipLaunchKernelGGL(ggemm_kernel_64, dim3(grid), dim3(256), gg_lds64, st, d_tiles, d_groups, d_prods, ntiles, ctr GG_TRACE_ARG);
     DMRGX_HIP(hipGetLastError());
     return DMRGX_OK;
 }
 
-}
+dmrgx_status ggemm_launch_fused(const GTile* d_tiles, const GGroup* d_groups, const GProd* d_prods, int32_t ntiles, const GFused& fz, hipStream_t st)
+{
+    if (ntiles <= 0) return DMRGX_OK;
+#ifdef DMRGX_TILE_TRACE
+    unsigned long long* trace_ = nullptr;
+    if (g_trace_buf && g_trace_used + (size_t)ntiles * 8 <= g_trace_cap) { trace_ = g_trace_buf + g_trace_used; g_trace_used += (size_t)ntiles * 8; }
+#endif
+    const unsigned grid = (unsigned)std::min(ntiles, ggemm_slots(1));
+    int* ctr = nullptr;
+    if (ntiles > (int32_t)grid) DMRGX_CHK(claim_counters(st, &ctr));
+    hipLaunchKernelGGL(ggemm_kernel_64_fused, dim3(grid), dim3(256), gg_lds64, st, d_tiles, d_groups, d_prods, ntiles, ctr, fz GG_TRACE_ARG);
+    DMRGX_HIP(hipGetLastError());
+    return DMRGX_OK;
+}
+
+void ggemm_fuse_lists(const std::vector<GTile>& s1, const std::vector<GTile>& s2, std::vector<GTile>& out, std::vector<int32_t>& src)
+{
+    std::vector<int32_t> q[8];
+    for (size_t i = 0; i < s1.size(); ++i) if (s1[i].group >= 0) q[i & 7].push_back((int32_t)i);
+    for (size_t i = 0; i < s2.size(); ++i) if (s2[i].group >= 0) q[i & 7].push_back((int32_t)(s1.size() + i));
+    size_t maxq = 0;
+    for (int x = 0; x < 8; ++x) maxq = std::max(maxq, q[x].size());
+    out.assign(maxq * 8, GTile{-1, 0, 0, -1});
+    src.assign(maxq * 8, -1);
+    for (int x = 0; x < 8; ++x)
+        for (size_t p = 0; p < q[x].size(); ++p) {
+            const int32_t i = q[x][p];
+            out[p * 8 + x] = (size_t)i < s1.size() ? s1[(size_t)i] : s2[(size_t)i - s1.size()];
+            src[p * 8 + x] = i;
+        }
+}
+
+}
diff --git a/dmrg.x_amd/csrc/kron_plan.hip b/dmrg.x_amd/csrc/kron_plan.hip
--- a/dmrg.x_amd/csrc/kron_plan.hip
+++ b/dmrg.x_amd/csrc/kron_plan.hip
@@ -1,11 +1,13 @@
 #include "ggemm.h"
 #include <algorithm>
+#include <array>
 #include <functional>
 #include <map>
 #include <set>
 #include <tuple>
 #include <cstring>
 #include <memory>
+#include <mutex>
 #include <new>
 
 namespace dmrgx {
@@ -171,6 +173,35 @@
         gg[i] = g;
     }
 }
+}
+
+static bool fused_stages_default(int64_t n1, int64_t n2)
+{
+    (void)n1; (void)n2;
+    return true;
+}
+
+static std::mutex g_status_mu;
+static std::vector<unsigned*> g_status_free;
+static unsigned* status_word_acquire()
+{
+    std::lock_guard<std::mutex> lock(g_status_mu);
+    if (g_status_free.empty()) {
+        unsigned* chunk = nullptr;
+        constexpr size_t N = 1024;
+        if (hipHostMalloc((void**)&chunk, N * sizeof(unsigned), hipHostMallocDefault) != hipSuccess) { (void)hipGetLastError(); return nullptr; }
+        for (size_t i = 0; i < N; ++i) g_status_free.push_back(chunk + (N - 1 - i));
+    }
+    unsigned* w = g_status_free.back();
+    g_status_free.pop_back();
+    *(volatile unsigned*)w = 0u;
+    return w;
+}
+static void status_word_release(unsigned* w)
+{
+    if (!w) return;
+    std::lock_guard<std::mutex> lock(g_status_mu);
+    g_status_free.push_back(w);
 }
 
 struct dmrgx_kron_plan {
@@ -193,10 +224,21 @@
     std::vector<DiagSeg> diag_segs;
     int32_t diag_terms = 0, diag_rounds = 0;
     int64_t diag_NL = 0, diag_NR = 0;
+    bool fused = false;
+    DevBuf d_tilesf, d_deps, d_waits;
+    int32_t ntilesf = 0, ncells = 0;
+    struct CellRing { DevBuf buf; unsigned next = 0; };
+    std::map<hipStream_t, std::unique_ptr<CellRing>> cell_rings;
+    static constexpr unsigned CELL_HALF = 32;
+    unsigned* status = nullptr;
     bool timing = false;
     std::vector<hipEvent_t> ev;
     size_t ev_used = 0;
-    ~dmrgx_kron_plan() { for (hipEvent_t e : ev) (void)hipEventDestroy(e); }
+    ~dmrgx_kron_plan()
+    {
+        for (hipEvent_t e : ev) (void)hipEventDestroy(e);
+        status_word_release(status);
+    }
 };
 
 namespace {
@@ -503,6 +545,10 @@
     build_side({{1.0, &HL}}, false, PHL);
     build_side({{1.0, &HR}}, true, PHRT);
 
+    arena_ops = (arena_ops + 15) / 16 * 16;
+    auto t_ld = [&](int32_t k) { return (panel_ld(k, me) + 15) / 16 * 16; };
+    struct TMat { int64_t off; int32_t ld, rows, w; };
+    std::vector<TMat> tmats;
     int64_t arena_T = 0;
     std::vector<std::vector<int64_t>> Toff(G.size(), std::vector<int64_t>(nb, -1));
     std::vector<std::vector<int32_t>> Ksrc(G.size(), std::vector<int32_t>(nb, -1));
@@ -512,11 +558,16 @@
             if (it == kmap.end()) continue;
             Ksrc[g][k] = it->second;
             Toff[g][k] = arena_ops + arena_T;
-            arena_T += (int64_t)nLk(it->second) * panel_ld(k, me);
+            if (panel_ld(k, me) > 0) tmats.push_back(TMat{Toff[g][k], t_ld(k), nLk(it->second), panel_ld(k, me)});
+            arena_T += (int64_t)nLk(it->second) * t_ld(k);
         }
     std::vector<int64_t> TRoff(nb, -1);
     if (!PHRT.empty())
-        for (int32_t k = 0; k < nb; ++k) { TRoff[k] = arena_ops + arena_T; arena_T += (int64_t)nLk(k) * panel_ld(k, me); }
+        for (int32_t k = 0; k < nb; ++k) {
+            TRoff[k] = arena_ops + arena_T;
+            if (panel_ld(k, me) > 0) tmats.push_back(TMat{TRoff[k], t_ld(k), nLk(k), panel_ld(k, me)});
+            arena_T += (int64_t)nLk(k) * t_ld(k);
+        }
 
     Builder B;
     std::vector<ZeroRect> zero_rects;
@@ -524,7 +575,7 @@
         (void)sB;
         const int32_t ir = d->block_ir[k], cs = cbeg(k, me), ce = cend(k, me), w = ce - cs;
         if (w <= 0) return;
-        const int32_t M = nLk(ksrc);
+        const int32_t M = nLk(ksrc), tld = t_ld(k);
         std::set<int32_t> cuts = {cs, ce};
         auto clampc = [&](int32_t v) { return std::min(std::max(v, cs), ce); };
         for (const PCell& c : cellsT) {
@@ -539,8 +590,8 @@
             if (o0 >= o1) continue;
             bool any = false;
             for (const PCell& c : cellsT) if (c.q == ir && c.c0 <= o0 && c.c0 + c.nc >= o1) { any = true; break; }
-            if (!any) { zero_rects.push_back(ZeroRect{toff + (o0 - cs), w, M, o1 - o0, 0}); continue; }
-            const int32_t g = B.open(BASE_ARENA, toff + (o0 - cs), w, M, o1 - o0, 0);
+            if (!any) { zero_rects.push_back(ZeroRect{toff + (o0 - cs), tld, M, o1 - o0, 0}); continue; }
+            const int32_t g = B.open(BASE_ARENA, toff + (o0 - cs), tld, M, o1 - o0, 0);
             for (const PCell& c : cellsT) {
                 if (c.q != ir || c.c0 > o0 || c.c0 + c.nc < o1) continue;
                 if (c.kind == DMRGX_CELL_DENSE) {
@@ -566,7 +617,7 @@
     const int32_t n_groups_stage1 = (int32_t)B.groups.size();
 
     for (int32_t k = 0; k < nb; ++k) {
-        const int32_t il = d->block_il[k], w = panel_ld(k, me), nl = nLk(k);
+        const int32_t il = d->block_il[k], w = panel_ld(k, me), nl = nLk(k), tld = t_ld(k);
         if (w <= 0) continue;
         std::set<int32_t> cuts = {0, nl};
         for (size_t g = 0; g < G.size(); ++g) if (Ksrc[g][k] >= 0) for (const PCell& c : G[g].left) if (c.q == il) { cuts.insert(c.r0); cuts.insert(c.r0 + c.nr); }
@@ -580,9 +631,9 @@
                 for (const PCell& c : G[g].left) {
                     if (c.q != il || c.r0 > ra || c.r0 + c.nr < rb) continue;
                     if (c.kind == DMRGX_CELL_DENSE)
-                        B.add_gemm(BASE_ARENA, c.off + (int64_t)(ra - c.r0) * c.nc, c.nc, BASE_ARENA, Toff[g][k] + (int64_t)c.c0 * w, w, c.nc);
+                        B.add_gemm(BASE_ARENA, c.off + (int64_t)(ra - c.r0) * c.nc, c.nc, BASE_ARENA, Toff[g][k] + (int64_t)c.c0 * tld, tld, c.nc);
                     else
-                        B.add_axpy(BASE_ARENA, Toff[g][k] + (int64_t)(c.c0 + (ra - c.r0)) * w, w, c.scale);
+                        B.add_axpy(BASE_ARENA, Toff[g][k] + (int64_t)(c.c0 + (ra - c.r0)) * tld, tld, c.scale);
                 }
             }
             for (const PCell& c : PHL) {
@@ -592,7 +643,7 @@
                 else
                     B.add_axpy(BASE_X, panel_off(k, me) + (int64_t)(c.c0 + (ra - c.r0)) * w, w, c.scale);
             }
-            if (TRoff[k] >= 0) B.add_axpy(BASE_ARENA, TRoff[k] + (int64_t)ra * w, w, 1.0);
+            if (TRoff[k] >= 0) B.add_axpy(BASE_ARENA, TRoff[k] + (int64_t)ra * tld, tld, 1.0);
             B.close(grp, 2);
         }
     }
@@ -604,6 +655,80 @@
     ggemm_schedule(B.tiles2, B.groups);
     ggemm_schedule(B.tiles1b, B.groups, 2);
     ggemm_schedule(B.tiles2b, B.groups, 2);
+    struct PTile { int32_t r0, r1, c0, c1, cell; };
+    std::vector<GTile> tilesf;
+    std::vector<int32_t> fsrc;
+    std::vector<GDep> fdeps;
+    std::vector<GWait> fwaits;
+    std::vector<int32_t> cell_count;
+    std::vector<std::array<int32_t, 6>> dump_prod, dump_read;
+    bool fused = false;
+    {
+        const char* env = getenv("DMRGX_FUSED_STAGES");
+        bool want = fused_stages_default((int64_t)B.tiles1.size(), (int64_t)B.tiles2.size());
+        if (env && env[0]) want = env[0] != '0';
+        fused = want && B.tiles1b.empty() && B.tiles2b.empty() && !B.tiles1.empty() && !B.tiles2.empty();
+    }
+    if (fused) {
+        const bool dumping = getenv("DMRGX_PLAN_DUMP") != nullptr;
+        auto tmat_of = [&](int64_t off) -> int32_t {
+            if (tmats.empty() || off < tmats.front().off || off >= arena_ops + arena_T) return -1;
+            size_t lo = 0, hi = tmats.size();
+            while (hi - lo > 1) { const size_t mid = (lo + hi) / 2; if (tmats[mid].off <= off) lo = mid; else hi = mid; }
+            return (int32_t)lo;
+        };
+        ggemm_fuse_lists(B.tiles1, B.tiles2, tilesf, fsrc);
+        const int32_t n1 = (int32_t)B.tiles1.size();
+        fdeps.assign(tilesf.size(), GDep{-1, 0, 0, 0});
+        std::vector<std::vector<PTile>> ptiles(tmats.size());
+        std::map<std::pair<int32_t, int32_t>, int32_t> cell_of;
+        for (size_t i = 0; i < tilesf.size() && fused; ++i) {
+            if (fsrc[i] < 0 || fsrc[i] >= n1) continue;
+            const GTile& t = tilesf[i];
+            const RelGroup& G2 = B.groups[t.group];
+            const int32_t tm = G2.c_base == BASE_ARENA ? tmat_of(G2.c_off) : -1;
+            if (tm < 0) { fused = false; break; }
+            const int32_t col0 = (int32_t)((G2.c_off - tmats[tm].off) % tmats[tm].ld), row0 = (int32_t)((G2.c_off - tmats[tm].off) / tmats[tm].ld);
+            PTile pt;
+            pt.r0 = row0 + t.tm * GG_BM; pt.r1 = row0 + std::min(G2.M, (t.tm + 1) * GG_BM);
+            const int32_t c0 = col0 + t.tn * GG_BN, c1 = col0 + std::min(G2.N, (t.tn + 1) * GG_BN);
+            pt.c0 = c0 / 16 * 16; pt.c1 = (c1 + 15) / 16 * 16;
+            auto ins = cell_of.emplace(std::make_pair(tm, pt.c0 / GG_BN), (int32_t)cell_count.size());
+            if (ins.second) cell_count.push_back(0);
+            pt.cell = ins.first->second;
+            ++cell_count[(size_t)pt.cell];
+            fdeps[i].cell = pt.cell;
+            ptiles[(size_t)tm].push_back(pt);
+            if (dumping) dump_prod.push_back({(int32_t)i, tm, pt.r0, pt.r1, c0, c1});
+        }
+        std::vector<int32_t> cells;
+        for (size_t i = 0; i < tilesf.size() && fused; ++i) {
+            if (fsrc[i] < n1) continue;
+            const GTile& t = tilesf[i];
+            const RelGroup& G2 = B.groups[t.group];
+            const int32_t m0 = t.tm * GG_BM, n0 = t.tn * GG_BN, mrem = std::min(GG_BM, G2.M - m0), nrem = std::min(GG_BN, G2.N - n0);
+            cells.clear();
+            for (int32_t q = G2.prod_begin; q < G2.prod_end; ++q) {
+                const RelProd& pr = B.prods[q];
+                if (pr.b_base != BASE_ARENA) continue;
+                const int32_t tm = tmat_of(pr.b_off);
+                if (tm < 0) continue;
+                const int64_t rel = pr.b_off - tmats[tm].off;
+                const int32_t row0 = (int32_t)(rel / tmats[tm].ld), colb = (int32_t)(rel % tmats[tm].ld);
+                const int32_t r0 = pr.kind == GPROD_GEMM ? row0 : row0 + m0, r1 = pr.kind == GPROD_GEMM ? row0 + pr.K : row0 + m0 + mrem;
+                const int32_t c0 = colb + n0, c1 = colb + n0 + nrem;
+                if (dumping) dump_read.push_back({(int32_t)i, tm, r0, r1, c0, c1});
+                for (const PTile& pt : ptiles[(size_t)tm])
+                    if (pt.r0 < r1 && r0 < pt.r1 && pt.c0 < c1 && c0 < pt.c1) cells.push_back(pt.cell);
+            }
+            std::sort(cells.begin(), cells.end());
+            cells.erase(std::unique(cells.begin(), cells.end()), cells.end());
+            fdeps[i].dep_begin = (int32_t)fwaits.size();
+            for (int32_t c : cells) fwaits.push_back(GWait{c, cell_count[(size_t)c]});
+            fdeps[i].dep_end = (int32_t)fwaits.size();
+        }
+        if (!fused) { tilesf.clear(); fsrc.clear(); fdeps.clear(); fwaits.clear(); cell_count.clear(); dump_prod.clear(); dump_read.clear(); }
+    }
     if (const char* dump = getenv("DMRGX_PLAN_DUMP")) {
         if (FILE* f = fopen(dump, "w")) {
             auto put = [&](const char* name, const std::vector<GTile>& tl) {
@@ -615,6 +740,21 @@
                 }
             };
             put("s1", B.tiles1); put("s2", B.tiles2); put("s1b", B.tiles1b); put("s2b", B.tiles2b);
+            fprintf(f, "fused %d\n", fused ? 1 : 0);
+            for (size_t i = 0; i < tmats.size(); ++i) fprintf(f, "tmat %zu %lld %d %d %d\n", i, (long long)tmats[i].off, tmats[i].ld, tmats[i].rows, tmats[i].w);
+            if (fused) {
+                put("sf", tilesf);
+                for (size_t i = 0; i < fsrc.size(); ++i) if (fsrc[i] >= 0) fprintf(f, "src %zu %d %d\n", i, fsrc[i] < (int32_t)B.tiles1.size() ? 1 : 2, fsrc[i] < (int32_t)B.tiles1.size() ? fsrc[i] : fsrc[i] - (int32_t)B.tiles1.size());
+                for (size_t i = 0; i < cell_count.size(); ++i) fprintf(f, "dc %zu %d\n", i, cell_count[i]);
+                for (const auto& r : dump_prod) fprintf(f, "pt %d %d %d %d %d %d %d\n", r[0], fdeps[(size_t)r[0]].cell, r[1], r[2], r[3], r[4], r[5]);
+                for (const auto& r : dump_read) fprintf(f, "ur %d %d %d %d %d %d\n", r[0], r[1], r[2], r[3], r[4], r[5]);
+                for (size_t i = 0; i < fdeps.size(); ++i) {
+                    if (fsrc[i] < (int32_t)B.tiles1.size()) continue;
+                    fprintf(f, "uw %zu", i);
+                    for (int32_t w = fdeps[i].dep_begin; w < fdeps[i].dep_end; ++w) fprintf(f, " %d", fwaits[(size_t)w].cell);
+                    fprintf(f, "\n");
+                }
+            }
             for (size_t i = 0; i < zero_rects.size(); ++i) {
                 const ZeroRect& z = zero_rects[i];
                 fprintf(f, "zr %zu %lld %d %d %d\n", i, (long long)z.off, z.ld, z.nr, z.nc);
@@ -675,7 +815,8 @@
         P->nlayout = (int32_t)segs.size();
         PackedUpload pk;
         const size_t o0 = pk.add(B.prods), o1 = pk.add(B.groups), o2 = pk.add(B.tiles1), o3 = pk.add(B.tiles2), o4 = pk.add(B.tiles1b), o5 = pk.add(B.tiles2b),
-                     o8 = pk.add(B.red_tasks), o9 = pk.add(B.red_tiles), o10 = pk.add(segs);
+                     o8 = pk.add(B.red_tasks), o9 = pk.add(B.red_tiles), o10 = pk.add(segs),
+                     o11 = pk.add(tilesf), o12 = pk.add(fdeps), o13 = pk.add(fwaits);
         DMRGX_CHK(pk.upload(P->d_tables, st));
         PackedUpload::view<std::decay<decltype(B.prods[0])>::type>(P->d_rprods, P->d_tables, o0, B.prods.size());
         PackedUpload::view<std::decay<decltype(B.groups[0])>::type>(P->d_rgroups, P->d_tables, o1, B.groups.size());
@@ -686,6 +827,14 @@
         PackedUpload::view<std::decay<decltype(B.red_tasks[0])>::type>(P->d_red_tasks, P->d_tables, o8, B.red_tasks.size());
         PackedUpload::view<std::decay<decltype(B.red_tiles[0])>::type>(P->d_red_tiles, P->d_tables, o9, B.red_tiles.size());
         PackedUpload::view<LayoutSeg>(P->d_layout, P->d_tables, o10, segs.size());
+        PackedUpload::view<GTile>(P->d_tilesf, P->d_tables, o11, tilesf.size());
+        PackedUpload::view<GDep>(P->d_deps, P->d_tables, o12, fdeps.size());
+        PackedUpload::view<GWait>(P->d_waits, P->d_tables, o13, fwaits.size());
+        P->fused = fused; P->ntilesf = (int32_t)tilesf.size(); P->ncells = (int32_t)cell_count.size();
+        if (fused) {
+            P->status = status_word_acquire();
+            if (!P->status) DMRGX_FAIL(DMRGX_ERR_MEM, "kron_plan: no pinned memory for the status word");
+        }
     }
 
     {
@@ -745,7 +894,9 @@
     for (auto& g : G) { cellbytes(g.left); cellbytes(g.rightT); }
     cellbytes(PHL); cellbytes(PHRT);
     I.bytes_alg = opbytes + 8.0 * ((double)N + (double)seg_off[me][nb]);
-    I.bytes_workspace = 16.0 * (double)arena_T + 16.0 * (double)B.slab_elems;
+    double t_elems = 0;
+    for (const auto& tmx : tmats) t_elems += (double)tmx.rows * tmx.w;
+    I.bytes_workspace = 16.0 * t_elems + 16.0 * (double)B.slab_elems;
     I.n_groups = (int32_t)G.size(); I.n_tiles_stage1 = P->ntiles1 + P->ntiles1b; I.n_tiles_stage2 = P->ntiles2 + P->ntiles2b;
     I.n_tiles_big = P->ntiles1b + P->ntiles2b; I.flops_alg_big = B.flops_alg_big;
     (void)n_groups_stage1;
@@ -760,10 +911,27 @@
     return DMRGX_OK;
 }
 
+dmrgx_status dmrgx::kron_plan_check_status(const dmrgx_kron_plan* P)
+{
+    if (P && P->status && *(volatile const unsigned*)P->status != 0u)
+        DMRGX_FAIL(DMRGX_ERR_INTERNAL, "kron plan: a stage-2 unit of a fused launch gave up waiting for its stage-1 tiles (status word %u); results of this plan are invalid", *(volatile const unsigned*)P->status);
+    return DMRGX_OK;
+}
+
+extern "C" dmrgx_status dmrgx_kron_plan_stage_mode(const dmrgx_kron_plan* plan, int32_t* fused, int32_t* n_cells, int32_t* status)
+{
+    if (!plan) DMRGX_FAIL(DMRGX_ERR_ARG, "kron_plan_stage_mode: null plan");
+    if (fused) *fused = plan->fused ? 1 : 0;
+    if (n_cells) *n_cells = plan->ncells;
+    if (status) *status = plan->status ? (int32_t)*(volatile const unsigned*)plan->status : 0;
+    return DMRGX_OK;
+}
+
 extern "C" dmrgx_status dmrgx_kron_apply(dmrgx_kron_plan* P, const double* x_full, double* y_local, void* stream)
 {
     hipStream_t st = (hipStream_t)stream;
     if (!P || !x_full || !y_local) DMRGX_FAIL(DMRGX_ERR_ARG, "kron_apply: null argument");
+    DMRGX_CHK(kron_plan_check_status(P));
     dmrgx_kron_plan::Patched* T = nullptr;
     for (auto& c : P->patched) if (c->x == x_full && c->y == y_local) { T = c.get(); break; }
     if (!T) {
@@ -794,6 +962,28 @@
         e = &P->ev[P->ev_used];
         P->ev_used += 5;
     }
+    if (P->fused) {
+        auto& slot = P->cell_rings[st];
+        if (!slot) slot.reset(new (std::nothrow) dmrgx_kron_plan::CellRing());
+        if (!slot) DMRGX_FAIL(DMRGX_ERR_MEM, "out of host memory");
+        constexpr unsigned HALF = dmrgx_kron_plan::CELL_HALF;
+        const size_t nc = ((size_t)std::max(P->ncells, 1) + 3) / 4 * 4;
+        if (!slot->buf.p) { DMRGX_CHK(slot->buf.alloc(2 * HALF * nc * sizeof(unsigned))); slot->next = 0; }
+        const unsigned pos = slot->next % (2 * HALF);
+        if (pos % HALF == 0) DMRGX_HIP(hipMemsetAsync(slot->buf.as<unsigned>() + (size_t)pos * nc, 0, HALF * nc * sizeof(unsigned), st));
+        slot->next = pos + 1;
+        GFused fz;
+        fz.deps = P->d_deps.as<GDep>(); fz.waits = P->d_waits.as<GWait>();
+        fz.cells = slot->buf.as<unsigned>() + (size_t)pos * nc; fz.status = P->status;
+        if (e) DMRGX_HIP(hipEventRecord(e[1], st));
+        DMRGX_CHK(ggemm_launch_fused(P->d_tilesf.as<GTile>(), T->groups.as<GGroup>(), T->prods.as<GProd>(), P->ntilesf, fz, st));
+        if (e) DMRGX_HIP(hipEventRecord(e[2], st));
+        if (P->n_red_tiles > 0) {
+            hipLaunchKernelGGL(slab_reduce_kernel, dim3((unsigned)P->n_red_tiles), dim3(256), 0, st, P->d_red_tiles.as<RedTile>(), P->d_red_tasks.as<RedTask>(), y_local, P->arena.as<double>());
+            DMRGX_HIP(hipGetLastError());
+        }
+        return DMRGX_OK;
+    }
     if (e) DMRGX_HIP(hipEventRecord(e[0], st));
     DMRGX_CHK(ggemm_launch(P->d_tiles1b.as<GTile>(), T->groups.as<GGroup>(), T->prods.as<GProd>(), P->ntiles1b, st, 1));
     if (e) DMRGX_HIP(hipEventRecord(e[1], st));
@@ -822,6 +1012,13 @@
 {
     if (!P || !ms || !n_applies) DMRGX_FAIL(DMRGX_ERR_ARG, "kron_plan_timing_read: null argument");
     ms[0] = ms[1] = ms[2] = ms[3] = 0.0; *n_applies = (int64_t)(P->ev_used / 5);
+    if (P->fused) {
+        for (size_t i = 0; i + 4 < P->ev_used; i += 5) {
+            DMRGX_HIP(hipEventSynchronize(P->ev[i + 2]));
+            float t = 0; DMRGX_HIP(hipEventElapsedTime(&t, P->ev[i + 1], P->ev[i + 2])); ms[1] += t;
+        }
+        return DMRGX_OK;
+    }
     for (size_t i = 0; i + 4 < P->ev_used; i += 5) {
         DMRGX_HIP(hipEventSynchronize(P->ev[i + 4]));
         for (int k = 0; k < 4; ++k) { float t = 0; DMRGX_HIP(hipEventElapsedTime(&t, P->ev[i + k], P->ev[i + k + 1])); ms[k] += t; }
diff --git a/dmrg.x_amd/superblock.py b/dmrg.x_amd/superblock.py
--- a/dmrg.x_amd/superblock.py
+++ b/dmrg.x_amd/superblock.py
@@ -130,6 +130,11 @@
     def timing(self, enable):
         _capi.check(_capi.lib().dmrgx_kron_plan_timing(self._handle, 1 if enable else 0))
 
+    def stage_mode(self):
+        f, n, s = C.c_int32(0), C.c_int32(0), C.c_int32(0)
+        _capi.check(_capi.lib().dmrgx_kron_plan_stage_mode(self._handle, C.byref(f), C.byref(n), C.byref(s)))
+        return bool(f.value), n.value, s.value
+
     def timing_read(self):
         ms, n = (C.c_double * 4)(), C.c_int64(0)
         _capi.check(_capi.lib().dmrgx_kron_plan_timing_read(self._handle, ms, C.byref(n)))
diff --git a/include/dmrgx.h b/include/dmrgx.h
--- a/include/dmrgx.h
+++ b/include/dmrgx.h
@@ -108,6 +108,7 @@
 dmrgx_status dmrgx_kron_apply(dmrgx_kron_plan* plan, const double* x_full, double* y_local, void* stream);
 dmrgx_status dmrgx_kron_plan_destroy(dmrgx_kron_plan* plan);
 dmrgx_status dmrgx_kron_diag(dmrgx_kron_plan* plan, double* d_local_dev, void* stream);
+dmrgx_status dmrgx_kron_plan_stage_mode(const dmrgx_kron_plan* plan, int32_t* fused, int32_t* n_cells, int32_t* status);
 dmrgx_status dmrgx_kron_plan_timing(dmrgx_kron_plan* plan, int32_t enable);
 dmrgx_status dmrgx_kron_plan_timing_read(dmrgx_kron_plan* plan, double* ms4, int64_t* n_applies);
 dmrgx_status dmrgx_kron_vec_to_striped(const dmrgx_kron_plan* plan, const double* v_ref_dev, double* v_full_dev, void* stream);
```

New measurement: 363.7, median of 2. 0.98x the previous value.
